# kubernetes-sigs/karpenter

Measured on NVIDIA H100. Metric: pods scheduled/sec, higher is better.
Workload: dtype int64

## Files before the change

### karpenter_b200/csrc/kp_api.cu

```cuda
#include <cuda_runtime.h>
#include <cub/cub.cuh>

#include <dlfcn.h>

#include <chrono>
#include <cstdio>
#include <cstdlib>
#include <memory>
#include <string>
#include <vector>

#include "kp_consolidate.cuh"
#include "kp_gosort_host.hpp"
#include "kp_prep.hpp"

#define CK(call)                                                                                     \
  do {                                                                                               \
    cudaError_t e_ = (call);                                                                         \
    if (e_ != cudaSuccess) {                                                                         \
      h->err = std::string(#call) + ": " + cudaGetErrorString(e_);                                   \
      return KP_ERR_CUDA;                                                                            \
    }                                                                                                \
  } while (0)

struct Arena {
  struct Chunk {
    char* base;
    size_t cap, used;
  };
  std::vector<Chunk> chunks;
  size_t bytes = 0;
  template <class T>
  cudaError_t alloc(T** out, size_t n) {
    size_t need = (std::max<size_t>(n, 1) * sizeof(T) + 255) & ~(size_t)255;
    bytes += need;
    for (auto& c : chunks)
      if (c.cap - c.used >= need) {
        *out = (T*)(c.base + c.used);
        c.used += need;
        return cudaSuccess;
      }
    size_t cap = std::max<size_t>(need, (size_t)32 << 20);
    void* p = nullptr;
    cudaError_t e = cudaMalloc(&p, cap);
    if (e != cudaSuccess) return e;
    chunks.push_back(Chunk{(char*)p, cap, need});
    *out = (T*)p;
    return cudaSuccess;
  }
  void reset() {
    if (chunks.size() > 1) {
      size_t total = bytes + bytes / 4;
      destroy();
      void* p = nullptr;
      if (cudaMalloc(&p, total) == cudaSuccess) chunks.push_back(Chunk{(char*)p, total, 0});
    }
    for (auto& c : chunks) c.used = 0;
    bytes = 0;
  }
  void destroy() {
    for (auto& c : chunks) cudaFree(c.base);
    chunks.clear();
  }
};

struct Instance {
  KpDev dev;
  HostTables host;
  bool resident = false;
  int64_t P = 0;
  int n_keys = 0, n_resources = 0, n_its = 0, hostname_key = -1, n_nodes = 0;
  std::vector<int> key_nvalues;
  std::vector<int64_t> tmpl_remaining0;
  int32_t* d_pod_class = nullptr;
  int64_t* d_pod_creation = nullptr;
  uint64_t *d_uid_hi = nullptr, *d_uid_lo = nullptr;
  int64_t* d_class_rank = nullptr;
  int32_t *d_nsig_rs = nullptr, *d_nsig_tolset = nullptr;
  int64_t* d_rv_req = nullptr;
  int strict_undefined = 0;
  struct Reset {
    void* dst;
    const void* src;
    size_t bytes;
  };
  std::vector<Reset> resets;
  const int32_t* d_host_cnt_nodes = nullptr;
  const uint32_t* d_host_pop_nodes = nullptr;
  void *sort_keys_a = nullptr, *sort_keys_b = nullptr, *sort_tmp = nullptr;
  int32_t* sort_perm_b = nullptr;
  size_t sort_tmp_bytes = 0;
  bool lean = false;
  bool cohort = false;
  int max_its = 0;
  PriceTabs price_tabs{};
  double* trunc_key = nullptr;
  int32_t* trunc_val = nullptr;
  unsigned long long* trunc_bits = nullptr;
  uint8_t* d_dropped = nullptr;
  int CS = 0, CR = 0;
  size_t smem = 0;
  int32_t* d_slot_src = nullptr;
  int64_t n_slots = 0, slot_off = 0;
};

struct NcclApi {
  void* lib = nullptr;
  int (*GetUniqueId)(void*) = nullptr;
  int (*CommInitRank)(void**, int,  struct KpNcclId, int) = nullptr;
  int (*AllReduce)(const void*, void*, size_t, int, int, void*, cudaStream_t) = nullptr;
  int (*CommDestroy)(void*) = nullptr;
  const char* (*GetErrorString)(int) = nullptr;
};
struct KpNcclId {
  char internal[128];
};
static NcclApi g_nccl;
static bool nccl_load(std::string& err) {
  if (g_nccl.lib) return true;
  void* lib = dlopen("libnccl.so.2", RTLD_NOW | RTLD_GLOBAL);
  if (!lib) lib = dlopen("libnccl.so", RTLD_NOW | RTLD_GLOBAL);
  if (!lib) {
    err = std::string("NCCL is not available: ") + dlerror();
    return false;
  }
  g_nccl.GetUniqueId = (int (*)(void*))dlsym(lib, "ncclGetUniqueId");
  g_nccl.CommInitRank = (int (*)(void**, int, KpNcclId, int))dlsym(lib, "ncclCommInitRank");
  g_nccl.AllReduce = (int (*)(const void*, void*, size_t, int, int, void*, cudaStream_t))dlsym(lib, "ncclAllReduce");
  g_nccl.CommDestroy = (int (*)(void*))dlsym(lib, "ncclCommDestroy");
  g_nccl.GetErrorString = (const char* (*)(int))dlsym(lib, "ncclGetErrorString");
  if (!g_nccl.GetUniqueId || !g_nccl.CommInitRank || !g_nccl.AllReduce || !g_nccl.CommDestroy) {
    err = "libnccl lacks an expected symbol";
    return false;
  }
  g_nccl.lib = lib;
  return true;
}

struct kp_handle {
  int device = 0;
  int n_sm = 132;
  cudaStream_t stream = nullptr;
  std::string err;
  Arena arena;
  enum Uploader { NONE, SINGLE, BATCH } uploaded = NONE;
  std::vector<std::unique_ptr<Instance>> insts;
  KpDev* d_devs = nullptr;
  int2* d_plan = nullptr;
  int devs_cap = 0;
  void* comm = nullptr;
  int comm_rank = 0, comm_world = 1;
  int32_t* d_gcnt = nullptr;
  int64_t gcnt_slots = 0;
  float allreduce_ms = 0;
  cudaEvent_t ev3 = nullptr;
  kp_stats stats{};
  cudaEvent_t ev0 = nullptr, ev1 = nullptr;
};

template <class T>
static cudaError_t up(kp_handle* h, const T** dst, const std::vector<T>& v) {
  T* p;
  cudaError_t e = h->arena.alloc(&p, v.size());
  if (e != cudaSuccess) return e;
  if (!v.empty()) e = cudaMemcpyAsync(p, v.data(), v.size() * sizeof(T), cudaMemcpyHostToDevice, h->stream);
  h->stats.bytes_h2d += v.size() * sizeof(T);
  *dst = p;
  return e;
}
template <class T>
static cudaError_t up_mut(kp_handle* h, Instance& in, T** dst, const std::vector<T>& v) {
  const T* init;
  cudaError_t e = up(h, &init, v);
  if (e != cudaSuccess) return e;
  T* work;
  e = h->arena.alloc(&work, v.size());
  if (e != cudaSuccess) return e;
  if (!v.empty()) in.resets.push_back(Instance::Reset{work, init, v.size() * sizeof(T)});
  *dst = work;
  return cudaSuccess;
}
template <class T>
static cudaError_t up_raw(kp_handle* h, T** dst, const T* src, size_t n) {
  T* p;
  cudaError_t e = h->arena.alloc(&p, n);
  if (e != cudaSuccess) return e;
  if (n) e = cudaMemcpyAsync(p, src, n * sizeof(T), cudaMemcpyHostToDevice, h->stream);
  h->stats.bytes_h2d += n * sizeof(T);
  *dst = p;
  return e;
}
template <class T>
static cudaError_t zeros(kp_handle* h, T** dst, size_t n) {
  T* p;
  cudaError_t e = h->arena.alloc(&p, n);
  if (e != cudaSuccess) return e;
  e = cudaMemsetAsync(p, 0, std::max<size_t>(n, 1) * sizeof(T), h->stream);
  *dst = p;
  return e;
}

__global__ void k_sort_keys(const int32_t* pod_class, const int64_t* class_rank, const int32_t* perm, int64_t n,
                            int64_t* out) {
  int64_t i = blockIdx.x * (int64_t)blockDim.x + threadIdx.x;
  if (i < n) out[i] = class_rank[pod_class[perm[i]]];
}
template <class T>
__global__ void k_gather(const T* src, const int32_t* perm, int64_t n, T* out) {
  int64_t i = blockIdx.x * (int64_t)blockDim.x + threadIdx.x;
  if (i < n) out[i] = src[perm[i]];
}
__global__ void k_fill_i32(int32_t* p, int64_t n, int32_t v) {
  int64_t i = blockIdx.x * (int64_t)blockDim.x + threadIdx.x;
  if (i < n) p[i] = v;
}

__global__ void k_scatter_counts(const int32_t* dom_cnt, const int32_t* slot_src, int64_t n, int32_t* out) {
  int64_t i = blockIdx.x * (int64_t)blockDim.x + threadIdx.x;
  if (i < n) out[i] = dom_cnt[slot_src[i]];
}

__global__ void k_slot_kats(const int64_t* val_int, uint64_t isint, uint64_t univ, const kp_slot_case* cs, int n, kp_slot_out* out) {
  const int i = blockIdx.x * blockDim.x + threadIdx.x;
  if (i >= n) return;
  const KeyInfo ki{val_int, isint, univ};
  const kp_slot_case c = cs[i];
  const Slot a{c.flags_a, c.mask_a, c.gte_a, c.lte_a}, b{c.flags_b, c.mask_b, c.gte_b, c.lte_b};
  kp_slot_out o;
  memset(&o, 0, sizeof(o));
  if (slot_present(a) && slot_present(b)) {
    const Slot r = slot_intersection(ki, a, b);
    o.mask = r.m;
    o.gte = r.gte;
    o.lte = r.lte;
    o.flags = r.f;
    o.op = slot_op(r);
    o.has_intersection = slot_has_intersection(ki, a, b);
  }
  o.has_value = c.value >= 0 ? slot_has(ki, a, c.value) : 0;
  o.compatible = slot_compatible(ki, a, b, c.well_known != 0, c.allow_undefined != 0);
  out[i] = o;
}

static int kp_consolidate_impl(kp_handle* h, const kp_problem* p, const kp_consol_input* in, int64_t deadline_ms,
                               kp_consol_result* out);
extern "C" {

int kp_debug_slot_algebra(kp_handle* h, const int64_t* value_int, uint64_t value_is_int, uint64_t universe,
                          const kp_slot_case* cases, int32_t n, kp_slot_out* out) {
  if (n < 0 || !value_int || (n > 0 && (!cases || !out))) return h->err = "kp_debug_slot_algebra: bad arguments", KP_ERR_INVALID;
  cudaSetDevice(h->device);
  int64_t* dv = nullptr;
  kp_slot_case* dc = nullptr;
  kp_slot_out* dout = nullptr;
  CK(cudaMalloc(&dv, 64 * 8));
  CK(cudaMalloc(&dc, sizeof(kp_slot_case) * std::max(n, 1)));
  CK(cudaMalloc(&dout, sizeof(kp_slot_out) * std::max(n, 1)));
  CK(cudaMemcpy(dv, value_int, 64 * 8, cudaMemcpyHostToDevice));
  CK(cudaMemcpy(dc, cases, sizeof(kp_slot_case) * n, cudaMemcpyHostToDevice));
  if (n > 0) k_slot_kats<<<(n + 127) / 128, 128, 0, h->stream>>>(dv, value_is_int, universe, dc, n, dout);
  CK(cudaStreamSynchronize(h->stream));
  CK(cudaGetLastError());
  CK(cudaMemcpy(out, dout, sizeof(kp_slot_out) * n, cudaMemcpyDeviceToHost));
  cudaFree(dv);
  cudaFree(dc);
  cudaFree(dout);
  return KP_OK;
}
}

extern "C" {

#define KP_TRUNC_BLOCKS 132
int kp_version(void) { return KP_ABI_VERSION; }

int kp_go_sort_f64(const double* keys, int32_t n, int32_t* perm_out) {
  if (n < 0 || (n > 0 && (!keys || !perm_out))) return KP_ERR_INVALID;
  host_go_sort(keys, n, perm_out);
  return KP_OK;
}
int kp_go_sort_i64(const int64_t* keys, int32_t n, int32_t* perm_out) {
  if (n < 0 || (n > 0 && (!keys || !perm_out))) return KP_ERR_INVALID;
  host_go_sort(keys, n, perm_out);
  return KP_OK;
}

int kp_create(int device, kp_handle** out) {
  *out = nullptr;
  int count = 0;
  if (cudaGetDeviceCount(&count) != cudaSuccess || count == 0) return KP_ERR_CUDA;
  kp_handle* h = new kp_handle();
  if (device < 0) cudaGetDevice(&device);
  h->device = device;
  if (cudaSetDevice(device) != cudaSuccess || cudaStreamCreate(&h->stream) != cudaSuccess) {
    delete h;
    return KP_ERR_CUDA;
  }
  cudaEventCreate(&h->ev0);
  cudaEventCreate(&h->ev1);
  cudaEventCreate(&h->ev3);
  cudaDeviceGetAttribute(&h->n_sm, cudaDevAttrMultiProcessorCount, device);
// ... 38 lines not shown
  d.E = t.E;
  d.D = t.D;
  d.n_reqsets = t.n_reqsets;
  d.n_taintsets = t.n_taintsets;
  d.n_tolsets = t.n_tolsets;
  d.has_bounds = t.has_bounds;
  d.hostname_key = t.hostname_key;
  d.nodes_res = t.nodes_res;
  d.n_rv = t.n_rv;
  d.stable_order = p->claim_order_mode == 1;
  CK(up(h, &d.key_wellknown, t.key_wellknown));
  CK(up(h, &d.key_univ, t.key_univ));
  CK(up(h, &d.val_int, t.val_int));
  CK(up(h, &d.val_isint, t.val_isint));
  CK(up(h, &d.rs_flags, t.rs_flags));
  CK(up(h, &d.rs_mask, t.rs_mask));
  CK(up(h, &d.rs_gte, t.rs_gte));
  CK(up(h, &d.rs_lte, t.rs_lte));
  CK(up(h, &d.tol_ok, t.tol_ok));
  CK(up(h, &d.itv_off, t.itv_off));
  CK(up(h, &d.itv, t.itv));
  CK(up(h, &d.it_nokey, t.it_nokey));
  CK(up(h, &d.it_dne, t.it_dne));
  CK(up(h, &d.it_nonempty, t.it_nonempty));
  CK(up(h, &d.it_valid, t.it_valid));
  CK(up(h, &d.ge_off, t.ge_off));
  CK(up(h, &d.ge_vals, t.ge_vals));
  CK(up(h, &d.ge_bits, t.ge_bits));
  d.n_ge = (int)t.ge_vals.size();
  d.n_itv = std::max(t.itv_off[d.K], 1);
  CK(up(h, &d.off_slots, t.off_slots));
  CK(up(h, &d.off_keys, t.off_keys));
  CK(up(h, &d.offset_bits, t.offset_bits));
  CK(up(h, &d.it_capacity, t.it_capacity));
  CK(up(h, &d.tmpl_rs, t.tmpl_rs));
  CK(up(h, &d.tmpl_taintset, t.tmpl_taintset));
  CK(up(h, &d.tmpl_its_raw, t.tmpl_its_raw));
  CK(zeros(h, &d.tmpl_its, t.tmpl_its_raw.size()));
  CK(up(h, &d.tmpl_daemon, t.tmpl_daemon));
  CK(up_mut(h, in, &d.tmpl_remaining, t.tmpl_remaining));
  CK(up(h, &d.tmpl_limit_present, t.tmpl_limit_present));
  CK(up(h, &d.cls_req, t.cls_req));
  CK(up(h, &d.cls_rs, t.cls_rs));
  CK(up(h, &d.cls_tolset, t.cls_tolset));
  CK(up(h, &d.cls_relax, t.cls_relax));
  d.mv_strict = t.min_values_strict ? 1 : 0;
  CK(up(h, &d.tmpl_mv_off, t.tmpl_mv_off));
  CK(up(h, &d.tmpl_mv_key, t.tmpl_mv_key));
  CK(up(h, &d.tmpl_mv_need, t.tmpl_mv_need));
  CK(up(h, &d.mv_val_off, t.mv_val_off));
  CK(up(h, &d.mv_masks, t.mv_masks));
  CK(up(h, &d.cls_match, t.cls_match));
  CK(up(h, &d.cls_rec, t.cls_rec));
  {
    if (t.N > 64) return h->err = "more than 64 NodePools", KP_ERR_CAPACITY;
    const ClassPlan& plan = t.plan;
    const bool domain_fp = !getenv("KP_NO_DOMAIN_FP");
    const size_t XK = (size_t)std::max(t.X, 1) * t.K;
    std::vector<int64_t> pg(XK, 0), pl(XK, 0), sg(XK, 0), sl(XK, 0);
    std::vector<ClsLane> rows((size_t)std::max(t.X, 1) * 32);
    memset(rows.data(), 0, rows.size() * sizeof(ClsLane));
    for (int x = 0; x < t.X; x++) {
      const int nm = t.cls_match_off[x + 1] - t.cls_match_off[x], nr = t.cls_rec_off[x + 1] - t.cls_rec_off[x];
      const int asig = plan.asig[x];
      int tki = 0xff;
      if (!plan.chain[x]) {
        tki = asig < 64 ? asig | TKI_ABIT : 0xff;
        if (plan.fast[x] && asig < 64) tki |= TKI_FAST;
        if (plan.fp[x] && nm <= KP_PG && nr <= KP_PG && domain_fp) tki |= TKI_FP | (plan.has_tk[x] ? TKI_TK : 0);
        if (nm + nr > 0) tki |= TKI_TOPO;
      }
      const int32_t hdr[KP_HDR] = {t.cls_tolset[x], t.cls_rv[x], t.cls_match_off[x], t.cls_match_off[x + 1], t.cls_rec_off[x],
                                   t.cls_rec_off[x + 1], plan.fsig[x], plan.nsig[x], plan.hchk_off[x], plan.hchk_off[x + 1]};
      const size_t a = (size_t)t.cls_rs[x] * t.K, b = (size_t)t.cls_strict_rs[x] * t.K;
      for (int l = 0; l < 32; l++) {
        ClsLane& c = rows[(size_t)x * 32 + l];
        if (l < t.K) {
          c.pod_m = t.rs_mask[a + l];
          c.strict_m = t.rs_mask[b + l];
          c.pod_f = t.rs_flags[a + l];
          c.strict_f = t.rs_flags[b + l];
          pg[(size_t)x * t.K + l] = t.rs_gte[a + l];
          pl[(size_t)x * t.K + l] = t.rs_lte[a + l];
          sg[(size_t)x * t.K + l] = t.rs_gte[b + l];
          sl[(size_t)x * t.K + l] = t.rs_lte[b + l];
        }
        if (l < t.R) c.req = t.cls_req[(size_t)x * t.R + l];
        if (l < KP_HDR) c.hdr = hdr[l];
        if (l == KP_HDR + 2) c.hdr = (int32_t)(plan.tok[x] & 0xffffffffull);
        if (l == KP_HDR + 3) c.hdr = (int32_t)(plan.tok[x] >> 32);
        if (l == KP_HDR + 4) c.hdr = t.cls_relax[x];
        if (l == KP_HDR + 5) c.hdr = tki;
        if (l == KP_HDR + 10) c.hdr = t.cls_vol_next[x];
        if (l >= KP_HDR + 6 && l <= KP_HDR + 9 && p->n_hostports > 0 && p->class_hostports) {
          const uint64_t ports = p->class_hostports[x];
          uint64_t conf = 0;
          for (uint64_t m = ports; m;) {
            const int i = __builtin_ctzll(m);
            m &= m - 1;
            conf |= p->hostport_conflicts[i];
          }
          const uint64_t v = l < KP_HDR + 8 ? ports : conf;
          c.hdr = (int32_t)(((l - KP_HDR) & 1) ? (v >> 32) : (v & 0xffffffffull));
        }
      }
    }
    std::vector<int4> hchk;
    for (const HostCheck& c : plan.hchk) hchk.push_back(int4{c.row, c.type | (c.self << 8), c.max_skew, c.g});
    if (hchk.empty()) hchk.push_back(int4{0, 0, 0, 0});
    std::vector<int32_t> nsig_rs = plan.nsig_rs, nsig_tolset = plan.nsig_tolset;
    if (nsig_rs.empty()) {
      nsig_rs.push_back(0);
      nsig_tolset.push_back(-1);
    }
    d.tk_key = plan.tk_key;
    d.n_fsig = plan.n_fsig;
    d.n_nsig = (int)plan.nsig_rs.size();
    d.EW = (t.E + 31) / 32;
    in.strict_undefined = plan.strict_undefined ? 1 : 0;
    std::vector<int64_t> rv_req((size_t)std::max(t.n_rv, 1) * t.R, 0);
    for (int x = 0; x < t.X; x++)
      for (int r = 0; r < t.R; r++) rv_req[(size_t)t.cls_rv[x] * t.R + r] = t.cls_req[(size_t)x * t.R + r];
    {
      const int32_t *a_, *b_;
      const int64_t* c_;
      CK(up(h, &a_, nsig_rs));
      CK(up(h, &b_, nsig_tolset));
      CK(up(h, &c_, rv_req));
      in.d_nsig_rs = const_cast<int32_t*>(a_);
      in.d_nsig_tolset = const_cast<int32_t*>(b_);
      in.d_rv_req = const_cast<int64_t*>(c_);
    }
    CK(up(h, &d.cls_hchk, hchk));
    std::vector<uint32_t> nact(std::max(d.EW, 1), 0);
    for (int n = 0; n < t.E; n++)
      if (t.node_flags[n] & KP_NODE_SCHEDULABLE) nact[n >> 5] |= 1u << (n & 31);
    CK(up_mut(h, in, &d.nactive, nact));
    d.ESW = (d.EW + 31) / 32;
    CK(zeros(h, &d.nfit_sum, (size_t)std::max(t.n_rv, 1) * std::max(d.ESW, 1)));
    CK(zeros(h, &d.nstat_sum, (size_t)std::max(d.n_nsig, 1) * std::max(d.ESW, 1)));
    CK(zeros(h, &d.nfit, (size_t)std::max(t.n_rv, 1) * std::max(d.EW, 1)));
    CK(zeros(h, &d.nstat, (size_t)std::max(d.n_nsig, 1) * std::max(d.EW, 1)));
    CK(up(h, &d.cls_lane, rows));
    CK(up(h, &d.cp_g, pg));
    CK(up(h, &d.cp_l, pl));
    CK(up(h, &d.cs_g, sg));
    CK(up(h, &d.cs_l, sl));
  }
  CK(up(h, &d.groups, t.groups));
  CK(up(h, &d.filter_rs, t.filter_rs));
  CK(up_mut(h, in, &d.dom_cnt, t.dom_cnt));
  CK(up_mut(h, in, &d.dom_reg, t.dom_reg));
  CK(up_mut(h, in, &d.dom_pop, t.dom_pop));
  d.n_lazy = 0;
  for (int32_t b : t.g_born) d.n_lazy += b == 0;
  CK(up_mut(h, in, &d.g_born, t.g_born));
  CK(up_mut(h, in, &d.g_birth, t.g_birth));
  CK(up(h, &d.cls_lazy_off, t.cls_lazy_off));
  CK(up(h, &d.cls_lazy, t.cls_lazy));
  CK(up_mut(h, in, &d.g_ndomains, t.g_ndomains));
  CK(up_mut(h, in, &d.g_nempty, t.g_nempty));
  CK(up(h, &d.node_taintset, t.node_taintset));
  CK(up(h, &d.node_flags, t.node_flags));
  CK(up_mut(h, in, &d.node_rem, t.node_rem));
  CK(up_mut(h, in, &d.node_rem_present, t.node_rem_present));
  CK(up_mut(h, in, &d.node_sflags, t.node_sflags));
  CK(up_mut(h, in, &d.node_smask, t.node_smask));
  CK(up_mut(h, in, &d.node_sgte, t.node_sgte));
  CK(up_mut(h, in, &d.node_slte, t.node_slte));
  CK(zeros(h, &d.node_npods, (size_t)std::max(t.E, 1)));
  d.Cmax = cmax_hint;
  size_t C = (size_t)d.Cmax;
  CK(zeros(h, &d.c_tmpl, C));
  CK(zeros(h, &d.c_npods, C));
  CK(zeros(h, &d.c_req, C * t.R));
  CK(zeros(h, &d.c_sflags, C * t.K));
  CK(zeros(h, &d.c_smask, C * t.K));
  CK(zeros(h, &d.c_sgte, C * t.K));
  CK(zeros(h, &d.c_slte, C * t.K));
  CK(zeros(h, &d.c_its, C * t.ITW));
  CK(zeros(h, &d.c_j, C * t.R));
  CK(zeros(h, &d.order, C));
  CK(zeros(h, &d.cnt_at, C));
  CK(zeros(h, &d.cmask, C));
  CK(zeros(h, &d.amask, C));
  CK(zeros(h, &d.c_dom, C));
  d.n_hostports = p->n_hostports > 0 ? p->n_hostports : 0;
  if (d.n_hostports > 64) return h->err = "more than 64 distinct host ports", KP_ERR_CAPACITY;
  if (d.n_hostports > 0 && !p->hostport_conflicts) return h->err = "hostport_conflicts is null", KP_ERR_INVALID;
  {
    std::vector<unsigned long long> np(std::max(t.E, 1), 0ull), tp(std::max(t.N, 1), 0ull);
    for (int n = 0; n < t.E; n++)
      if (d.n_hostports && p->node_hostports) np[n] = p->node_hostports[n];
    for (int n = 0; n < t.N; n++)
      if (d.n_hostports && p->tmpl_hostports) tp[n] = p->tmpl_hostports[n];
    CK(up_mut(h, in, &d.node_ports, np));
    CK(up(h, &d.tmpl_ports, tp));
    CK(zeros(h, &d.c_ports, C));
  }
  d.n_rsv = t.n_rsv;
  d.rsv_strict = t.rsv_strict ? 1 : 0;
  d.rsv_sets = 0;
  {
    std::vector<int32_t> sr(std::max(t.D, 1), -1);
    for (int dd = 0; dd < t.D && dd < (int)t.set_rsv.size(); dd++) {
      sr[dd] = t.set_rsv[dd];
      if (sr[dd] >= 0) d.rsv_sets |= 1u << dd;
    }
    CK(up(h, &d.set_rsv, sr));
    std::vector<int32_t> cap0 = t.rsv_cap0;
    if (cap0.empty()) cap0.push_back(0);
    CK(up_mut(h, in, &d.rsv_cap, cap0));
    CK(zeros(h, &d.c_rsv, C));
    d.rsv_ct_key = p->reservation_capacity_type_key;
    d.rsv_reserved_val = p->reservation_reserved_value;
    d.rsv_id_key = p->reservation_id_key;
    memset(d.rsv_val_of, 0, sizeof(d.rsv_val_of));
    if (t.n_rsv > 0) {
      if (d.rsv_ct_key < 0 || d.rsv_ct_key >= t.K || d.rsv_id_key < 0 || d.rsv_id_key >= t.K || !p->reservation_value ||
          d.rsv_reserved_val < 0 || d.rsv_reserved_val >= 64)
        return h->err = "reserved offerings need reservation_capacity_type_key / reservation_id_key / reservation_value", KP_ERR_INVALID;
      for (int i = 0; i < t.n_rsv; i++) {
        if (p->reservation_value[i] < 0 || p->reservation_value[i] >= 64) return h->err = "reservation_value out of range", KP_ERR_INVALID;
        d.rsv_val_of[i] = 1ull << p->reservation_value[i];
      }
    }
  }
  d.tmpl_all = t.N >= 64 ? ~0ull : ((1ull << t.N) - 1);
  d.H = t.E + d.Cmax;
  d.GHS = std::max(t.GH, 1);
  CK(zeros(h, &d.host_cnt, (size_t)d.GHS * d.H));
  {
    std::vector<int32_t> tr((size_t)std::max(t.E, 1) * d.GHS, 0);
    for (int r = 0; r < t.GH; r++)
      for (int n = 0; n < t.E; n++) tr[(size_t)n * d.GHS + r] = t.host_cnt_nodes[(size_t)r * t.E + n];
    CK(up(h, &in.d_host_cnt_nodes, tr));
  }
  d.HW = (d.H + 31) / 32;
  CK(zeros(h, &d.host_pop, (size_t)std::max(t.GH, 1) * d.HW));
  {
    const int ew = (t.E + 31) / 32;
    std::vector<uint32_t> bits((size_t)std::max(t.GH, 1) * std::max(ew, 1), 0);
    for (int r = 0; r < t.GH; r++)
      for (int n = 0; n < t.E; n++)
        if (t.host_cnt_nodes[(size_t)r * t.E + n] > 0) bits[(size_t)r * ew + (n >> 5)] |= 1u << (n & 31);
    CK(up(h, &in.d_host_pop_nodes, bits));
  }
  CK(zeros(h, &d.n_claims, 1));
  CK(zeros(h, &d.counters, 16));
  CK(zeros(h, &d.status, 1));
  return KP_OK;
}

static int reset_dynamic(kp_handle* h, Instance& in) {
  HostTables& t = in.host;
  KpDev& d = in.dev;
  for (auto& r : in.resets) CK(cudaMemcpyAsync(r.dst, r.src, r.bytes, cudaMemcpyDeviceToDevice, h->stream));
  CK(cudaMemsetAsync(d.node_npods, 0, (size_t)std::max(t.E, 1) * 4, h->stream));
  size_t C = (size_t)d.Cmax;
  CK(cudaMemsetAsync(d.c_npods, 0, C * 4, h->stream));
  CK(cudaMemsetAsync(d.cmask, 0, C * sizeof(ulonglong2), h->stream));
  CK(cudaMemsetAsync(d.amask, 0, C * 8, h->stream));
  CK(cudaMemsetAsync(d.c_rsv, 0, C * 8, h->stream));
  if (in.d_dropped) CK(cudaMemsetAsync(in.d_dropped, 0, C, h->stream));
  CK(cudaMemsetAsync(d.host_cnt, 0, (size_t)d.GHS * d.H * 4, h->stream));
  if (t.E && t.GH)
    CK(cudaMemcpyAsync(d.host_cnt, in.d_host_cnt_nodes, (size_t)t.E * d.GHS * 4, cudaMemcpyDeviceToDevice, h->stream));
  CK(cudaMemsetAsync(d.host_pop, 0, (size_t)std::max(t.GH, 1) * d.HW * 4, h->stream));
  if (t.E && t.GH) {
    const size_t ew = (size_t)(t.E + 31) / 32;
    CK(cudaMemcpy2DAsync(d.host_pop, (size_t)d.HW * 4, in.d_host_pop_nodes, ew * 4, ew * 4, t.GH,
                         cudaMemcpyDeviceToDevice, h->stream));
  }
  CK(cudaMemsetAsync(d.n_claims, 0, 4, h->stream));
  CK(cudaMemsetAsync(d.counters, 0, 128, h->stream));
  CK(cudaMemsetAsync(d.status, 0, 4, h->stream));
  CK(cudaMemsetAsync(d.last_len, 0, (size_t)std::max<int64_t>(in.P, 1) * 4, h->stream));
  return KP_OK;
}

static int plan_tables(const KpDev& d, size_t fixed, size_t budget) {
  const size_t tb = kp_tab_bytes(d);
  return (fixed + tb <= budget && tb <= 110 * 1024) ? (int)tb : 0;
}

static void plan_solve(Instance& in) {
  KpDev& d = in.dev;
  const size_t budget = 224 * 1024;
  const size_t fixed = KP_ALIGN16(sizeof(WSolveShared));
  d.tab_bytes = plan_tables(d, fixed, budget);
  size_t tb = d.tab_bytes;
  auto row_bytes = [&](int cr) {
    return KP_ALIGN16((size_t)cr * d.K * 8) + KP_ALIGN16((size_t)cr * d.R * 8) + KP_ALIGN16((size_t)cr * d.ITW * 8) +
           KP_ALIGN16((size_t)cr * d.R * 4) + KP_ALIGN16((size_t)cr * d.K);
  };
  int CR = std::min(d.Cmax, 512);
  while (CR > 0 && fixed + tb + row_bytes(CR) > budget / 2) CR -= 32;
  CR = std::max(CR, 0);
  if (getenv("KP_CS_LIMIT")) CR = std::min(CR, 32);
  if (const char* e = getenv("KP_CR")) CR = std::min(CR, std::max(0, atoi(e)) / 32 * 32);
  tb += CR ? row_bytes(CR) : 0;
  auto small_bytes = [&](int cs) { return (size_t)cs * 37; };
  int CS = 0;
  if (fixed + tb + small_bytes(64) + 64 <= budget) {
    int lo = 64, hi = ((d.Cmax + 31) / 32) * 32;
    if (const char* e = getenv("KP_CS_CAP")) hi = std::min(hi, std::max(64, atoi(e) / 32 * 32));
    while (lo < hi) {
      int mid = ((lo + hi + 32) / 64) * 32;
      if (mid <= lo) mid = lo + 32;
      if (fixed + tb + small_bytes(mid) + 64 <= budget)
        lo = mid;
      else
        hi = mid - 32;
    }
    CS = lo;
  }
  if (const char* lim = getenv("KP_CS_LIMIT")) CS = std::min(CS, std::max(0, atoi(lim)) / 32 * 32);
  in.lean = in.host.G == 0 && !in.host.has_bounds && !in.host.min_values_strict && in.host.n_rsv == 0 && d.n_hostports == 0 &&
            !in.host.has_vol_alts && !getenv("KP_NO_LEAN");
  if (in.host.has_vol_alts) in.cohort = false;
  in.CS = CS;
  in.CR = CR;
  in.smem = fixed + tb + (CS ? small_bytes(CS) : 0) + 64;
}

static void begin_upload(kp_handle* h, kp_handle::Uploader by) {
  cudaSetDevice(h->device);
  cudaStreamSynchronize(h->stream);
  h->insts.clear();
  h->uploaded = by;
  h->d_gcnt = nullptr;
  h->gcnt_slots = 0;
  h->arena.reset();
  h->stats = kp_stats{};
}

static int add_instance(kp_handle* h, const kp_problem* p, int64_t cmax) {
  h->insts.push_back(std::make_unique<Instance>());
  Instance& in = *h->insts.back();
  auto t0 = std::chrono::steady_clock::now();
  std::vector<uint8_t> active(p->n_nodes, 0);
  for (int i = 0; i < p->n_nodes; i++) active[i] = (p->node_flags[i] & KP_NODE_SCHEDULABLE) != 0;
  std::vector<int32_t> pending(p->pod_class, p->pod_class + p->n_pods);
  int rc = kp_prepare(p, active, {}, pending, in.host, h->err);
  if (rc != KP_OK) return rc;
  auto t1 = std::chrono::steady_clock::now();
  h->stats.prep_ms += std::chrono::duration<double, std::milli>(t1 - t0).count();
  in.P = p->n_pods;
  in.n_keys = p->n_keys;
  in.n_resources = p->n_resources;
  in.n_its = p->n_its;
  in.n_nodes = p->n_nodes;
  in.hostname_key = in.host.hostname_key;
  in.key_nvalues.resize(p->n_keys);
  for (int k = 0; k < p->n_keys; k++) in.key_nvalues[k] = p->key_value_off[k + 1] - p->key_value_off[k];
  if (p->n_pods >= (1ll << 31) - 2) return h->err = "more than 2^31 pods", KP_ERR_CAPACITY;
  rc = upload_tables(h, in, p, (int)cmax);
  if (rc != KP_OK) return rc;
  KpDev& d = in.dev;
  d.P = p->n_pods;
  size_t P = (size_t)p->n_pods;
  CK(up_raw(h, &in.d_pod_class, p->pod_class, P));
  d.pod_class = in.d_pod_class;
  if (p->pod_creation) {
    CK(up_raw(h, &in.d_pod_creation, p->pod_creation, P));
  } else {
    CK(zeros(h, &in.d_pod_creation, P));
  }
  CK(up_raw(h, &in.d_uid_hi, p->pod_uid_hi, P));
  CK(up_raw(h, &in.d_uid_lo, p->pod_uid_lo, P));
  const std::vector<int64_t>& rank = in.host.plan.rank;
  CK(up_raw(h, &in.d_class_rank, rank.data(), rank.size()));
  {
    const int X = in.host.X;
    std::vector<int64_t> pods_of(std::max(X, 1), 0), classes_at(std::max(X, 1), 0);
    for (size_t i = 0; i < P; i++) pods_of[p->pod_class[i]]++;
    for (int x = 0; x < X; x++)
      if (pods_of[x] > 0) classes_at[rank[x]]++;
    int64_t in_runs = 0;
    for (int x = 0; x < X; x++)
      if (pods_of[x] > 1 && classes_at[rank[x]] == 1) in_runs += pods_of[x];
    in.cohort = (in_runs * 4 >= (int64_t)P && P > 0 && !getenv("KP_NO_COHORT")) || getenv("KP_COHORT");
    d.cohort = in.cohort ? 1 : 0;
  }
  in.max_its = p->max_instance_types > 0 ? p->max_instance_types : 0;
  if (in.max_its > 0) {
    const int T = p->n_its;
    const PriceLists ml = order_by_price(p, in.host);
    CK(up(h, &in.price_tabs.ml_off, ml.off));
    CK(up(h, &in.price_tabs.ml_set, ml.set));
    CK(up(h, &in.price_tabs.ml_price, ml.price));
    const size_t NW = (size_t)KP_TRUNC_BLOCKS * 4;
    CK(h->arena.alloc(&in.trunc_key, NW * std::max(T, 1)));
    CK(h->arena.alloc(&in.trunc_val, NW * std::max(T, 1)));
    CK(h->arena.alloc(&in.trunc_bits, NW * std::max((T + 63) / 64, 1)));
    CK(zeros(h, &in.d_dropped, (size_t)std::max<int64_t>(d.Cmax, 1)));
  }
  {
    int64_t* ka;
    int64_t* kb;
    CK(h->arena.alloc(&ka, P));
    CK(h->arena.alloc(&kb, P));
    CK(h->arena.alloc(&in.sort_perm_b, P));
    in.sort_keys_a = ka;
    in.sort_keys_b = kb;
    size_t n1 = 0, n2 = 0;
    cub::DeviceRadixSort::SortPairs(nullptr, n1, (const uint64_t*)nullptr, (uint64_t*)nullptr, (const int32_t*)nullptr,
                                    (int32_t*)nullptr, (int)std::max<size_t>(P, 1));
    cub::DeviceRadixSort::SortPairs(nullptr, n2, (const int64_t*)nullptr, (int64_t*)nullptr, (const int32_t*)nullptr,
                                    (int32_t*)nullptr, (int)std::max<size_t>(P, 1));
    in.sort_tmp_bytes = std::max(n1, n2);
    char* tmp;
    CK(h->arena.alloc(&tmp, in.sort_tmp_bytes));
    in.sort_tmp = tmp;
  }
  CK(zeros(h, &d.queue, P + 1));
  CK(zeros(h, &d.qcls, P + 1));
  CK(zeros(h, &d.last_len, P));
  CK(zeros(h, &d.pod_target, P));
  CK(zeros(h, &d.pod_error, P));
  CK(cudaStreamSynchronize(h->stream));
  auto t2 = std::chrono::steady_clock::now();
  h->stats.upload_ms += std::chrono::duration<double, std::milli>(t2 - t1).count();
  plan_solve(in);
  in.resident = true;
  return KP_OK;
}

static int upload(kp_handle* h, const kp_problem* const* problems, int n, const int64_t* cmax, kp_handle::Uploader by) {
  begin_upload(h, by);
  for (int b = 0; b < n; b++) {
    int rc = add_instance(h, problems[b], cmax[b]);
    if (rc != KP_OK) return rc;
  }
  return KP_OK;
}

static int64_t cmax_guess(const kp_problem* p) {
  return std::max<int64_t>(1, std::min<int64_t>(p->n_pods, std::max<int64_t>(4096, p->n_pods / 8)));
}

int kp_upload(kp_handle* h, const kp_problem* p) {
  const int64_t cmax = cmax_guess(p);
  return upload(h, &p, 1, &cmax, kp_handle::SINGLE);
}

__global__ void k_iota(int32_t* p, int64_t n) {
  int64_t i = blockIdx.x * (int64_t)blockDim.x + threadIdx.x;
  if (i < n) p[i] = (int32_t)i;
}

static int sort_queue(kp_handle* h, Instance& in) {
  KpDev& d = in.dev;
  const int64_t P = in.P;
  if (P <= 0) return KP_OK;
  const int nb = (int)((P + 255) / 256), n = (int)P;
  int32_t* perm_a = d.queue;
  int32_t* perm_b = in.sort_perm_b;
  uint64_t *ua = (uint64_t*)in.sort_keys_a, *ub = (uint64_t*)in.sort_keys_b;
  int64_t *sa = (int64_t*)in.sort_keys_a, *sb = (int64_t*)in.sort_keys_b;
  size_t tb = in.sort_tmp_bytes;
  k_iota<<<nb, 256, 0, h->stream>>>(perm_a, P);
  k_gather<<<nb, 256, 0, h->stream>>>(in.d_uid_lo, perm_a, P, ua);
  CK(cub::DeviceRadixSort::SortPairs(in.sort_tmp, tb, ua, ub, perm_a, perm_b, n, 0, 64, h->stream));
  k_gather<<<nb, 256, 0, h->stream>>>(in.d_uid_hi, perm_b, P, ua);
  CK(cub::DeviceRadixSort::SortPairs(in.sort_tmp, tb, ua, ub, perm_b, perm_a, n, 0, 64, h->stream));
  k_gather<<<nb, 256, 0, h->stream>>>(in.d_pod_creation, perm_a, P, sa);
  CK(cub::DeviceRadixSort::SortPairs(in.sort_tmp, tb, sa, sb, perm_a, perm_b, n, 0, 64, h->stream));
  k_sort_keys<<<nb, 256, 0, h->stream>>>(d.pod_class, in.d_class_rank, perm_b, P, sa);
  CK(cub::DeviceRadixSort::SortPairs(in.sort_tmp, tb, sa, sb, perm_b, perm_a, n, 0, 64, h->stream));
  k_gather<<<nb, 256, 0, h->stream>>>(d.pod_class, d.queue, P, d.qcls);
  h->stats.kernel_launches += 6;
  return KP_OK;
}

static int launch_node_cand(kp_handle* h, Instance& in) {
  KpDev& d = in.dev;
  if (d.E <= 0) return KP_OK;
  dim3 grid((d.E + 255) / 256, d.n_nsig + d.n_rv);
  k_node_cand<<<grid, 256, 0, h->stream>>>(d, in.d_nsig_rs, in.d_nsig_tolset, in.d_rv_req, in.strict_undefined);
  const int nsum = (d.n_rv + d.n_nsig) * d.ESW;
  k_node_sum<<<(nsum + 255) / 256, 256, 0, h->stream>>>(d);
  h->stats.kernel_launches += 2;
  return KP_OK;
}

static int prep_solve(kp_handle* h, Instance& in) {
  KpDev& d = in.dev;
  if (d.N > 0) {
    k_feasibility<<<(d.N * 32 + 255) / 256, 256, 0, h->stream>>>(d, nullptr, 1);
    h->stats.kernel_launches++;
  }
  int rc = sort_queue(h, in);
  if (rc != KP_OK) return rc;
  if (in.P > 0) {
    k_fill_i32<<<(int)((in.P + 255) / 256), 256, 0, h->stream>>>(d.pod_target, in.P, KP_TARGET_UNSCHEDULED);
    h->stats.kernel_launches++;
  }
  return launch_node_cand(h, in);
}

static int reduce_counters(kp_handle* h) {
  if (!h->d_gcnt) return KP_OK;
  CK(cudaEventRecord(h->ev3, h->stream));
  CK(cudaMemsetAsync(h->d_gcnt, 0, (size_t)h->gcnt_slots * 4, h->stream));
  for (auto& in : h->insts)
    if (in->n_slots > 0) {
      k_scatter_counts<<<(int)((in->n_slots + 255) / 256), 256, 0, h->stream>>>(in->dev.dom_cnt, in->d_slot_src, in->n_slots,
                                                                                 h->d_gcnt + in->slot_off);
      h->stats.kernel_launches++;
    }
  if (h->comm) {
    int rc = g_nccl.AllReduce(h->d_gcnt, h->d_gcnt, (size_t)h->gcnt_slots,  2,  0, h->comm, h->stream);
    if (rc != 0) return h->err = std::string("ncclAllReduce: ") + (g_nccl.GetErrorString ? g_nccl.GetErrorString(rc) : "?"), KP_ERR_CUDA;
  }
  return KP_OK;
}

static const void* solver_kernel(const std::vector<std::unique_ptr<Instance>>& insts) {
  bool lean = true, cohort = false, vol = false;
  for (auto& in : insts) {
    lean = lean && in->lean;
    cohort = cohort || in->cohort;
    vol = vol || in->host.has_vol_alts;
  }
  if (vol) return (const void*)k_wsolve_batch<false, false, true>;
  return lean ? (cohort ? (const void*)k_wsolve_batch<true, true> : (const void*)k_wsolve_batch<true, false>)
              : (cohort ? (const void*)k_wsolve_batch<false, true> : (const void*)k_wsolve_batch<false, false>);
}

static int run_solve(kp_handle* h, int64_t deadline_ms, std::vector<int32_t>& statuses) {
  const int n = (int)h->insts.size();
  statuses.assign(n, KP_OK);
  if (n == 0) return KP_OK;
  cudaSetDevice(h->device);
  if (n > h->devs_cap) {
    cudaFree(h->d_devs);
    cudaFree(h->d_plan);
    h->d_devs = nullptr;
    h->d_plan = nullptr;
    h->devs_cap = 0;
    CK(cudaMalloc(&h->d_devs, sizeof(KpDev) * n));
    CK(cudaMalloc(&h->d_plan, sizeof(int2) * n));
    h->devs_cap = n;
  }
  std::vector<KpDev> devs(n);
  std::vector<int2> plan(n);
  size_t smem = 0;
  for (int b = 0; b < n; b++) {
    Instance& in = *h->insts[b];
    if (!in.resident) return h->err = "the last upload did not complete", KP_ERR_INVALID;
    in.dev.deadline_ns = deadline_ms > 0 ? deadline_ms * 1000000ll : 0;
    int rc = reset_dynamic(h, in);
    if (rc != KP_OK) return rc;
    devs[b] = in.dev;
    plan[b] = make_int2(in.CS, in.CR);
    smem = std::max(smem, in.smem);
  }
  CK(cudaMemcpyAsync(h->d_devs, devs.data(), sizeof(KpDev) * n, cudaMemcpyHostToDevice, h->stream));
  CK(cudaMemcpyAsync(h->d_plan, plan.data(), sizeof(int2) * n, cudaMemcpyHostToDevice, h->stream));
  CK(cudaEventRecord(h->ev0, h->stream));
  h->stats.kernel_launches = 0;
  h->stats.cohort_pods = 0;
  for (auto& in : h->insts) {
    int rc = prep_solve(h, *in);
    if (rc != KP_OK) return rc;
  }
  const void* fn = solver_kernel(h->insts);
  CK(cudaFuncSetAttribute(fn, cudaFuncAttributeMaxDynamicSharedMemorySize, (int)smem));
  {
    void* args[] = {(void*)&h->d_devs, (void*)&h->d_plan};
    CK(cudaLaunchKernel(fn, dim3(n), dim3(64), args, smem, h->stream));
  }
  h->stats.kernel_launches++;
  for (auto& in : h->insts)
    if (in->max_its > 0) {
      k_truncate_claims<<<KP_TRUNC_BLOCKS, 128, 0, h->stream>>>(in->dev, in->price_tabs, in->max_its, in->trunc_key, in->trunc_val,
                                                                 in->trunc_bits, in->d_dropped);
      if (in->P > 0)
        k_mark_dropped<<<(int)((in->P + 255) / 256), 256, 0, h->stream>>>(in->dev.pod_target, in->dev.pod_error, in->d_dropped, in->P);
      h->stats.kernel_launches += 2;
    }
  int rc = reduce_counters(h);
  if (rc != KP_OK) return rc;
  CK(cudaEventRecord(h->ev1, h->stream));
  CK(cudaStreamSynchronize(h->stream));
  CK(cudaGetLastError());
  float ms = 0;
  cudaEventElapsedTime(&ms, h->ev0, h->ev1);
  h->stats.solve_ms = ms;
  if (h->d_gcnt) cudaEventElapsedTime(&h->allreduce_ms, h->ev3, h->ev1);
  if (getenv("KP_DEBUG")) fprintf(stderr, "[kp] %d instance(s): step %.3f ms\n", n, ms);
  for (int b = 0; b < n; b++) CK(cudaMemcpy(&statuses[b], h->insts[b]->dev.status, 4, cudaMemcpyDeviceToHost));
  return KP_OK;
}

struct ReqLayout {
  int K, hostname_key;
  std::vector<int> woff;
  explicit ReqLayout(const Instance& in) : K(in.n_keys), hostname_key(in.hostname_key), woff(in.n_keys + 1, 0) {
    for (int k = 0; k < K; k++) woff[k + 1] = woff[k] + (k == hostname_key ? 0 : (in.key_nvalues[k] + 63) / 64);
  }
  int words() const { return woff[K]; }
  void store(size_t r, const uint8_t* sf, const uint64_t* sm, const int64_t* sg, const int64_t* sl, uint8_t* flags,
             int64_t* gte, int64_t* lte, uint64_t* mask) const {
    for (int k = 0; k < K; k++) {
      const uint8_t f = sf[k];
      if (!(f & SF_PRESENT) || k == hostname_key) continue;
      flags[r * K + k] = KP_SLOT_PRESENT | ((f & SF_COMPLEMENT) ? KP_REQ_COMPLEMENT : 0) | ((f & SF_HAS_GTE) ? KP_REQ_HAS_GTE : 0) |
                         ((f & SF_HAS_LTE) ? KP_REQ_HAS_LTE : 0);
      if ((f & SF_HAS_GTE) && sg) gte[r * K + k] = sg[k];
      if ((f & SF_HAS_LTE) && sl) lte[r * K + k] = sl[k];
      if (woff[k + 1] > woff[k]) mask[r * words() + woff[k]] = sm[k];
    }
  }
};

static int download(kp_handle* h, Instance& in, kp_result* out) {
  KpDev& d = in.dev;
  auto t0 = std::chrono::steady_clock::now();
  memset(out, 0, sizeof(*out));
  int32_t nclaims = 0;
  int64_t counters[16];
  CK(cudaMemcpy(&nclaims, d.n_claims, 4, cudaMemcpyDeviceToHost));
  CK(cudaMemcpy(counters, d.counters, 128, cudaMemcpyDeviceToHost));
  h->stats.cohort_pods += counters[5];
  if (getenv("KP_DEBUG"))
    fprintf(stderr, "[kp] slow_sorts=%lld evals=%lld commits=%lld fast_commits=%lld cohort_pods=%lld\n", (long long)counters[4],
            (long long)counters[6], (long long)counters[3], (long long)counters[9], (long long)counters[5]);
  int64_t P = in.P;
  int K = in.n_keys, R = in.n_resources, ITW = (in.n_its + 63) / 64;
  size_t C = (size_t)nclaims, c1 = C ? C : 1;
  out->n_pods = P;
  out->pod_target = (int32_t*)malloc(sizeof(int32_t) * (P ? P : 1));
  out->pod_error = (uint8_t*)malloc(P ? P : 1);
  CK(cudaMemcpy(out->pod_target, d.pod_target, P * 4, cudaMemcpyDeviceToHost));
  CK(cudaMemcpy(out->pod_error, d.pod_error, P, cudaMemcpyDeviceToHost));
  out->n_claims = nclaims;
  out->claim_template = (int32_t*)calloc(c1, 4);
  out->claim_npods = (int32_t*)calloc(c1, 4);
  out->claim_rank = (int32_t*)calloc(c1, 4);
  out->claim_reservations = (uint64_t*)calloc(c1, 8);
  CK(cudaMemcpy(out->claim_reservations, d.c_rsv, C * 8, cudaMemcpyDeviceToHost));
  out->claim_dropped = (uint8_t*)calloc(c1, 1);
  if (in.d_dropped) CK(cudaMemcpy(out->claim_dropped, in.d_dropped, C, cudaMemcpyDeviceToHost));
  out->claim_requests = (int64_t*)calloc(c1 * R, 8);
  out->it_words = ITW;
  out->claim_its = (uint64_t*)calloc(c1 * (ITW ? ITW : 1), 8);
  CK(cudaMemcpy(out->claim_template, d.c_tmpl, C * 4, cudaMemcpyDeviceToHost));
  CK(cudaMemcpy(out->claim_npods, d.c_npods, C * 4, cudaMemcpyDeviceToHost));
  CK(cudaMemcpy(out->claim_requests, d.c_req, C * R * 8, cudaMemcpyDeviceToHost));
  CK(cudaMemcpy(out->claim_its, d.c_its, C * ITW * 8, cudaMemcpyDeviceToHost));
  std::vector<int32_t> order(c1);
  CK(cudaMemcpy(order.data(), d.order, C * 4, cudaMemcpyDeviceToHost));
  for (size_t pos = 0; pos < C; pos++) out->claim_rank[order[pos]] = (int32_t)pos;
  std::vector<uint8_t> sf(c1 * K);
  std::vector<uint64_t> sm(c1 * K);
  std::vector<int64_t> sg(c1 * K), sl(c1 * K);
  CK(cudaMemcpy(sf.data(), d.c_sflags, C * K, cudaMemcpyDeviceToHost));
  CK(cudaMemcpy(sm.data(), d.c_smask, C * K * 8, cudaMemcpyDeviceToHost));
  CK(cudaMemcpy(sg.data(), d.c_sgte, C * K * 8, cudaMemcpyDeviceToHost));
  CK(cudaMemcpy(sl.data(), d.c_slte, C * K * 8, cudaMemcpyDeviceToHost));
  const ReqLayout L(in);
  const int MW = L.words();
  out->n_keys = K;
  out->mask_words = MW;
  out->claim_req_flags = (uint8_t*)calloc(c1 * (K ? K : 1), 1);
  out->claim_req_gte = (int64_t*)calloc(c1 * (K ? K : 1), 8);
  out->claim_req_lte = (int64_t*)calloc(c1 * (K ? K : 1), 8);
  out->claim_req_mask = (uint64_t*)calloc(c1 * (MW ? MW : 1), 8);
  for (size_t c = 0; c < C; c++)
    L.store(c, sf.data() + c * K, sm.data() + c * K, sg.data() + c * K, sl.data() + c * K, out->claim_req_flags,
            out->claim_req_gte, out->claim_req_lte, out->claim_req_mask);
  HostTables& t = in.host;
  std::vector<int32_t> cnt((size_t)std::max(t.G, 1) * 64);
  CK(cudaMemcpy(cnt.data(), d.dom_cnt, cnt.size() * 4, cudaMemcpyDeviceToHost));
  std::vector<int32_t> birth(std::max(t.G, 1));
  CK(cudaMemcpy(birth.data(), d.g_birth, birth.size() * 4, cudaMemcpyDeviceToHost));
  std::vector<int> gorder;
  for (int g = 0; g < t.n_regular; g++)
    if (t.g_born[g]) gorder.push_back(g);
  {
    std::vector<std::pair<int, int>> born;
    for (int g = 0; g < t.n_regular; g++)
      if (!t.g_born[g] && birth[g] >= 0) born.push_back({birth[g], g});
    std::sort(born.begin(), born.end());
    for (auto& b : born) gorder.push_back(b.second);
  }
  for (int g = t.n_regular; g < t.G; g++) gorder.push_back(g);
  std::vector<int32_t> off{0}, flat;
  for (int g : gorder) {
    int key = t.groups[g].key;
    if (key != t.hostname_key) {
      int nv = in.key_nvalues[key];
      for (int v = 0; v < nv; v++) flat.push_back(cnt[(size_t)g * 64 + v]);
    }
    off.push_back((int32_t)flat.size());
  }
  out->n_groups = (int32_t)gorder.size();
  out->n_domain_slots = (int32_t)flat.size();
  out->group_domain_off = (int32_t*)malloc(off.size() * 4);
  memcpy(out->group_domain_off, off.data(), off.size() * 4);
  out->domain_counts = (int32_t*)malloc((flat.size() ? flat.size() : 1) * 4);
  if (!flat.empty()) memcpy(out->domain_counts, flat.data(), flat.size() * 4);
  out->n_existing_evals = counters[0];
  out->n_inflight_evals = counters[1];
  out->n_template_evals = counters[2];
  out->n_commits = counters[3];
  out->solve_ms = h->stats.solve_ms;
  h->stats.bytes_d2h += P * 5 + C * (8 + (size_t)R * 8 + (size_t)ITW * 8 + (size_t)K * 25) + cnt.size() * 4;
  auto t1 = std::chrono::steady_clock::now();
  h->stats.download_ms += std::chrono::duration<double, std::milli>(t1 - t0).count();
  return KP_OK;
}

static int download_all(kp_handle* h, const std::vector<int32_t>& statuses, kp_result* outs) {
  h->stats.download_ms = 0;
  h->stats.bytes_d2h = 0;
  int worst = KP_OK;
  for (size_t b = 0; b < h->insts.size(); b++) {
    int rc = download(h, *h->insts[b], &outs[b]);
    if (rc != KP_OK) {
      for (size_t i = 0; i < b; i++) kp_result_free(&outs[i]);
      return rc;
    }
    if (statuses[b] == KP_DEADLINE) worst = KP_DEADLINE;
  }
  return worst;
}

static int solve_uploaded(kp_handle* h, int64_t deadline_ms, kp_result* outs) {
  std::vector<int32_t> st;
  int rc = run_solve(h, deadline_ms, st);
  if (rc != KP_OK) return rc;
  for (int32_t s : st)
    if (s != KP_OK && s != KP_DEADLINE) return h->err = "claim capacity exceeded", s;
  return download_all(h, st, outs);
}

static int solve_growing(kp_handle* h, const kp_problem* const* problems, int n, kp_handle::Uploader by, int64_t deadline_ms,
                         kp_result* outs) {
  std::vector<int64_t> cmax(n);
  for (int b = 0; b < n; b++) cmax[b] = cmax_guess(problems[b]);
  for (;;) {
    int rc = upload(h, problems, n, cmax.data(), by);
    if (rc != KP_OK) return rc;
    std::vector<int32_t> st;
    rc = run_solve(h, deadline_ms, st);
    if (rc != KP_OK) return rc;
    bool grow = false;
    for (int b = 0; b < n; b++) {
      if (st[b] == KP_ERR_CAPACITY && cmax[b] < problems[b]->n_pods) {
        cmax[b] = std::min<int64_t>(problems[b]->n_pods, cmax[b] * 4);
        grow = true;
      } else if (st[b] != KP_OK && st[b] != KP_DEADLINE) {
        return h->err = "claim capacity exceeded", st[b];
      }
    }
    if (!grow) return download_all(h, st, outs);
  }
}

int kp_solve_resident(kp_handle* h, int64_t deadline_ms, kp_result* out) {
  if (h->uploaded != kp_handle::SINGLE) return h->err = "kp_upload has not been called", KP_ERR_INVALID;
  return solve_uploaded(h, deadline_ms, out);
}

int kp_solve(kp_handle* h, const kp_problem* p, int64_t deadline_ms, kp_result* out) {
  return solve_growing(h, &p, 1, kp_handle::SINGLE, deadline_ms, out);
}

int kp_comm_unique_id(uint8_t* id128) {
  std::string err;
  if (!nccl_load(err)) return KP_ERR_CUDA;
  KpNcclId id;
  if (g_nccl.GetUniqueId(&id) != 0) return KP_ERR_CUDA;
  memcpy(id128, &id, sizeof(id));
  return KP_OK;
}

int kp_comm_init(kp_handle* h, const uint8_t* id128, int32_t rank, int32_t world) {
  if (!nccl_load(h->err)) return KP_ERR_CUDA;
  if (h->comm) {
    g_nccl.CommDestroy(h->comm);
    h->comm = nullptr;
  }
  cudaSetDevice(h->device);
  KpNcclId id;
  memcpy(&id, id128, sizeof(id));
  int rc = g_nccl.CommInitRank(&h->comm, world, id, rank);
  if (rc != 0) return h->err = std::string("ncclCommInitRank: ") + (g_nccl.GetErrorString ? g_nccl.GetErrorString(rc) : "?"), KP_ERR_CUDA;
  h->comm_rank = rank;
  h->comm_world = world;
  return KP_OK;
}

static Instance* pick_instance(kp_handle* h, int32_t instance) {
  const size_t i = instance < 0 ? 0 : (size_t)instance;
  if (h->uploaded != (instance < 0 ? kp_handle::SINGLE : kp_handle::BATCH) || i >= h->insts.size()) return nullptr;
  return h->insts[i]->resident ? h->insts[i].get() : nullptr;
}
int64_t kp_comm_counter_slots(kp_handle* h, int32_t instance) {
  Instance* in = pick_instance(h, instance);
  if (!in) return -1;
  int64_t n = 0;
  for (int g = 0; g < in->host.G; g++)
    if (in->host.groups[g].key != in->host.hostname_key) n += in->key_nvalues[in->host.groups[g].key];
  return n;
}

int kp_comm_set_counter_layout(kp_handle* h, int64_t total_slots, const int64_t* slot_offset, int32_t n_instances) {
  cudaSetDevice(h->device);
  if (n_instances <= 0 ? !pick_instance(h, -1) : h->uploaded != kp_handle::BATCH || n_instances != (int)h->insts.size())
    return h->err = "kp_comm_set_counter_layout: the instances do not match the upload", KP_ERR_INVALID;
  if (total_slots < 0) return h->err = "kp_comm_set_counter_layout: negative size", KP_ERR_INVALID;
  CK(h->arena.alloc(&h->d_gcnt, (size_t)std::max<int64_t>(total_slots, 1)));
  h->gcnt_slots = total_slots;
  for (size_t i = 0; i < h->insts.size(); i++) {
    Instance* in = h->insts[i].get();
    std::vector<int32_t> src;
    for (int g = 0; g < in->host.G; g++) {
      const int key = in->host.groups[g].key;
      if (key == in->host.hostname_key) continue;
      for (int v = 0; v < in->key_nvalues[key]; v++) src.push_back(g * 64 + v);
    }
    in->n_slots = (int64_t)src.size();
    in->slot_off = slot_offset[i];
    if (in->slot_off < 0 || in->slot_off + in->n_slots > total_slots)
      return h->err = "kp_comm_set_counter_layout: slice outside the table", KP_ERR_INVALID;
    CK(h->arena.alloc(&in->d_slot_src, std::max<size_t>(src.size(), 1)));
    if (!src.empty()) CK(cudaMemcpyAsync(in->d_slot_src, src.data(), src.size() * 4, cudaMemcpyHostToDevice, h->stream));
    CK(cudaStreamSynchronize(h->stream));
  }
  return KP_OK;
}

int kp_comm_global_counts(kp_handle* h, int32_t* out, int64_t n) {
  if (!h->d_gcnt || n != h->gcnt_slots) return h->err = "kp_comm_global_counts: no table of that size", KP_ERR_INVALID;
  cudaSetDevice(h->device);
  CK(cudaMemcpy(out, h->d_gcnt, (size_t)n * 4, cudaMemcpyDeviceToHost));
  return KP_OK;
}

double kp_comm_last_allreduce_ms(kp_handle* h) { return h->allreduce_ms; }

void kp_comm_destroy(kp_handle* h) {
  if (h->comm && g_nccl.CommDestroy) g_nccl.CommDestroy(h->comm);
  h->comm = nullptr;
}

int kp_upload_batch(kp_handle* h, const kp_problem* const* problems, int32_t n) {
  if (n < 0 || (n > 0 && !problems)) return h->err = "kp_upload_batch: bad arguments", KP_ERR_INVALID;
  std::vector<int64_t> cmax(n);
  for (int b = 0; b < n; b++) cmax[b] = cmax_guess(problems[b]);
  return upload(h, problems, n, cmax.data(), kp_handle::BATCH);
}

int kp_solve_batch_resident(kp_handle* h, int64_t deadline_ms, kp_result* outs) {
  if (h->uploaded != kp_handle::BATCH) return KP_OK;
  return solve_uploaded(h, deadline_ms, outs);
}

int kp_solve_batch(kp_handle* h, const kp_problem* const* problems, int32_t n, int64_t deadline_ms, kp_result* outs) {
  if (n < 0 || (n > 0 && (!problems || !outs))) return h->err = "kp_solve_batch: bad arguments", KP_ERR_INVALID;
  return solve_growing(h, problems, n, kp_handle::BATCH, deadline_ms, outs);
}

void kp_result_free(kp_result* r) {
  free(r->pod_target);
  free(r->pod_error);
  free(r->claim_template);
  free(r->claim_npods);
  free(r->claim_rank);
  free(r->claim_requests);
  free(r->claim_its);
  free(r->claim_req_flags);
  free(r->claim_req_gte);
  free(r->claim_req_lte);
  free(r->claim_req_mask);
  free(r->group_domain_off);
  free(r->domain_counts);
  free(r->claim_reservations);
  free(r->claim_dropped);
  memset(r, 0, sizeof(*r));
}

int kp_feasibility(kp_handle* h, const kp_problem* p, uint64_t* out_bits, int32_t* out_it_words) {
  const int64_t one = 1;
  int rc = upload(h, &p, 1, &one, kp_handle::SINGLE);
  if (rc != KP_OK) return rc;
  KpDev& d = h->insts[0]->dev;
  *out_it_words = d.ITW;
  size_t n = (size_t)d.X * d.N * d.ITW;
  uint64_t* dout;
  CK(cudaMalloc(&dout, std::max<size_t>(n, 1) * 8));
  if (d.N > 0) k_feasibility<<<(d.N * 32 + 255) / 256, 256, 0, h->stream>>>(d, nullptr, 1);
  CK(cudaEventRecord(h->ev0, h->stream));
  if (d.N > 0 && d.X > 0) {
    int blocks = h->n_sm * 8;
    k_feasibility<<<blocks, 256, 0, h->stream>>>(d, dout, 0);
  }
  CK(cudaEventRecord(h->ev1, h->stream));
  CK(cudaStreamSynchronize(h->stream));
  CK(cudaGetLastError());
  float ms = 0;
  cudaEventElapsedTime(&ms, h->ev0, h->ev1);
  h->stats.solve_ms = ms;
  CK(cudaMemcpy(out_bits, dout, n * 8, cudaMemcpyDeviceToHost));
  cudaFree(dout);
  return KP_OK;
}

int kp_consolidate(kp_handle* h, const kp_problem* cluster, const kp_consol_input* in, int64_t deadline_ms,
                   kp_consol_result* out) {
  memset(out, 0, sizeof(*out));
  int rc = kp_consolidate_impl(h, cluster, in, deadline_ms, out);
  if (rc != KP_OK && rc != KP_DEADLINE) kp_consol_result_free(out);
  return rc;
}

void kp_consol_result_free(kp_consol_result* r) {
  free(r->decision);
  free(r->replacement_its);
  free(r->n_new_claims);
  free(r->n_unscheduled);
  free(r->repl_template);
  free(r->repl_requests);
  free(r->repl_req_flags);
  free(r->repl_req_gte);
  free(r->repl_req_lte);
  free(r->repl_req_mask);
  free(r->repl_order_off);
  free(r->repl_order);
  memset(r, 0, sizeof(*r));
}
}

__global__ void k_scatter_rank(const int32_t* perm, int64_t n, int32_t* rank) {
  int64_t i = blockIdx.x * (int64_t)blockDim.x + threadIdx.x;
  if (i < n) rank[perm[i]] = (int32_t)i;
}

static int read_consol(kp_handle* h, const KpConsol& q, int n, const int32_t* at, const ReqLayout& L, int R, int ITW,
                       std::vector<std::vector<int32_t>>& order_rows, kp_consol_result* out) {
  const size_t K = (size_t)L.K, n1 = (size_t)std::max(n, 1), cap = (size_t)q.order_cap;
  auto sub = [&](size_t b) { return at ? (size_t)at[b] : b; };
  auto rows = [&](auto* dst, const auto* src, size_t width) {
    const size_t row = width * sizeof(*dst);
    if (!at) return cudaMemcpy(dst, src, n * row, cudaMemcpyDeviceToHost);
    std::vector<std::remove_pointer_t<decltype(dst)>> tmp(n1 * width);
    const cudaError_t e = cudaMemcpy(tmp.data(), src, n * row, cudaMemcpyDeviceToHost);
    for (size_t b = 0; b < (size_t)n; b++) memcpy(dst + sub(b) * width, tmp.data() + b * width, row);
    return e;
  };
  CK(rows(out->decision, q.decision, 1));
  CK(rows(out->replacement_its, q.replacement_its, ITW));
  CK(rows(out->n_new_claims, q.n_new_claims, 1));
  CK(rows(out->n_unscheduled, q.n_unscheduled, 1));
  CK(rows(out->repl_template, q.repl_tmpl, 1));
  CK(rows(out->repl_requests, q.repl_req, R));
  std::vector<uint8_t> sfl(n1 * K);
  std::vector<uint64_t> smk(n1 * K);
  std::vector<int32_t> on(n1), ord(q.repl_order ? n1 * cap : 0);
  std::vector<int64_t> sg(q.repl_sgte ? n1 * K : 0), sl(sg.size());
  CK(cudaMemcpy(sfl.data(), q.repl_sflags, (size_t)n * K, cudaMemcpyDeviceToHost));
  CK(cudaMemcpy(smk.data(), q.repl_smask, (size_t)n * K * 8, cudaMemcpyDeviceToHost));
  if (q.repl_sgte) {
    CK(cudaMemcpy(sg.data(), q.repl_sgte, (size_t)n * K * 8, cudaMemcpyDeviceToHost));
    CK(cudaMemcpy(sl.data(), q.repl_slte, (size_t)n * K * 8, cudaMemcpyDeviceToHost));
  }
  if (q.repl_order) {
    CK(cudaMemcpy(ord.data(), q.repl_order, (size_t)n * cap * 4, cudaMemcpyDeviceToHost));
    CK(cudaMemcpy(on.data(), q.repl_order_n, (size_t)n * 4, cudaMemcpyDeviceToHost));
  }
  for (size_t b = 0; b < (size_t)n; b++) {
    const size_t s = sub(b);
    if (out->decision[s] != KP_DECISION_REPLACE)
      out->repl_template[s] = -1;
    else
      L.store(s, sfl.data() + b * K, smk.data() + b * K, q.repl_sgte ? sg.data() + b * K : nullptr,
              q.repl_sgte ? sl.data() + b * K : nullptr, out->repl_req_flags, out->repl_req_gte, out->repl_req_lte,
              out->repl_req_mask);
    if (q.repl_order) order_rows[s].assign(ord.begin() + b * cap, ord.begin() + b * cap + on[b]);
  }
  return KP_OK;
}

static int kp_consolidate_impl(kp_handle* h, const kp_problem* p, const kp_consol_input* in, int64_t deadline_ms,
                               kp_consol_result* out) {
  const auto t_call = std::chrono::steady_clock::now();
  const int S = in->n_subsets;
  const int n_extra = in->n_extra_pods > 0 ? in->n_extra_pods : 0;
  if (p->n_nodes > 0 && !in->node_pod_off) return h->err = "kp_consolidate: node_pod_off is null", KP_ERR_INVALID;
  const int64_t extra_row0 = p->n_nodes > 0 ? in->node_pod_off[p->n_nodes] : 0;
  if (n_extra > 0 && (!in->extra_pod_kind || extra_row0 + n_extra != p->n_pods))
    return h->err = "kp_consolidate: the extra pods must be the last n_extra_pods rows of the pod table, with kinds", KP_ERR_INVALID;
  for (int i = 0; i < n_extra; i++)
// ... 396 lines not shown
```

### karpenter_b200/csrc/kp_consolidate.cuh

```cuda
#pragma once
#include "kp_wsolve.cuh"

#define KP_ALIGN16(x) (((x) + 15) & ~(size_t)15)

__host__ __device__ inline size_t kp_tab_bytes(const KpDev& d) {
  size_t K = d.K, R = d.R, ITW = d.ITW, D = d.D > 0 ? d.D : 1, N = d.N > 0 ? d.N : 1;
  size_t b = 0;
  b += KP_ALIGN16(K) + 2 * KP_ALIGN16(8 * K);
  b += KP_ALIGN16(4 * (R + 1)) + KP_ALIGN16(8 * (size_t)d.n_ge) + KP_ALIGN16(8 * (size_t)d.n_ge * ITW);
  b += KP_ALIGN16(4 * (K + 1)) + KP_ALIGN16(8 * (size_t)d.n_itv * ITW);
  b += 3 * KP_ALIGN16(8 * K * ITW) + KP_ALIGN16(8 * ITW);
  b += KP_ALIGN16(sizeof(Slot) * D * K) + KP_ALIGN16(4 * D) + KP_ALIGN16(8 * D * ITW);
  b += KP_ALIGN16(4 * N);
  b += KP_ALIGN16(4 * (size_t)d.n_rv * d.ESW) + KP_ALIGN16(4 * (size_t)d.n_nsig * d.ESW);
  return b;
}

__device__ __forceinline__ void stage_tables(const KpDev& d_in, KpDev* ds, unsigned char* tab) {
  const int tid = threadIdx.x, nt = blockDim.x;
  {
    const int* src = reinterpret_cast<const int*>(&d_in);
    int* dst = reinterpret_cast<int*>(ds);
    for (int i = tid; i < (int)(sizeof(KpDev) / 4); i += nt) dst[i] = src[i];
  }
  __syncthreads();
  if (d_in.tab_bytes > 0) {
    size_t off = 0;
#define KP_STAGE(field, type, count)                                     \
  {                                                                      \
    size_t n_ = (size_t)(count);                                         \
    type* dst_ = reinterpret_cast<type*>(tab + off);                     \
    const type* src_ = d_in.field;                                       \
    for (size_t i_ = tid; i_ < n_; i_ += nt) dst_[i_] = src_[i_];        \
    if (tid == 0) ds->field = dst_;                                      \
    off += KP_ALIGN16(sizeof(type) * n_);                                \
  }
    const size_t K_ = d_in.K, R_ = d_in.R, W_ = d_in.ITW, D_ = d_in.D > 0 ? d_in.D : 1, N_ = d_in.N > 0 ? d_in.N : 1;
    KP_STAGE(key_wellknown, uint8_t, K_)
    KP_STAGE(key_univ, uint64_t, K_)
    KP_STAGE(val_isint, uint64_t, K_)
    KP_STAGE(ge_off, int32_t, R_ + 1)
    KP_STAGE(ge_vals, int64_t, d_in.n_ge)
    KP_STAGE(ge_bits, uint64_t, (size_t)d_in.n_ge * W_)
    KP_STAGE(itv_off, int32_t, K_ + 1)
    KP_STAGE(itv, uint64_t, (size_t)d_in.n_itv * W_)
    KP_STAGE(it_nokey, uint64_t, K_ * W_)
    KP_STAGE(it_dne, uint64_t, K_ * W_)
    KP_STAGE(it_nonempty, uint64_t, K_ * W_)
    KP_STAGE(it_valid, uint64_t, W_)
    KP_STAGE(off_slots, Slot, D_ * K_)
    KP_STAGE(off_keys, uint32_t, D_)
    KP_STAGE(offset_bits, uint64_t, D_ * W_)
    KP_STAGE(tmpl_taintset, int32_t, N_)
    KP_STAGE(nfit_sum, uint32_t, (size_t)d_in.n_rv * d_in.ESW)
    KP_STAGE(nstat_sum, uint32_t, (size_t)d_in.n_nsig * d_in.ESW)
#undef KP_STAGE
  }
  __syncthreads();
}

__global__ void __launch_bounds__(256) k_node_cand(KpDev d, const int32_t* nsig_rs, const int32_t* nsig_tolset,
                                                    const int64_t* rv_req, int strict_undefined) {
  const int n = blockIdx.x * blockDim.x + threadIdx.x, row = blockIdx.y, lane = threadIdx.x & 31;
  bool bit = false;
  if (n < d.E) {
    if (row < d.n_nsig) {
      bit = tolerated(d, nsig_tolset[row], d.node_taintset[n]);
      const int rs = nsig_rs[row];
      for (int k = 0; rs >= 0 && k < d.K && bit; k++) {
        Slot pod = rs_slot(d, rs, k);
        if (!slot_present(pod)) continue;
        Slot nd = load_slot(d.node_sflags, d.node_smask, d.node_sgte, d.node_slte, (size_t)n * d.K + k, d.has_bounds);
        if (!slot_present(nd)) {
          if (strict_undefined && !op_is_negative(slot_op(pod))) bit = false;
        } else if (!slot_has_intersection(key_info(d, k), nd, pod) &&
                   !(op_is_negative(slot_op(pod)) && op_is_negative(slot_op(nd)))) {
          bit = false;
        }
      }
    } else {
      const int rv = row - d.n_nsig;
      const uint32_t pr = d.node_rem_present[n];
      bit = true;
      for (int r = 0; r < d.R; r++) {
        const int64_t rem = d.node_rem[(size_t)n * d.R + r];
        const bool present = (pr >> r) & 1;
        if (present && rem < 0) bit = false;
        if (rv_req[(size_t)rv * d.R + r] > (present ? rem : 0)) bit = false;
      }
    }
  }
  const unsigned m = __ballot_sync(FULL, bit);
  const int w = n >> 5;
  if (lane == 0 && w < d.EW) {
    if (row < d.n_nsig)
      d.nstat[(size_t)row * d.EW + w] = m;
    else
      d.nfit[(size_t)(row - d.n_nsig) * d.EW + w] = m;
  }
}

__global__ void __launch_bounds__(256) k_node_sum(KpDev d) {
  const int i = blockIdx.x * blockDim.x + threadIdx.x, rows = d.n_rv + d.n_nsig;
  if (i >= rows * d.ESW) return;
  const int row = i / d.ESW, s = i % d.ESW;
  const uint32_t* src = row < d.n_rv ? d.nfit + (size_t)row * d.EW : d.nstat + (size_t)(row - d.n_rv) * d.EW;
  uint32_t out = 0;
  for (int w = 0; w < 32; w++) {
    const int idx = s * 32 + w;
    if (idx < d.EW && (src[idx] & d.nactive[idx])) out |= 1u << w;
  }
  if (row < d.n_rv)
    d.nfit_sum[(size_t)row * d.ESW + s] = out;
  else
    d.nstat_sum[(size_t)(row - d.n_rv) * d.ESW + s] = out;
}

struct WSolveShared {
  KpDev ds;
  WInst inst;
  StageRing ring;
  Slot scratch[KP_MAXK];
};

template <bool LEAN, bool COHORT, bool VOL>
__device__ __forceinline__ void wsolve_cta(const KpDev& d_in, int CS, int CR) {
  extern __shared__ __align__(16) unsigned char smem_raw[];
  WSolveShared& sh = *reinterpret_cast<WSolveShared*>(smem_raw);
  const int lane = threadIdx.x & 31, warp = threadIdx.x >> 5;
  unsigned char* tab = smem_raw + KP_ALIGN16(sizeof(WSolveShared));
  stage_tables(d_in, &sh.ds, tab);
  const KpDev& d = sh.ds;
  WInst& I = sh.inst;
  const int Cmax = d.Cmax;
  if (threadIdx.x == 0) {
    sh.ring.produced = 0;
    sh.ring.consumed = 0;
    sh.ring.tail_pub = (int)d.P;
    sh.ring.done = 0;
    sh.ring.skip_to = 0;
    I.P = (int)d.P;
    I.queue = d.queue;
    I.qcls = d.qcls;
    I.last_len = d.last_len;
    I.pod_target = d.pod_target;
    I.pod_error = d.pod_error;
    I.pod_kind = d.pod_kind;
    I.Cmax = Cmax;
    I.c_tmpl = d.c_tmpl;
    I.c_npods = d.c_npods;
    I.c_req = d.c_req;
    I.c_sflags = d.c_sflags;
    I.c_smask = d.c_smask;
    I.c_sgte = d.c_sgte;
    I.c_slte = d.c_slte;
    I.c_its = d.c_its;
    I.c_j = d.c_j;
    I.order = d.order;
    I.cnt_at = d.cnt_at;
    I.cmask = d.cmask;
    I.amask = d.amask;
    I.tmpl_remaining = d.tmpl_remaining;
    I.node_rem = d.node_rem;
    I.node_rem_present = d.node_rem_present;
    I.node_sflags = d.node_sflags;
    I.node_smask = d.node_smask;
    I.node_sgte = d.node_sgte;
    I.node_slte = d.node_slte;
    I.node_npods = d.node_npods;
    I.nfit = d.nfit;
    I.nstat = d.nstat;
    I.nactive = d.nactive;
    I.nfit_sum = d.nfit_sum;
    I.nstat_sum = d.nstat_sum;
    I.n_removed = 0;
    I.removed = nullptr;
    I.ov_cap = 0;
    I.n_ov = 0;
    I.CS = 0;
    I.g_order = d.order;
    I.g_cnt_at = d.cnt_at;
    I.g_c_tmpl = d.c_tmpl;
    I.g_cmask = d.cmask;
    I.g_amask = d.amask;
    I.c_dom = d.c_dom;
    I.g_c_dom = d.c_dom;
    I.rsv_cap = d.rsv_cap;
    I.c_rsv = d.c_rsv;
    I.c_ports = d.c_ports;
    I.node_ports = d.node_ports;
    I.ov_ports = nullptr;
    I.CR = 0;
    unsigned char* p = tab + d_in.tab_bytes;
    if (CR > 0) {
      I.s_smask = reinterpret_cast<uint64_t*>(p);
      p += KP_ALIGN16((size_t)CR * d.K * 8);
      I.s_req = reinterpret_cast<int64_t*>(p);
      p += KP_ALIGN16((size_t)CR * d.R * 8);
      I.s_its = reinterpret_cast<uint64_t*>(p);
      p += KP_ALIGN16((size_t)CR * d.ITW * 8);
      I.s_j = reinterpret_cast<int32_t*>(p);
      p += KP_ALIGN16((size_t)CR * d.R * 4);
      I.s_sflags = reinterpret_cast<uint8_t*>(p);
      p += KP_ALIGN16((size_t)CR * d.K);
      I.CR = CR;
    }
    if (CS > 0) {
      I.cmask = reinterpret_cast<ulonglong2*>(p);
      p += (size_t)CS * 16;
      I.amask = reinterpret_cast<unsigned long long*>(p);
      p += (size_t)CS * 8;
      I.order = reinterpret_cast<int32_t*>(p);
      p += (size_t)CS * 4;
      I.cnt_at = reinterpret_cast<int32_t*>(p);
      p += (size_t)CS * 4;
      I.c_tmpl = reinterpret_cast<int32_t*>(p);
      p += (size_t)CS * 4;
      I.c_dom = reinterpret_cast<uint8_t*>(p);
      I.CS = CS;
    }
  }
  __syncthreads();
  if (warp == 1) {
    stager_run<COHORT>(d, I, &sh.ring, lane);
    return;
  }
  wsolve_run<false, true, LEAN, COHORT, VOL>(d, I, sh.ring.slot[0], sh.scratch, lane, &sh.ring);
  const int nC = I.n_claims;
  claim_rows_flush(d, I, nC, lane);
  if (!LEAN) claims_finalize(d, I.c_sflags, I.c_smask, I.c_rsv, nC, lane);
  if (I.CS > 0) {
    for (int i = lane; i < nC; i += 32) {
      d_in.order[i] = I.order[i];
      d_in.cnt_at[i] = I.cnt_at[i];
      d_in.c_tmpl[i] = I.c_tmpl[i];
    }
  }
  if (lane == 0) {
    *d.n_claims = nC;
    *d.status = I.status;
    d.counters[0] = I.ev_existing;
    d.counters[1] = I.ev_inflight;
    d.counters[2] = I.ev_tmpl;
    d.counters[3] = I.commits;
    d.counters[4] = I.slow_sorts;
    d.counters[5] = I.scan_chunks;
    d.counters[6] = I.evals;
    d.counters[7] = I.n_unsched;
    d.counters[8] = I.n_uninit;
    d.counters[9] = I.fast_commits;
  }
}
template <bool LEAN, bool COHORT, bool VOL = false>
__global__ void __launch_bounds__(64, 1) k_wsolve_batch(const KpDev* __restrict__ devs, const int2* __restrict__ plan) {
  wsolve_cta<LEAN, COHORT, VOL>(devs[blockIdx.x], plan[blockIdx.x].x, plan[blockIdx.x].y);
}

struct KpConsol {
  int n_subsets;
  const int32_t* subset_off;
  const int32_t* subset_nodes;
  const int32_t* node_pod_off;
  const int32_t* pod_class;
  const int32_t* pod_rank;
  const double* node_price;
  const uint8_t* node_is_spot;
  const int32_t* node_it;
  int filter_same_type;
  const int32_t* node_tmpl;
  const int64_t* node_capacity;
  const int64_t* tmpl_remaining0;
  const int32_t* wl_off;
  const int32_t* wl_set;
  const double* wl_price;
  const int32_t* ml_off;
  const int32_t* ml_set;
  const double* ml_price;
  int T;
  double* sort_key;
  int32_t* sort_val;
  unsigned long long* sort_bits;
  int ct_key, ct_spot, ct_od, ct_order_valid;
  int spot_to_spot_enabled;
  int n_extra, extra_row0;
  const uint8_t* extra_kind;
  uint8_t* kindl;
  int32_t* rsv_cap;
  unsigned long long* c_rsv;
  unsigned long long *c_ports, *ov_ports;
  long long deadline_ns;
  unsigned long long* t_start;
  int capq;
  int32_t *queue, *qcls, *last_len, *clsl, *rk;
  int32_t *c_tmpl, *c_npods, *order, *cnt_at;
  int64_t* c_req;
  uint8_t* c_sflags;
  uint64_t* c_smask;
  int64_t *c_sgte, *c_slte;
  uint64_t* c_its;
  int32_t* c_j;
  ulonglong2* cmask;
  unsigned long long* amask;
  int64_t* tmpl_remaining;
  int32_t* ov_node;
  int64_t* ov_rem;
  uint32_t* ov_present;
  uint8_t* ov_sflags;
  uint64_t* ov_smask;
  int64_t *ov_sgte, *ov_slte;
  uint8_t* decision;
  uint64_t* replacement_its;
  int32_t* n_new_claims;
  int32_t* n_unscheduled;
  int32_t* repl_tmpl;
  int64_t* repl_req;
  uint8_t* repl_sflags;
  uint64_t* repl_smask;
  int64_t *repl_sgte, *repl_slte;
  int export_order;
  int32_t* repl_order;
  int32_t* repl_order_n;
  int order_cap;
  int32_t* next;
  int32_t* status;
};

struct PriceTabs {
  const int32_t* ml_off;
  const int32_t* ml_set;
  const double* ml_price;
};
__device__ __forceinline__ void order_by_price(const PriceTabs& pt, uint64_t cur, int n_its, unsigned okmask, double* sk,
                                               int32_t* sv, int ITW, int lane) {
  const int cw = lane < ITW ? __popcll(cur) : 0;
  int pre = cw;
  for (int o = 1; o < 32; o <<= 1) {
    const int t = __shfl_up_sync(FULL, pre, o);
    if (lane >= o) pre += t;
  }
  int at = pre - cw;
  for (uint64_t bits = lane < ITW ? cur : 0ull; bits;) {
    const int b = __ffsll((long long)bits) - 1;
    bits &= bits - 1;
    const int t = lane * 64 + b;
    double mp = 1.7976931348623157e308;
    for (int e = pt.ml_off[t]; e < pt.ml_off[t + 1]; e++)
      if ((okmask >> pt.ml_set[e]) & 1u) {
        mp = pt.ml_price[e];
        break;
      }
    sk[at] = mp;
    sv[at] = t;
    at++;
  }
  __syncwarp();
  WarpSorterT<double> srt{sk, sv, lane};
  srt.pdqsort(0, n_its, WarpSorterT<double>::bits_len((unsigned long long)n_its));
}
__device__ __forceinline__ uint64_t first_types_bitmap(const int32_t* sv, int n, unsigned long long* sb, int ITW, int lane) {
  if (lane < ITW) sb[lane] = 0ull;
  __syncwarp();
  for (int i = lane; i < n; i += 32) atomicOr(&sb[sv[i] >> 6], 1ull << (sv[i] & 63));
  __syncwarp();
  return lane < ITW ? sb[lane] : 0ull;
}

__device__ __forceinline__ void consol_decide(const KpDev& d, const KpConsol& q, size_t slot, Slot* scratch,
                                              const uint8_t* c_sflags, const uint64_t* c_smask, const int64_t* c_sgte,
                                              const int64_t* c_slte, const uint64_t* c_its, int c_tmpl0, const int64_t* c_req0,
                                              int c_npods0, int sn, const int32_t* snodes, int unscheduled, int n_new, int s,
                                              int lane) {
  const int K = d.K, ITW = d.ITW;
  int decision = KP_DECISION_NOOP;
  uint64_t rep = 0;
  bool have_slots = false;
  bool spot_pinned = false, mv_dropped = false;
  int n_ord_out = 0;
  if (!unscheduled) {
    if (n_new == 0) {
      decision = KP_DECISION_DELETE;
    } else if (n_new == 1) {
      Slot S = lane < K ? load_slot(c_sflags, c_smask, c_sgte, c_slte, (size_t)lane, d.has_bounds) : slot_absent();
      const uint64_t its = lane < ITW ? c_its[lane] : 0ull;
      int n_its = lane < ITW ? __popcll(its) : 0;
      for (int o = 16; o; o >>= 1) n_its += __shfl_xor_sync(FULL, n_its, o);
      double price = 0;
      bool zero = false, all_spot = true;
      for (int i = 0; i < sn; i++) {
        const double np = q.node_price[snodes[i]];
        if (np < 0) zero = true;
        price += np;
        if (!q.node_is_spot[snodes[i]]) all_spot = false;
      }
      if (zero) price = 0.0;
      bool spot_ok = false;
      if (q.ct_key >= 0 && q.ct_spot >= 0) {
        const uint32_t f = __shfl_sync(FULL, S.f, q.ct_key);
        const uint64_t m = __shfl_sync(FULL, S.m, q.ct_key);
        const int64_t g = __shfl_sync(FULL, S.gte, q.ct_key), l = __shfl_sync(FULL, S.lte, q.ct_key);
        spot_ok = slot_has(key_info(d, q.ct_key), Slot{f, m, g, l}, q.ct_spot);
      }
      if (lane < K) scratch[lane] = S;
      __syncwarp();
      have_slots = true;
      unsigned okmask = offering_ok_mask(d, scratch, lane);
      const bool spot_path = all_spot && spot_ok;
      uint64_t cur = its;
      double* sk = q.sort_key + slot * (size_t)q.T;
// ... 99 lines not shown
        }
        if (any && q.filter_same_type && sn >= 2) {
          double max_price = 1.7976931348623157e308;
          for (int i = 0; i < sn; i++) {
            const int t = q.node_it[snodes[i]];
            if (t < 0) continue;
            const bool in_rep = (__shfl_sync(FULL, rep, t >> 6) >> (t & 63)) & 1ull;
            if (!in_rep) continue;
            double mine = 1.7976931348623157e308;
            for (int j = 0; j < sn; j++)
              if (q.node_it[snodes[j]] == t && q.node_price[snodes[j]] >= 0 && q.node_price[snodes[j]] < mine)
                mine = q.node_price[snodes[j]];
            if (mine > 1e308) mine = 0.0;
            if (mine < max_price) max_price = mine;
          }
          if (max_price < 1e308) {
            uint64_t keep = 0;
            if (lane < ITW)
              for (uint64_t bits = rep; bits;) {
                const int b = __ffsll((long long)bits) - 1;
                bits &= bits - 1;
                const int t = lane * 64 + b;
                double worst = 1.7976931348623157e308;
                for (int ci = 0; ci < 3 && worst > 1e308; ci++) {
                  if (q.ct_key < 0 || !((q.ct_order_valid >> ci) & 1)) continue;
                  for (int e = q.wl_off[t * 3 + ci]; e < q.wl_off[t * 3 + ci + 1]; e++)
                    if ((okmask >> q.wl_set[e]) & 1u) {
                      worst = q.wl_price[e];
                      break;
                    }
                }
                if (worst < max_price) keep |= 1ull << b;
              }
            rep = keep;
            any = __any_sync(FULL, rep != 0);
            if (any && d.mv_strict && !min_values_ok(d, c_tmpl0, rep, lane)) any = false;
          }
        }
        if (any) decision = KP_DECISION_REPLACE;
        if (any && q.export_order && q.repl_order) {
          if (lane < ITW) sb[lane] = rep;
          __syncwarp();
          int32_t* dst = q.repl_order + (size_t)s * q.order_cap;
          for (int b0 = 0; b0 < n_ord; b0 += 32) {
            const int i = b0 + lane;
            const int t = i < n_ord ? sv[i] : 0;
            const bool in = i < n_ord && ((sb[t >> 6] >> (t & 63)) & 1ull);
            const unsigned m = __ballot_sync(FULL, in);
            const int at = n_ord_out + __popc(m & ((1u << lane) - 1));
            if (in && at < q.order_cap) dst[at] = t;
            n_ord_out += __popc(m);
          }
          if (n_ord_out > q.order_cap) n_ord_out = q.order_cap;
        }
      }
    }
  }
  if (decision != KP_DECISION_REPLACE) rep = 0;
  if (lane < ITW) q.replacement_its[(size_t)s * ITW + lane] = rep;
  if (q.repl_tmpl) {
    const bool repl = decision == KP_DECISION_REPLACE && have_slots;
    Slot F = slot_absent();
    if (repl && lane < K) {
      F = scratch[lane];
      if (!spot_pinned && lane == q.ct_key && q.ct_spot >= 0 && q.ct_od >= 0) {
        const KeyInfo ki = key_info(d, lane);
        if (slot_has(ki, F, q.ct_spot) && slot_has(ki, F, q.ct_od)) F = slot_add(ki, F, Slot{SF_PRESENT, 1ull << q.ct_spot, 0, 0});
      }
    }
    if (lane < K) {
      const size_t i = (size_t)s * K + lane;
      q.repl_sflags[i] = (uint8_t)F.f;
      q.repl_smask[i] = F.m;
      if (q.repl_sgte) {
        q.repl_sgte[i] = F.gte;
        q.repl_slte[i] = F.lte;
      }
    }
    if (lane < d.R) q.repl_req[(size_t)s * d.R + lane] = repl ? c_req0[lane] : 0;
    if (lane == 0) {
      q.repl_tmpl[s] = repl ? c_tmpl0 : -1;
      if (q.repl_order_n) q.repl_order_n[s] = repl ? n_ord_out : 0;
    }
  }
  if (lane == 0) {
    q.decision[s] = (uint8_t)decision;
    q.n_new_claims[s] = n_new;
    q.n_unscheduled[s] = unscheduled;
  }
  __syncwarp();
}

#define CONSOL_WARPS 8
struct ConsolWarp {
  WInst inst;
  PodCtx ctx;
  Slot scratch[KP_MAXK];
};
struct ConsolShared {
  KpDev ds;
  ConsolWarp w[CONSOL_WARPS];
};

#ifndef CONSOL_MIN_CTAS
#define CONSOL_MIN_CTAS 2
#endif
template <bool LEAN>
__global__ void __launch_bounds__(CONSOL_WARPS * 32, CONSOL_MIN_CTAS) k_consolidate(const __grid_constant__ KpDev d_in,
                                                                    const __grid_constant__ KpConsol q) {
  extern __shared__ __align__(16) unsigned char smem_raw[];
  ConsolShared& sh = *reinterpret_cast<ConsolShared*>(smem_raw);
  const int lane = threadIdx.x & 31, warp = threadIdx.x >> 5;
  stage_tables(d_in, &sh.ds, smem_raw + KP_ALIGN16(sizeof(ConsolShared)));
  const KpDev& d = sh.ds;
  ConsolWarp& W = sh.w[warp];
  WInst& I = W.inst;
  const int K = d.K, R = d.R, ITW = d.ITW, N = d.N;
  const size_t slot = (size_t)blockIdx.x * CONSOL_WARPS + warp;
  const int capq = q.capq;
  if (lane == 0) {
    I.queue = q.queue + slot * (capq + 1);
    I.qcls = q.qcls + slot * (capq + 1);
    I.last_len = q.last_len + slot * capq;
    I.pod_target = nullptr;
    I.pod_error = nullptr;
    I.Cmax = capq;
    I.c_tmpl = q.c_tmpl + slot * capq;
    I.c_npods = q.c_npods + slot * capq;
    I.c_req = q.c_req + slot * capq * R;
    I.c_sflags = q.c_sflags + slot * capq * K;
    I.c_smask = q.c_smask + slot * capq * K;
    I.c_sgte = q.c_sgte ? q.c_sgte + slot * capq * K : nullptr;
    I.c_slte = q.c_slte ? q.c_slte + slot * capq * K : nullptr;
    I.c_its = q.c_its + slot * capq * ITW;
    I.c_j = q.c_j + slot * capq * R;
    I.order = q.order + slot * capq;
    I.cnt_at = q.cnt_at + slot * capq;
    I.cmask = q.cmask + slot * capq;
    I.amask = q.amask + slot * capq;
    I.tmpl_remaining = q.tmpl_remaining + slot * (size_t)(N > 0 ? N : 1) * R;
    I.node_rem = d.node_rem;
    I.node_rem_present = d.node_rem_present;
    I.node_sflags = d.node_sflags;
    I.node_smask = d.node_smask;
    I.node_sgte = d.node_sgte;
    I.node_slte = d.node_slte;
    I.node_npods = nullptr;
    I.nfit = d.nfit;
    I.nstat = d.nstat;
    I.nactive = d.nactive;
    I.nfit_sum = d.nfit_sum;
    I.nstat_sum = d.nstat_sum;
    I.CS = 0;
    I.CR = 0;
    I.c_dom = nullptr;
    I.g_c_dom = nullptr;
    I.rsv_cap = d.n_rsv ? q.rsv_cap + slot * d.n_rsv : nullptr;
    I.c_rsv = d.n_rsv ? q.c_rsv + slot * capq : nullptr;
    I.c_ports = d.n_hostports ? q.c_ports + slot * capq : nullptr;
    I.ov_ports = d.n_hostports ? q.ov_ports + slot * capq : nullptr;
    I.node_ports = d.node_ports;
    I.ov_cap = capq;
    I.ov_node = q.ov_node + slot * capq;
    I.ov_rem = q.ov_rem + slot * capq * R;
    I.ov_present = q.ov_present + slot * capq;
    I.ov_sflags = q.ov_sflags + slot * capq * K;
    I.ov_smask = q.ov_smask + slot * capq * K;
    I.ov_sgte = q.ov_sgte ? q.ov_sgte + slot * capq * K : nullptr;
    I.ov_slte = q.ov_slte ? q.ov_slte + slot * capq * K : nullptr;
  }
  __syncwarp();
  int32_t* clsl = q.clsl + slot * capq;
  int32_t* rk = q.rk + slot * capq;
  uint8_t* kindl = q.n_extra > 0 ? q.kindl + slot * capq : nullptr;
  if (lane == 0) I.pod_kind = kindl;
  unsigned long long t0 = 0;
  if (q.deadline_ns > 0) {
    if (lane == 0) {
      unsigned long long now;
      asm volatile("mov.u64 %0, %%globaltimer;" : "=l"(now));
      t0 = atomicCAS(q.t_start, 0ull, now);
      if (t0 == 0) t0 = now;
    }
    t0 = __shfl_sync(FULL, t0, 0);
  }

  for (;;) {
    if (q.deadline_ns > 0) {
      unsigned long long now;
      asm volatile("mov.u64 %0, %%globaltimer;" : "=l"(now));
      now = __shfl_sync(FULL, now, 0);
      if ((long long)(now - t0) > q.deadline_ns) break;
    }
    int s = 0;
    if (lane == 0) s = atomicAdd(q.next, 1);
    s = __shfl_sync(FULL, s, 0);
    if (s >= q.n_subsets) break;
    const int so = q.subset_off[s], sn = q.subset_off[s + 1] - so;
    const int32_t* snodes = q.subset_nodes + so;
    int n = 0;
    for (int i = 0; i < sn; i++) {
      const int node = snodes[i];
      const int a = q.node_pod_off[node], b = q.node_pod_off[node + 1];
      for (int j = a + lane; j < b; j += 32) {
        const int o = n + (j - a);
        if (o < capq) {
          clsl[o] = q.pod_class[j];
          rk[o] = q.pod_rank[j];
        }
      }
      n += b - a;
    }
    const int n_cand_pods = n;
    for (int j = lane; j < q.n_extra; j += 32) {
      const int o = n + j;
      if (o < capq) {
        clsl[o] = q.pod_class[q.extra_row0 + j];
        rk[o] = q.pod_rank[q.extra_row0 + j];
      }
    }
    n += q.n_extra;
    if (kindl)
      for (int i = lane; i < n && i < capq; i += 32) kindl[i] = i < n_cand_pods ? 0 : q.extra_kind[i - n_cand_pods];
    if (n > capq) {
      if (lane == 0) *q.status = KP_ERR_CAPACITY;
      break;
    }
    __syncwarp();
    for (int i = lane; i < n; i += 32) {
      const int my = rk[i];
      int pos = 0;
      for (int j = 0; j < n; j++) pos += rk[j] < my ? 1 : 0;
      I.queue[pos] = i;
      I.qcls[pos] = clsl[i];
    }
    if (lane == 0) {
      I.P = n;
      I.n_ov = 0;
      I.n_removed = sn;
      I.removed = snodes;
    }
    for (int i = lane; i < d.n_rsv; i += 32) I.rsv_cap[i] = d.rsv_cap[i];
    for (int i = lane; i < N * R; i += 32) {
      const int t = i / R, r = i % R;
      int64_t rem = q.tmpl_remaining0[i];
      if ((d.tmpl_limit_present[t] >> r) & 1)
        for (int c = 0; c < sn; c++)
          if (q.node_tmpl[snodes[c]] == t) rem += q.node_capacity[(size_t)snodes[c] * R + r];
      I.tmpl_remaining[i] = rem;
    }
    __syncwarp();
    wsolve_run<true, false, LEAN>(d, I, W.ctx, W.scratch, lane);
    if (I.status != KP_OK) {
      if (lane == 0) *q.status = I.status;
      break;
    }
    if (!LEAN) claims_finalize(d, I.c_sflags, I.c_smask, I.c_rsv, I.n_claims, lane);
    consol_decide(d, q, slot, W.scratch, I.c_sflags, I.c_smask, I.c_sgte, I.c_slte, I.c_its, I.n_claims > 0 ? I.c_tmpl[0] : -1,
                  I.c_req, I.n_claims > 0 ? I.c_npods[0] : 0, sn, snodes, I.n_unsched + I.n_uninit, I.n_claims, s, lane);
  }
}

__global__ void __launch_bounds__(32) k_decide_batch(const KpDev* __restrict__ devs, KpConsol q, const int32_t* __restrict__ soff,
                                                     const int32_t* __restrict__ snodes) {
  __shared__ Slot scratch[KP_MAXK];
  const int lane = threadIdx.x, b = blockIdx.x;
  const KpDev& d = devs[b];
  const int unscheduled = (int)(d.counters[7] + d.counters[8]);
  const int n_new = *d.n_claims;
  consol_decide(d, q, (size_t)b, scratch, d.c_sflags, d.c_smask, d.c_sgte, d.c_slte, d.c_its, n_new > 0 ? d.c_tmpl[0] : -1,
                d.c_req, n_new > 0 ? d.c_npods[0] : 0, soff[b + 1] - soff[b], snodes + soff[b], unscheduled, n_new, b, lane);
}

__global__ void __launch_bounds__(128) k_truncate_claims(KpDev d, PriceTabs pt, int max_n, double* sort_key, int32_t* sort_val,
                                                         unsigned long long* sort_bits, uint8_t* dropped) {
  __shared__ Slot scratch[4][KP_MAXK];
  const int lane = threadIdx.x & 31, wi = threadIdx.x >> 5, warp = blockIdx.x * 4 + wi, nw = gridDim.x * 4;
  const int K = d.K, ITW = d.ITW, nC = *d.n_claims;
  double* sk = sort_key + (size_t)warp * d.T;
  int32_t* sv = sort_val + (size_t)warp * d.T;
  unsigned long long* sb = sort_bits + (size_t)warp * ITW;
  for (int c = warp; c < nC; c += nw) {
    const uint64_t its = lane < ITW ? d.c_its[(size_t)c * ITW + lane] : 0ull;
    int n_its = lane < ITW ? __popcll(its) : 0;
    for (int o = 16; o; o >>= 1) n_its += __shfl_xor_sync(FULL, n_its, o);
    if (n_its <= max_n) continue;
    if (lane < K) scratch[wi][lane] = load_slot(d.c_sflags, d.c_smask, d.c_sgte, d.c_slte, (size_t)c * K + lane, d.has_bounds);
    __syncwarp();
    const unsigned okmask = offering_ok_mask(d, scratch[wi], lane);
    order_by_price(pt, its, n_its, okmask, sk, sv, ITW, lane);
    const uint64_t cur = first_types_bitmap(sv, max_n, sb, ITW, lane);
    if (lane < ITW) d.c_its[(size_t)c * ITW + lane] = cur;
    const bool ok = !d.mv_strict || min_values_ok(d, d.c_tmpl[c], cur, lane);
    if (lane == 0 && !ok) dropped[c] = 1;
    __syncwarp();
  }
}
__global__ void __launch_bounds__(256) k_mark_dropped(const int32_t* pod_target, uint8_t* pod_error, const uint8_t* dropped, int64_t P) {
  const int64_t i = blockIdx.x * (int64_t)blockDim.x + threadIdx.x;
  if (i >= P) return;
  const int t = pod_target[i];
  if (t <= -2 && dropped[-2 - t]) pod_error[i] = KP_PODERR_MINVALUES_TRUNCATED;
}
```

### karpenter_b200/csrc/kp_kernels.cuh

```cuda
#pragma once
#include <cuda_runtime.h>

#include "../../include/karpsolve.h"
#include "kp_slot.hpp"

#define FULL 0xffffffffu

__device__ __forceinline__ KeyInfo key_info(const KpDev& d, int k) {
  return KeyInfo{d.val_int + (size_t)k * 64, d.val_isint[k], d.key_univ[k]};
}
__device__ __forceinline__ Slot load_slot(const uint8_t* f, const uint64_t* m, const int64_t* g, const int64_t* l,
                                          size_t i, int has_bounds) {
  Slot s;
  s.f = f[i];
  s.m = m[i];
  s.gte = has_bounds ? g[i] : 0;
  s.lte = has_bounds ? l[i] : 0;
  return s;
}
__device__ __forceinline__ bool tolerated(const KpDev& d, int tolset, int taintset) {
  if (taintset < 0 || d.n_taintsets == 0) return true;
  return d.tol_ok[(size_t)(tolset + 1) * d.n_taintsets + taintset];
}
__device__ __forceinline__ Slot rs_slot(const KpDev& d, int rs, int k) {
  return load_slot(d.rs_flags, d.rs_mask, d.rs_gte, d.rs_lte, (size_t)rs * d.K + k, d.has_bounds);
}

__device__ __forceinline__ uint64_t fits_word(const KpDev& d, int64_t q_lane, int lane, int* j_lane, uint64_t its) {
  const int R = d.R, ITW = d.ITW;
  int j = 0;
  bool adv = false, fresh = false;
  if (lane < R) {
    const int end = d.ge_off[lane + 1];
    int lo = *j_lane;
    fresh = lo < d.ge_off[lane];
    if (fresh) lo = d.ge_off[lane];
    const int start = lo;
    while (lo < end && d.ge_vals[lo] < q_lane) lo++;
    adv = fresh || lo != start;
    j = lo == end ? -1 : lo;
    *j_lane = lo;
  }
  unsigned advm = __ballot_sync(FULL, adv);
  uint64_t fw = its;
  if (__any_sync(FULL, fresh)) fw &= (lane < ITW) ? d.it_valid[lane] : 0ull;
  while (advm) {
    const int r = __ffs(advm) - 1;
    advm &= advm - 1;
    const int jr = __shfl_sync(FULL, j, r);
    if (lane < ITW) fw &= jr >= 0 ? d.ge_bits[(size_t)jr * ITW + lane] : 0ull;
  }
  return fw;
}
__device__ __forceinline__ uint64_t compat_off_word(const KpDev& d, const Slot* S, int lane) {
  const int K = d.K, ITW = d.ITW;
  bool off_ok = false;
  if (lane < d.D) {
    uint32_t keys = d.off_keys[lane];
    off_ok = true;
    while (keys) {
      int k = __ffs(keys) - 1;
      keys &= keys - 1;
      if (!slot_compatible(key_info(d, k), S[k], d.off_slots[(size_t)lane * K + k], d.key_wellknown[k], true))
        off_ok = false;
    }
  }
  uint32_t off_mask = __ballot_sync(FULL, off_ok);
  uint64_t ow = 0, cw = ~0ull;
  if (lane < ITW) {
    while (off_mask) {
      int dd = __ffs(off_mask) - 1;
      off_mask &= off_mask - 1;
      ow |= d.offset_bits[(size_t)dd * ITW + lane];
    }
    for (int k = 0; k < K; k++) {
      Slot s = S[k];
      if (!slot_present(s)) continue;
      KeyInfo ki = key_info(d, k);
      uint64_t allowed = slot_allowed(ki, s);
      uint64_t bw = d.it_nokey[(size_t)k * ITW + lane];
      if (allowed == ki.univ) {
        bw |= d.it_nonempty[(size_t)k * ITW + lane];
      } else {
        while (allowed) {
          int v = __ffsll((long long)allowed) - 1;
          allowed &= allowed - 1;
          bw |= d.itv[((size_t)d.itv_off[k] + v) * ITW + lane];
        }
      }
      if (op_is_negative(slot_op(s))) bw |= d.it_dne[(size_t)k * ITW + lane];
      cw &= bw;
    }
  } else {
    cw = 0;
  }
  return cw & ow;
}
__device__ __forceinline__ uint64_t filter_its_word(const KpDev& d, const Slot* S, int64_t q_lane, int lane,
                                                    uint64_t* fits_out) {
  int j0 = -1;
  uint64_t fw = fits_word(d, q_lane, lane, &j0, ~0ull);
  *fits_out = fw;
  return compat_off_word(d, S, lane) & fw;
}

__device__ __forceinline__ Slot topo_domains(const KpDev& d, int g, const KpGroup& G, bool self, const Slot& pod_d,
                                             const Slot& node_d, uint64_t reg, uint64_t pop) {
  KeyInfo ki = key_info(d, G.key);
  const int32_t* cnt = d.dom_cnt + G.dom_off;
  uint64_t pod_allowed = slot_allowed(ki, pod_d);
  uint64_t node_allowed = slot_allowed(ki, node_d);
  bool node_in = slot_present(node_d) && slot_op(node_d) == OP_IN;
  Slot out;
  out.f = SF_PRESENT;
  out.m = 0;
  out.gte = 0;
  out.lte = 0;
  if (G.type == KP_TOPO_SPREAD) {
    uint64_t sup = reg & pod_allowed;
    long long mn = 2147483647LL;
    int nsup = __popcll(sup);
    for (uint64_t s = sup; s;) {
      int v = __ffsll((long long)s) - 1;
      s &= s - 1;
      if (cnt[v] < mn) mn = cnt[v];
    }
    if (G.min_domains >= 0 && nsup < G.min_domains) mn = 0;
    uint64_t cand = node_in ? (node_d.m & reg) : (reg & node_allowed);
    long long best_c = 2147483647LL;
    int best = -1;
    while (cand) {
      int v = __ffsll((long long)cand) - 1;
      cand &= cand - 1;
      long long c = (long long)cnt[v] + (self ? 1 : 0);
      if (c - mn <= (long long)G.max_skew && c < best_c) {
        best = v;
        best_c = c;
      }
    }
    if (best >= 0) out.m = 1ull << best;
    return out;
  }
  if (G.type == KP_TOPO_AFFINITY) {
    uint64_t opts = node_in ? (node_d.m & pod_allowed & reg & pop) : (reg & pod_allowed & pop & node_allowed);
    if (opts) {
      out.m = opts;
      return out;
    }
    bool none_populated = (reg & pop) == 0;
    bool any_compat = (reg & pop & pod_allowed) != 0;
    if (self && (none_populated || !any_compat)) {
      Slot pd = slot_present(pod_d) ? pod_d : slot_exists();
      Slot nd = slot_present(node_d) ? node_d : slot_exists();
      Slot inter = slot_intersection(ki, pd, nd);
      uint64_t a = reg & slot_allowed(ki, inter);
      if (a) out.m |= a & (~a + 1);
      uint64_t b = reg & pod_allowed;
      if (b) out.m |= b & (~b + 1);
    }
    return out;
  }
  out.m = reg & ~pop & node_allowed & pod_allowed;
  return out;
}

__device__ __forceinline__ void host_record(const KpDev& d, int row, int g, int host) {
  uint32_t* w = d.host_pop + (size_t)row * d.HW + (host >> 5);
  const uint32_t bit = 1u << (host & 31), cur = *w;
  if (!(cur & bit)) {
    *w = cur | bit;
    d.g_nempty[g]--;
  }
  atomicAdd(d.host_cnt + (size_t)host * d.GHS + row, 1);
}
__device__ __forceinline__ void prefetch_l1(const void* p) { asm volatile("prefetch.global.L1 [%0];" ::"l"(p)); }

struct Eval {
  bool ok;
  bool res_dead;
  bool changed;
  bool compat_fail;
  bool pod_noop;
  int j;
  Slot F;
  int64_t q;
  uint64_t its;
};

#define KP_PG 6
#define TKI_FP 0x100
#define TKI_TK 0x200
#define TKI_FAST 0x400
#define TKI_ABIT 0x800
#define TKI_TOPO 0x1000
#define TKI_ASIG(t) ((t) & 0xff)
struct PodCtx {
  union {
    struct {
      int tolset, rv, moff, mend, roff, rend, fsig, nsig, hoff, hend, cls, pod;
      unsigned long long tmpl_ok;
      int relax;
      int tkinfo;
      unsigned long long ports;
      unsigned long long port_conf;
      int vol_next;
    };
    int hdr[KP_HDR + 11];
  };
  int64_t req[KP_MAXR];
  Slot pod_slot[KP_MAXK];
  Slot strict_slot[KP_MAXK];
  int n_mg, n_rg;
  int m_e[KP_PG];
  int r_g[KP_PG];
  KpGroup mg[KP_PG];
  KpGroup rg[KP_PG];
  int n_hc;
  int4 hc[KP_PG];
  int run_n;
  int run_pod[32];
};
__device__ __forceinline__ void pod_match(const KpDev& d, const PodCtx& px, int i, int* e, KpGroup* G) {
  if (px.n_mg >= 0) {
    *e = px.m_e[i];
    *G = px.mg[i];
  } else {
    *e = d.cls_match[px.moff + i];
    *G = d.groups[*e & 0x3fffffff];
  }
}
__device__ __forceinline__ void pod_rec(const KpDev& d, const PodCtx& px, int i, int* g, KpGroup* G) {
  if (px.n_rg >= 0) {
    *g = px.r_g[i];
    *G = px.rg[i];
  } else {
    *g = d.cls_rec[px.roff + i];
    *G = d.groups[*g];
  }
}

template <bool LEAN = false>
__device__ __forceinline__ Eval eval_candidate(const KpDev& d, const PodCtx& px, bool is_claim, const Slot& base,
                                               int64_t base_q, uint64_t base_its, int base_j, int host, Slot* scratch,
                                               int lane) {
  Eval ev;
  ev.ok = false;
  ev.res_dead = false;
  ev.changed = false;
  ev.compat_fail = false;
  ev.pod_noop = false;
  ev.j = 0;
  const int K = d.K;
  const bool allow_undef = is_claim;
  const bool wk = lane < K ? d.key_wellknown[lane] : false;
  KeyInfo ki = lane < K ? key_info(d, lane) : KeyInfo{d.val_int, 0ull, 0ull};
  Slot pod = lane < K ? px.pod_slot[lane] : slot_absent();
  const bool nb = LEAN || !d.has_bounds;
  bool bad = lane < K && !(nb ? slot_compatible_nb(base, pod, wk, allow_undef) : slot_compatible(ki, base, pod, wk, allow_undef));
  if (__any_sync(FULL, bad)) {
    ev.compat_fail = true;
    return ev;
  }
  Slot M = lane < K ? (nb ? slot_add_nb(base, pod) : slot_add(ki, base, pod)) : slot_absent();
  const int nm = LEAN ? 0 : px.mend - px.moff;
  if (nm > 0) {
    ev.pod_noop = !__any_sync(FULL, lane < K && !slot_eq(M, base));
    Slot Tt = M;
    bool fail = false;
    Slot strict = lane < K ? px.strict_slot[lane] : slot_absent();
    for (int i = 0; i < nm; i++) {
      int e;
      KpGroup G;
      pod_match(d, px, i, &e, &G);
      int g = e & 0x3fffffff;
      bool self = (e >> 30) & 1;
      if (G.key == d.hostname_key) {
        if (lane == 0) {
          int cnt = __ldcg(d.host_cnt + (size_t)host * d.GHS + G.host_row);
          bool ok;
          if (G.type == KP_TOPO_SPREAD)
            ok = cnt + (self ? 1 : 0) <= G.max_skew;
          else if (G.type == KP_TOPO_AFFINITY)
            ok = cnt > 0 || (self && (d.g_ndomains[g] - d.g_nempty[g]) == 0);
          else
            ok = cnt == 0;
          if (!ok) fail = true;
        }
      } else if (lane == G.key) {
        Slot dm = topo_domains(d, g, G, self, strict, M, d.dom_reg[g], d.dom_pop[g]);
        if (dm.m == 0)
          fail = true;
        else
          Tt = slot_add(ki, Tt, dm);
      }
    }
    if (__any_sync(FULL, fail)) return ev;
    bad = lane < K && !slot_compatible(ki, M, Tt, wk, allow_undef);
    if (__any_sync(FULL, bad)) return ev;
    M = lane < K ? slot_add(ki, M, Tt) : slot_absent();
  }
  ev.F = M;
  if (!is_claim) {
    ev.changed = __any_sync(FULL, lane < K && !slot_eq(M, base));
    if (nm <= 0) ev.pod_noop = !ev.changed;
    ev.ok = true;
    return ev;
  }
  const bool changed = __any_sync(FULL, lane < K && !slot_eq(M, base));
  ev.changed = changed;
  if (nm <= 0) ev.pod_noop = !changed;
  int64_t q = base_q + (lane < d.R ? px.req[lane] : 0);
  ev.j = base_j;
  uint64_t fw = fits_word(d, q, lane, &ev.j, base_its);
  uint64_t w = fw;
  if (changed) {
    if (lane < K) scratch[lane] = M;
    __syncwarp();
    w &= compat_off_word(d, scratch, lane);
    __syncwarp();
  }
  ev.q = q;
  ev.its = w;
  ev.ok = __any_sync(FULL, w != 0);
  ev.res_dead = !__any_sync(FULL, fw != 0);
  return ev;
}

struct ClassRegs {
  int hdr;
  int64_t req;
  Slot pod, strict;
};
__device__ __forceinline__ ClassRegs load_class_regs(const KpDev& d, int X, int pod, int lane) {
  ClassRegs c;
  const uint4* p = reinterpret_cast<const uint4*>(d.cls_lane + ((size_t)X * 32 + lane));
  const uint4 a = p[0], b = p[1];
  c.pod.m = (uint64_t)a.x | ((uint64_t)a.y << 32);
  c.strict.m = (uint64_t)a.z | ((uint64_t)a.w << 32);
  c.req = (int64_t)((uint64_t)b.x | ((uint64_t)b.y << 32));
  c.hdr = lane == KP_HDR ? X : (lane == KP_HDR + 1 ? pod : (int)b.z);
  c.pod.f = b.w & 0xffu;
  c.strict.f = (b.w >> 8) & 0xffu;
  c.pod.gte = c.pod.lte = c.strict.gte = c.strict.lte = 0;
  if (d.has_bounds && lane < d.K) {
    const size_t i = (size_t)X * d.K + lane;
    c.pod.gte = d.cp_g[i];
    c.pod.lte = d.cp_l[i];
    c.strict.gte = d.cs_g[i];
    c.strict.lte = d.cs_l[i];
  }
  return c;
}
__device__ __forceinline__ void store_class_regs(const KpDev& d, PodCtx& px, const ClassRegs& c, int lane) {
  if (lane < KP_HDR + 11) px.hdr[lane] = c.hdr;
  if (lane < d.R) px.req[lane] = c.req;
  if (lane < d.K) {
    px.pod_slot[lane] = c.pod;
    px.strict_slot[lane] = c.strict;
  }
  const int moff = __shfl_sync(FULL, c.hdr, 2), mend = __shfl_sync(FULL, c.hdr, 3);
  const int roff = __shfl_sync(FULL, c.hdr, 4), rend = __shfl_sync(FULL, c.hdr, 5);
  const int nm = mend - moff, nr = rend - roff;
  if (nm == 0 && nr == 0) {
    if (lane == 0) {
      px.n_mg = 0;
      px.n_rg = 0;
      px.n_hc = 0;
    }
    return;
  }
  const bool sm = nm <= KP_PG, sr = nr <= KP_PG;
  int e = 0, g = 0;
  if (sm && lane < nm) e = d.cls_match[moff + lane];
  if (sr && lane < nr) g = d.cls_rec[roff + lane];
  if (lane == 0) {
    px.n_mg = sm ? nm : -1;
    px.n_rg = sr ? nr : -1;
  }
  if (sm && lane < nm) px.m_e[lane] = e;
  if (sr && lane < nr) px.r_g[lane] = g;
  if (sm)
    for (int i = 0; i < nm; i++) {
      const int gi = __shfl_sync(FULL, e, i) & 0x3fffffff;
      if (lane < (int)(sizeof(KpGroup) / 4)) reinterpret_cast<int*>(&px.mg[i])[lane] = reinterpret_cast<const int*>(&d.groups[gi])[lane];
    }
  if (sr)
    for (int i = 0; i < nr; i++) {
      const int gi = __shfl_sync(FULL, g, i);
      if (lane < (int)(sizeof(KpGroup) / 4)) reinterpret_cast<int*>(&px.rg[i])[lane] = reinterpret_cast<const int*>(&d.groups[gi])[lane];
    }
  __syncwarp();
  bool is_host = false;
  KpGroup G;
  if (sm && lane < nm) {
    G = px.mg[lane];
    is_host = G.key == d.hostname_key;
  }
  const unsigned hm = __ballot_sync(FULL, is_host);
  if (is_host) px.hc[__popc(hm & ((1u << lane) - 1))] = make_int4(G.host_row, G.type | (((e >> 30) & 1) << 8), G.max_skew, e & 0x3fffffff);
  if (lane == 0) px.n_hc = sm ? __popc(hm) : -1;
}

__device__ __forceinline__ void topo_record(const KpDev& d, const PodCtx& px, const Slot& F, int taintset, int host,
                                            bool allow_undef, int lane) {
  const int K = d.K;
  (void)allow_undef;
  const int nr = px.rend - px.roff;
  for (int i = 0; i < nr; i++) {
    int g;
    KpGroup G;
    pod_rec(d, px, i, &g, &G);
    if (d.n_lazy && !d.g_born[g]) continue;
    bool counts = true;
    if (!G.inverse) {
      if (G.affinity_policy == 1 && G.filter_n > 0) {
        bool any_alt = false;
        for (int a = 0; a < G.filter_n; a++) {
          int rs = d.filter_rs[G.filter_off + a];
          bool bad = lane < K &&
                     !slot_compatible(key_info(d, lane), F, rs_slot(d, rs, lane), d.key_wellknown[lane], false);
          if (!__any_sync(FULL, bad)) {
            any_alt = true;
            break;
          }
        }
        counts = any_alt;
      }
      if (counts && G.taint_policy == 1) {
        counts = tolerated(d, G.tolset, taintset);
      }
    }
    if (!counts) continue;
    if (G.key == d.hostname_key) {
      if (lane == 0) host_record(d, G.host_row, g, host);
    } else {
      uint32_t ff = __shfl_sync(FULL, F.f, G.key);
      uint64_t mm = __shfl_sync(FULL, F.m, G.key);
      if (lane == 0 && (ff & SF_PRESENT)) {
        uint64_t rec = 0;
        if (G.inverse || G.type == KP_TOPO_ANTI_AFFINITY)
          rec = mm;
        else if (!(ff & SF_COMPLEMENT) && __popcll(mm) == 1)
          rec = mm;
        uint64_t bits = rec;
        while (bits) {
          int v = __ffsll((long long)bits) - 1;
          bits &= bits - 1;
          d.dom_cnt[G.dom_off + v]++;
        }
        d.dom_reg[g] |= rec;
        d.dom_pop[g] |= rec;
      }
    }
  }
}

__device__ __forceinline__ unsigned offering_ok_mask(const KpDev& d, const Slot* S, int lane) {
  bool ok = false;
  if (lane < d.D) {
    uint32_t keys = d.off_keys[lane];
    ok = true;
    while (keys) {
      const int k = __ffs(keys) - 1;
      keys &= keys - 1;
      if (!slot_compatible(key_info(d, k), S[k], d.off_slots[(size_t)lane * d.K + k], d.key_wellknown[k], true)) ok = false;
    }
  }
  return __ballot_sync(FULL, ok);
}

__device__ __forceinline__ unsigned long long offerings_to_reserve(const KpDev& d, const int32_t* rsv_cap, const Slot* scratch,
                                                                    uint64_t its, unsigned long long held, int lane, bool* error) {
  *error = false;
  unsigned sets = offering_ok_mask(d, scratch, lane) & d.rsv_sets;
  unsigned long long compat = 0;
  while (sets) {
    const int dd = __ffs(sets) - 1;
    sets &= sets - 1;
    const bool hit = lane < d.ITW && (its & d.offset_bits[(size_t)dd * d.ITW + lane]) != 0;
    if (__any_sync(FULL, hit)) compat |= 1ull << d.set_rsv[dd];
  }
  const bool c0 = lane < d.n_rsv && rsv_cap[lane] > 0, c1 = lane + 32 < d.n_rsv && rsv_cap[lane + 32] > 0;
  const unsigned long long avail = (unsigned long long)__ballot_sync(FULL, c0) | ((unsigned long long)__ballot_sync(FULL, c1) << 32);
  const unsigned long long take = compat & (held | avail);
  if (d.rsv_strict && take == 0 && (compat != 0 || held != 0)) *error = true;
  return take;
}
__device__ __forceinline__ void reservations_commit(const KpDev& d, int32_t* rsv_cap, unsigned long long held,
                                                    unsigned long long take, int lane) {
  const unsigned long long inc = held & ~take, dec = take & ~held;
  if (lane < d.n_rsv) rsv_cap[lane] += (int)((inc >> lane) & 1ull) - (int)((dec >> lane) & 1ull);
  if (lane + 32 < d.n_rsv) rsv_cap[lane + 32] += (int)((inc >> (lane + 32)) & 1ull) - (int)((dec >> (lane + 32)) & 1ull);
  __syncwarp();
}

__device__ __forceinline__ void claims_finalize(const KpDev& d, uint8_t* sflags, uint64_t* smask, const unsigned long long* c_rsv,
                                                int nC, int lane) {
  if (!d.n_rsv || d.rsv_ct_key < 0 || d.rsv_id_key < 0) return;
  for (int c = lane; c < nC; c += 32) {
    const unsigned long long held = c_rsv[c];
    if (!held) continue;
    sflags[(size_t)c * d.K + d.rsv_ct_key] = SF_PRESENT;
    smask[(size_t)c * d.K + d.rsv_ct_key] = 1ull << d.rsv_reserved_val;
    uint64_t vals = 0;
    for (unsigned long long h = held; h;) {
      const int id = __ffsll((long long)h) - 1;
      h &= h - 1;
      vals |= d.rsv_val_of[id];
    }
    const size_t i = (size_t)c * d.K + d.rsv_id_key;
    const Slot cur{sflags[i], smask[i], 0, 0};
    const Slot out = slot_add_nb(cur, Slot{SF_PRESENT, vals, 0, 0});
    sflags[i] = (uint8_t)out.f;
    smask[i] = out.m;
  }
  __syncwarp();
}

__device__ __forceinline__ uint64_t domain_mask(const KpDev& d, const PodCtx& px, int lane, bool* exact) {
  uint64_t ez = ~0ull;
  *exact = true;
  const int nm = px.n_mg;
  const Slot strict = px.strict_slot[d.tk_key];
  const uint64_t univ = d.key_univ[d.tk_key];
  const uint64_t pod_allowed = (strict.f & SF_PRESENT) ? (((strict.f & SF_COMPLEMENT) ? ~strict.m : strict.m) & univ) : univ;
  for (int i = 0; i < nm; i++) {
    const KpGroup G = px.mg[i];
    if (G.key != d.tk_key) continue;
    const int e = px.m_e[i], g = e & 0x3fffffff;
    const bool self = (e >> 30) & 1;
    const uint64_t reg = d.dom_reg[g], pop = d.dom_pop[g];
    if (G.type == KP_TOPO_SPREAD) {
      const int32_t* cnt = d.dom_cnt + G.dom_off;
      const long long c0 = (reg >> lane) & 1ull ? (long long)cnt[lane] : 0, c1 = (reg >> (lane + 32)) & 1ull ? (long long)cnt[lane + 32] : 0;
      const uint64_t sup = reg & pod_allowed;
      long long mn = 2147483647LL;
      if ((sup >> lane) & 1ull) mn = c0;
      if (((sup >> (lane + 32)) & 1ull) && c1 < mn) mn = c1;
      mn = __reduce_min_sync(FULL, (int)mn);
      if (G.min_domains >= 0 && __popcll(sup) < G.min_domains) mn = 0;
      const long long add = self ? 1 : 0;
      const bool ok0 = ((reg >> lane) & 1ull) && c0 + add - mn <= (long long)G.max_skew;
      const bool ok1 = ((reg >> (lane + 32)) & 1ull) && c1 + add - mn <= (long long)G.max_skew;
      const uint64_t m = (uint64_t)__ballot_sync(FULL, ok0) | ((uint64_t)__ballot_sync(FULL, ok1) << 32);
      ez &= m;
    } else if (G.type == KP_TOPO_ANTI_AFFINITY) {
      ez &= reg & ~pop & pod_allowed;
    } else {
      const bool none_populated = (reg & pop) == 0, any_compat = (reg & pop & pod_allowed) != 0;
      if (self && (none_populated || !any_compat))
        *exact = false;
      else
        ez &= reg & pop & pod_allowed;
    }
  }
  return ez;
}

__device__ __forceinline__ void topo_record_fast(const KpDev& d, const PodCtx& px, int z, int taintset, int host, int lane) {
  if (lane < px.n_rg) {
    const KpGroup G = px.rg[lane];
    const int g = px.r_g[lane];
    bool counts = true;
    if (!G.inverse && G.taint_policy == 1) counts = tolerated(d, G.tolset, taintset);
    if (counts) {
      if (G.key == d.hostname_key) {
        host_record(d, G.host_row, g, host);
      } else if (z >= 0) {
        d.dom_cnt[G.dom_off + z]++;
        const uint64_t bit = 1ull << z;
        if (!(d.dom_reg[g] & bit)) d.dom_reg[g] |= bit;
        if (!(d.dom_pop[g] & bit)) d.dom_pop[g] |= bit;
      }
    }
  }
  __syncwarp();
}

__device__ __forceinline__ bool min_values_ok(const KpDev& d, int n, uint64_t its, int lane) {
  for (int e = d.tmpl_mv_off[n]; e < d.tmpl_mv_off[n + 1]; e++) {
    const int m = d.tmpl_mv_key[e], need = d.tmpl_mv_need[e];
    int seen = 0;
    for (int v = d.mv_val_off[m]; v < d.mv_val_off[m + 1] && seen < need; v++) {
      const bool hit = lane < d.ITW && (its & d.mv_masks[(size_t)v * d.ITW + lane]) != 0;
      seen += __any_sync(FULL, hit) ? 1 : 0;
    }
    if (seen < need) return false;
  }
  return true;
}

__global__ void __launch_bounds__(256) k_feasibility(KpDev d, uint64_t* out, int prefilter_only) {
  __shared__ Slot scratch_all[8][KP_MAXK];
  int lane = threadIdx.x & 31, wib = threadIdx.x >> 5;
  Slot* scratch = scratch_all[wib];
  int warps = (gridDim.x * blockDim.x) >> 5;
  int gw = (blockIdx.x * blockDim.x + threadIdx.x) >> 5;
  int npairs = prefilter_only ? d.N : d.X * d.N;
  for (int pair = gw; pair < npairs; pair += warps) {
    int X = prefilter_only ? -1 : pair / d.N, n = prefilter_only ? pair : pair % d.N;
    Slot base = lane < d.K ? rs_slot(d, d.tmpl_rs[n], lane) : slot_absent();
    uint64_t its = lane < d.ITW ? (prefilter_only ? d.tmpl_its_raw : d.tmpl_its)[(size_t)n * d.ITW + lane] : 0ull;
    uint64_t w = 0;
    if (prefilter_only) {
      if (lane < d.K) scratch[lane] = base;
      __syncwarp();
      uint64_t fw;
      w = filter_its_word(d, scratch, 0, lane, &fw) & its;
      __syncwarp();
      if (d.mv_strict && !min_values_ok(d, n, w, lane)) w = 0;
      if (lane < d.ITW) d.tmpl_its[(size_t)n * d.ITW + lane] = w;
    } else {
      bool tol_ok = tolerated(d, d.cls_tolset[X], d.tmpl_taintset[n]);
      KeyInfo ki = lane < d.K ? key_info(d, lane) : KeyInfo{d.val_int, 0ull, 0ull};
      Slot pod = lane < d.K ? rs_slot(d, d.cls_rs[X], lane) : slot_absent();
      bool bad = lane < d.K && !slot_compatible(ki, base, pod, d.key_wellknown[lane], true);
      bool any_bad = __any_sync(FULL, bad);
      Slot M = lane < d.K ? slot_add(ki, base, pod) : slot_absent();
      if (lane < d.K) scratch[lane] = M;
      __syncwarp();
      int64_t q = lane < d.R ? d.tmpl_daemon[(size_t)n * d.R + lane] + d.cls_req[(size_t)X * d.R + lane] : 0;
      uint64_t fw;
      w = filter_its_word(d, scratch, q, lane, &fw) & its;
      __syncwarp();
      if (any_bad || !tol_ok) w = 0;
      if (lane < d.ITW) out[((size_t)X * d.N + n) * d.ITW + lane] = w;
    }
  }
}
```

### karpenter_b200/csrc/kp_tables.hpp

```cpp
#pragma once
#include <cstdint>
#ifndef __CUDACC__
struct int4 { int x, y, z, w; };
struct ulonglong2 { unsigned long long x, y; };
#endif

#define KP_MAXK 32
#define KP_MAXR 8
#define KP_MAX_ITW 32
#define KP_MAX_OFFSETS 32
#define KP_HDR 10

#define SF_COMPLEMENT 0x01u
#define SF_HAS_GTE 0x02u
#define SF_HAS_LTE 0x04u
#define SF_PRESENT 0x10u

#define OP_IN 0
#define OP_NOT_IN 1
#define OP_EXISTS 2
#define OP_DNE 3

struct Slot {
  uint32_t f;
  uint64_t m;
  int64_t gte, lte;
};

struct ClsLane {
  uint64_t pod_m, strict_m;
  int64_t req;
  int32_t hdr;
  uint8_t pod_f, strict_f, pad[2];
};
static_assert(sizeof(ClsLane) == 32, "ClsLane is loaded as two 16-byte vectors");

struct KpGroup {
  int32_t key;
  int32_t type;
  int32_t max_skew;
  int32_t min_domains;
  int32_t inverse;
  int32_t dom_off;
  int32_t filter_off, filter_n;
  int32_t taint_policy, affinity_policy;
  int32_t tolset;
  int32_t host_row;
};
static_assert(sizeof(KpGroup) == 48, "KpGroup is read by value on the solver's critical path: three 16-byte loads");


struct KpDev {
  int K, R, T, ITW, N, X, G, GH, E, D;
  int n_reqsets, n_taintsets, n_tolsets;
  int has_bounds;
  int hostname_key;
  const uint8_t* key_wellknown;
  const uint64_t* key_univ;
  const int64_t* val_int;
  const uint64_t* val_isint;
  const uint8_t* rs_flags;
  const uint64_t* rs_mask;
  const int64_t* rs_gte;
  const int64_t* rs_lte;
  const uint8_t* tol_ok;
  const int32_t* itv_off;
  const uint64_t* itv;
  const uint64_t* it_nokey;
  const uint64_t* it_dne;
  const uint64_t* it_nonempty;
  const uint64_t* it_valid;
  const int32_t* ge_off;
  const int64_t* ge_vals;
  const uint64_t* ge_bits;
  const Slot* off_slots;
  const uint32_t* off_keys;
  const uint64_t* offset_bits;
  int tab_bytes;
  int n_ge, n_itv;
  const int64_t* it_capacity;
  const int32_t* tmpl_rs;
  const int32_t* tmpl_taintset;
  const uint64_t* tmpl_its_raw;
  uint64_t* tmpl_its;
  const int64_t* tmpl_daemon;
  int64_t* tmpl_remaining;
  const uint32_t* tmpl_limit_present;
  int nodes_res;
  const int64_t* cls_req;
  const int32_t* cls_rs;
  const int32_t* cls_tolset;
  const int32_t* cls_relax;
  int n_lazy;
  int32_t* g_born;
  int32_t* g_birth;
  const int32_t* cls_lazy_off;
  const int32_t* cls_lazy;
  int mv_strict;
  const int32_t* tmpl_mv_off;
  const int32_t* tmpl_mv_key;
  const int32_t* tmpl_mv_need;
  const int32_t* mv_val_off;
  const uint64_t* mv_masks;
  int n_rv;
  const int32_t* cls_match;
  const int32_t* cls_rec;
  const ClsLane* cls_lane;
  const int4* cls_hchk;
  const int64_t* cp_g;
  const int64_t* cp_l;
  const int64_t* cs_g;
  const int64_t* cs_l;
  const KpGroup* groups;
  const int32_t* filter_rs;
  int32_t* dom_cnt;
  uint64_t* dom_reg;
  uint64_t* dom_pop;
  int32_t* g_ndomains;
  int32_t* g_nempty;
  int32_t* host_cnt;
  int GHS;
  uint32_t* host_pop;
  int HW;
  int H;
  const int32_t* node_taintset;
  const uint8_t* node_flags;
  int64_t* node_rem;
  uint32_t* node_rem_present;
  uint8_t* node_sflags;
  uint64_t* node_smask;
  int64_t* node_sgte;
  int64_t* node_slte;
  int32_t* node_npods;
  int Cmax;
  int CS;
  int32_t* c_tmpl;
  int32_t* c_npods;
  int64_t* c_req;
  uint8_t* c_sflags;
  uint64_t* c_smask;
  int64_t* c_sgte;
  int64_t* c_slte;
  uint64_t* c_its;
  int32_t* c_j;
  int32_t* order;
  int32_t* cnt_at;
  int n_fsig;
  ulonglong2* cmask;
  unsigned long long* amask;
  unsigned long long tmpl_all;
  int n_nsig, EW;
  uint32_t* nfit;
  uint32_t* nstat;
  uint32_t* nactive;
  int ESW;
  uint32_t* nfit_sum;
  uint32_t* nstat_sum;
  int64_t P;
  const int32_t* pod_class;
  int32_t* queue;
  int32_t* qcls;
  int32_t* last_len;
  int32_t* pod_target;
  uint8_t* pod_error;
  const uint8_t* pod_kind;
  int32_t* n_claims;
  int64_t* counters;
  int32_t* status;
  int stable_order;
  int n_hostports;
  int cohort;
  unsigned long long* c_ports;
  unsigned long long* node_ports;
  const unsigned long long* tmpl_ports;
  int n_rsv, rsv_strict;
  unsigned rsv_sets;
  const int32_t* set_rsv;
  int32_t* rsv_cap;
  unsigned long long* c_rsv;
  int rsv_ct_key, rsv_reserved_val, rsv_id_key;
  unsigned long long rsv_val_of[64];
  int tk_key;
  uint8_t* c_dom;
  long long deadline_ns;
};
```

### karpenter_b200/csrc/kp_wsolve.cuh

```cuda
#pragma once
#include "kp_gosort.cuh"
#include "kp_kernels.cuh"

enum { PERT_NONE = 0, PERT_INC = 1, PERT_APPEND = 2 };

struct WInst {
  int P;
  int32_t* queue;
  int32_t* qcls;
  int32_t* last_len;
  int32_t* pod_target;
  uint8_t* pod_error;
  const uint8_t* pod_kind;
  int Cmax;
  int32_t *c_tmpl, *c_npods;
  int64_t* c_req;
  uint8_t* c_sflags;
  uint64_t* c_smask;
  int64_t *c_sgte, *c_slte;
  uint64_t* c_its;
  int32_t* c_j;
  int CR;
  uint8_t* s_sflags;
  uint64_t* s_smask;
  int64_t* s_req;
  int32_t* s_j;
  uint64_t* s_its;
  int32_t *order, *cnt_at;
  ulonglong2* cmask;
  unsigned long long* amask;
  unsigned long long* g_amask;
  uint8_t *c_dom, *g_c_dom;
  int32_t* rsv_cap;
  unsigned long long* c_rsv;
  unsigned long long *c_ports, *node_ports, *ov_ports;
  int CS;
  int32_t *g_order, *g_cnt_at, *g_c_tmpl;
  ulonglong2* g_cmask;
  int64_t* tmpl_remaining;
  int64_t* node_rem;
  uint32_t* node_rem_present;
  uint8_t* node_sflags;
  uint64_t* node_smask;
  int64_t *node_sgte, *node_slte;
  int32_t* node_npods;
  uint32_t *nfit, *nstat;
  const uint32_t* nactive;
  const uint32_t *nfit_sum, *nstat_sum;
  int n_removed;
  const int32_t* removed;
  int ov_cap, n_ov;
  int32_t* ov_node;
  int64_t* ov_rem;
  uint32_t* ov_present;
  uint8_t* ov_sflags;
  uint64_t* ov_smask;
  int64_t *ov_sgte, *ov_slte;
  int n_claims, n_unsched, n_uninit, status;
  long long ev_existing, ev_inflight, ev_tmpl, commits, slow_sorts, scan_chunks, evals, fast_commits;
};

__device__ __forceinline__ int ov_find(const WInst& I, int node, int lane) {
  for (int b = 0; b < I.n_ov; b += 32) {
    int i = b + lane;
    unsigned m = __ballot_sync(FULL, i < I.n_ov && I.ov_node[i] == node);
    if (m) return b + __ffs(m) - 1;
  }
  return -1;
}

template <bool LEAN = false>
__device__ __forceinline__ void claim_load(const KpDev& d, const WInst& I, int c, int lane, Slot* b, int64_t* q,
                                           uint64_t* its, int* j) {
  const int K = d.K, R = d.R, ITW = d.ITW;
  *b = slot_absent();
  *q = 0;
  *its = 0;
  *j = 0;
  if (c < I.CR) {
    if (lane < K) {
      b->f = I.s_sflags[c * K + lane];
      b->m = I.s_smask[c * K + lane];
    }
    if (lane < R) {
      *q = I.s_req[c * R + lane];
      *j = I.s_j[c * R + lane];
    }
    if (lane < ITW) *its = I.s_its[c * ITW + lane];
  } else {
    if (lane < K) {
      b->f = I.c_sflags[(size_t)c * K + lane];
      b->m = I.c_smask[(size_t)c * K + lane];
    }
    if (lane < R) {
      *q = I.c_req[(size_t)c * R + lane];
      *j = I.c_j[(size_t)c * R + lane];
    }
    if (lane < ITW) *its = I.c_its[(size_t)c * ITW + lane];
  }
  if (!LEAN && d.has_bounds && lane < K) {
    b->gte = I.c_sgte[(size_t)c * K + lane];
    b->lte = I.c_slte[(size_t)c * K + lane];
  }
}
template <bool LEAN = false>
__device__ __forceinline__ void claim_store(const KpDev& d, WInst& I, int c, int lane, const Eval& ev, bool slots) {
  const int K = d.K, R = d.R, ITW = d.ITW;
  if (!LEAN && slots && I.c_dom && lane == d.tk_key)
    I.c_dom[c] = (ev.F.f == SF_PRESENT && __popcll(ev.F.m) == 1) ? (uint8_t)(__ffsll((long long)ev.F.m) - 1) : (uint8_t)0xff;
  if (c < I.CR) {
    if (slots && lane < K) {
      I.s_sflags[c * K + lane] = (uint8_t)ev.F.f;
      I.s_smask[c * K + lane] = ev.F.m;
    }
    if (lane < R) {
      I.s_req[c * R + lane] = ev.q;
      I.s_j[c * R + lane] = ev.j;
    }
    if (lane < ITW) I.s_its[c * ITW + lane] = ev.its;
  } else {
    if (slots && lane < K) {
      I.c_sflags[(size_t)c * K + lane] = (uint8_t)ev.F.f;
      I.c_smask[(size_t)c * K + lane] = ev.F.m;
    }
    if (lane < R) {
      I.c_req[(size_t)c * R + lane] = ev.q;
      I.c_j[(size_t)c * R + lane] = ev.j;
    }
    if (lane < ITW) I.c_its[(size_t)c * ITW + lane] = ev.its;
  }
  if (!LEAN && slots && d.has_bounds && lane < K) {
    I.c_sgte[(size_t)c * K + lane] = ev.F.gte;
    I.c_slte[(size_t)c * K + lane] = ev.F.lte;
  }
}
__device__ __forceinline__ void claim_load_rq(const KpDev& d, const WInst& I, int c, int lane, int64_t* q, int* j) {
  *q = 0;
  *j = 0;
  if (lane < d.R) {
    if (c < I.CR) {
      *q = I.s_req[c * d.R + lane];
      *j = I.s_j[c * d.R + lane];
    } else {
      *q = I.c_req[(size_t)c * d.R + lane];
      *j = I.c_j[(size_t)c * d.R + lane];
    }
  }
}
__device__ __forceinline__ uint64_t claim_load_its(const KpDev& d, const WInst& I, int c, int lane) {
  if (lane >= d.ITW) return 0ull;
  return c < I.CR ? I.s_its[c * d.ITW + lane] : I.c_its[(size_t)c * d.ITW + lane];
}
__device__ __forceinline__ void claim_store_rq(const KpDev& d, WInst& I, int c, int lane, int64_t q, int j, bool with_its,
                                               uint64_t its) {
  if (c < I.CR) {
    if (lane < d.R) {
      I.s_req[c * d.R + lane] = q;
      I.s_j[c * d.R + lane] = j;
    }
    if (with_its && lane < d.ITW) I.s_its[c * d.ITW + lane] = its;
  } else {
    if (lane < d.R) {
      I.c_req[(size_t)c * d.R + lane] = q;
      I.c_j[(size_t)c * d.R + lane] = j;
    }
    if (with_its && lane < d.ITW) I.c_its[(size_t)c * d.ITW + lane] = its;
  }
}
__device__ __forceinline__ void claim_rows_flush(const KpDev& d, WInst& I, int nC, int lane) {
  const int n = nC < I.CR ? nC : I.CR;
  for (int i = lane; i < n * d.K; i += 32) {
    I.c_sflags[i] = I.s_sflags[i];
    I.c_smask[i] = I.s_smask[i];
  }
  for (int i = lane; i < n * d.R; i += 32) {
    I.c_req[i] = I.s_req[i];
    I.c_j[i] = I.s_j[i];
  }
  for (int i = lane; i < n * d.ITW; i += 32) I.c_its[i] = I.s_its[i];
  __syncwarp();
}

struct ScanCtx {
  unsigned long long fbit, rbit, tok;
  bool all_tmpl;
  int hoff, hend;
  int first_clear, first_rclear;
  bool use_ez;
  uint64_t ez;
  const int4* hc;
};
template <int U, bool LEAN = false>
__device__ __forceinline__ int next_candidate(const KpDev& d, const WInst& I, const int32_t* ord, int nC, int from,
                                              ScanCtx& sc, int lane, int E, int* cc_out, int limit = 0x7fffffff) {
  const ulonglong2* cm = I.cmask;
  if (limit > nC) limit = nC;
  for (int base = from; base < limit; base += 32 * U) {
    bool pass[U], fclear[U], rclear[U];
    int c[U];
#pragma unroll
    for (int u = 0; u < U; u++) {
      const int pos = base + u * 32 + lane;
      c[u] = -1;
      pass[u] = fclear[u] = rclear[u] = false;
      if (pos < limit && pos >= from) {
        c[u] = ord[pos];
        const ulonglong2 mk = cm[c[u]];
        fclear[u] = !(mk.x & sc.fbit);
        rclear[u] = !(mk.y & sc.rbit);
        pass[u] = fclear[u] && rclear[u];
        if (pass[u] && !sc.all_tmpl) pass[u] = (sc.tok >> I.c_tmpl[c[u]]) & 1ull;
      }
    }
    if (!LEAN && sc.use_ez) {
#pragma unroll
      for (int u = 0; u < U; u++)
        if (pass[u]) {
          const int z = I.c_dom[c[u]];
          if (z != 0xff) pass[u] = (sc.ez >> z) & 1ull;
        }
    }
    for (int i = sc.hoff; !LEAN && i < sc.hend; i += 2) {
      const bool two = i + 1 < sc.hend;
      const int4 ha = sc.hc[i], hb = two ? sc.hc[i + 1] : ha;
      const bool cnt_a = (ha.y & 0xff) == KP_TOPO_SPREAD, cnt_b = (hb.y & 0xff) == KP_TOPO_SPREAD;
      int ca[U], cb[U];
#pragma unroll
      for (int u = 0; u < U; u++) {
        const int hi = E + c[u];
        ca[u] = cb[u] = 0;
        if (pass[u]) {
          ca[u] = cnt_a ? __ldcg(d.host_cnt + (size_t)hi * d.GHS + ha.x)
                        : (int)((d.host_pop[(size_t)ha.x * d.HW + (hi >> 5)] >> (hi & 31)) & 1u);
          if (two)
            cb[u] = cnt_b ? __ldcg(d.host_cnt + (size_t)hi * d.GHS + hb.x)
                          : (int)((d.host_pop[(size_t)hb.x * d.HW + (hi >> 5)] >> (hi & 31)) & 1u);
        }
      }
#pragma unroll
      for (int r = 0; r < 2; r++) {
        if (r == 1 && !two) break;
        const int4 hc = r == 0 ? ha : hb;
        const int type = hc.y & 0xff, self = hc.y >> 8;
#pragma unroll
        for (int u = 0; u < U; u++) {
          if (!pass[u]) continue;
          const int hcnt = r == 0 ? ca[u] : cb[u];
          if (type == KP_TOPO_SPREAD)
            pass[u] = hcnt + self <= hc.z;
          else if (type == KP_TOPO_AFFINITY)
            pass[u] = hcnt > 0 || (self && (d.g_ndomains[hc.w] - d.g_nempty[hc.w]) == 0);
          else
            pass[u] = hcnt == 0;
        }
      }
    }
#pragma unroll
    for (int u = 0; u < U; u++) {
      if (sc.fbit && sc.first_clear < 0) {
        const unsigned fm = __ballot_sync(FULL, fclear[u]);
        if (fm) sc.first_clear = base + u * 32 + __ffs(fm) - 1;
      }
      if (sc.rbit && sc.first_rclear < 0) {
        const unsigned rm = __ballot_sync(FULL, rclear[u]);
        if (rm) sc.first_rclear = base + u * 32 + __ffs(rm) - 1;
      }
      const unsigned m = __ballot_sync(FULL, pass[u]);
      if (m) {
        const int l = __ffs(m) - 1;
        *cc_out = __shfl_sync(FULL, c[u], l);
        return base + u * 32 + l;
      }
    }
  }
  return -1;
}

template <bool LEAN>
__device__ __forceinline__ bool cheap_pass(const KpDev& d, const WInst& I, const ScanCtx& sc, int c, int E) {
  const ulonglong2 mk = I.cmask[c];
  bool pass = !(mk.x & sc.fbit) && !(mk.y & sc.rbit);
  if (pass && !sc.all_tmpl) pass = (sc.tok >> I.c_tmpl[c]) & 1ull;
  for (int i = sc.hoff; !LEAN && pass && i < sc.hend; i++) {
    const int4 hc = sc.hc[i];
    const int type = hc.y & 0xff, self = hc.y >> 8, hi = E + c;
    const int hcnt = type == KP_TOPO_SPREAD ? __ldcg(d.host_cnt + (size_t)hi * d.GHS + hc.x)
                                            : (int)((d.host_pop[(size_t)hc.x * d.HW + (hi >> 5)] >> (hi & 31)) & 1u);
    if (type == KP_TOPO_SPREAD)
      pass = hcnt + self <= hc.z;
    else if (type == KP_TOPO_AFFINITY)
      pass = hcnt > 0 || (self && (d.g_ndomains[hc.w] - d.g_nempty[hc.w]) == 0);
    else
      pass = hcnt == 0;
  }
  return pass;
}

__device__ __forceinline__ bool fp_fit(const KpDev& d, const WInst& I, const PodCtx& px, int cc, int k, int lane, int64_t* q_out,
                                       int* lo_out, bool* any_adv_out, uint64_t* its_out) {
  int64_t q;
  int j;
  claim_load_rq(d, I, cc, lane, &q, &j);
  int lo = j;
  bool adv = false;
  if (lane < d.R) {
    q += px.req[lane] * (int64_t)k;
    const int end = d.ge_off[lane + 1];
    while (lo < end && d.ge_vals[lo] < q) lo++;
    adv = lo != j;
  }
  unsigned advm = __ballot_sync(FULL, adv);
  const bool any_adv = advm != 0;
  uint64_t its = 0;
  bool ok = true;
  if (any_adv) {
    its = claim_load_its(d, I, cc, lane);
    const int jj = (lane < d.R && lo == d.ge_off[lane + 1]) ? -1 : lo;
    while (advm) {
      const int r = __ffs(advm) - 1;
      advm &= advm - 1;
      const int jr = __shfl_sync(FULL, jj, r);
      if (lane < d.ITW) its &= jr >= 0 ? d.ge_bits[(size_t)jr * d.ITW + lane] : 0ull;
    }
    ok = __any_sync(FULL, its != 0);
  }
  *q_out = q;
  *lo_out = lo;
  *any_adv_out = any_adv;
  *its_out = its;
  return ok;
}

__device__ __forceinline__ void migrate_small(const KpDev& d, WInst& I, int nC, int lane) {
  for (int i = lane; i < nC; i += 32) {
    I.g_order[i] = I.order[i];
    I.g_cnt_at[i] = I.cnt_at[i];
    I.g_c_tmpl[i] = I.c_tmpl[i];
    I.g_cmask[i] = I.cmask[i];
    I.g_amask[i] = I.amask[i];
    if (I.c_dom) I.g_c_dom[i] = I.c_dom[i];
  }
  __syncwarp();
  if (lane == 0) {
    I.order = I.g_order;
    I.cnt_at = I.g_cnt_at;
    I.c_tmpl = I.g_c_tmpl;
    I.cmask = I.g_cmask;
    I.amask = I.g_amask;
    if (I.c_dom) I.c_dom = I.g_c_dom;
    I.CS = 0;
  }
  __syncwarp();
}

#define KP_RING 8
struct StageRing {
  volatile int produced;
  volatile int consumed;
  volatile int tail_pub;
  volatile int done;
  volatile int skip_to;
  PodCtx slot[KP_RING];
};

template <bool COHORT>
__device__ void stager_run(const KpDev& d, const WInst& I, StageRing* ring, const int lane) {
  const int cap = I.P + 1;
  for (int base = 0;;) {
    int avail;
    for (;;) {
      if (ring->done) return;
      const int sk = __shfl_sync(FULL, (int)ring->skip_to, 0);
      if (sk > base) base = sk;
      avail = __shfl_sync(FULL, (int)ring->tail_pub, 0) - base;
      if (avail > 0) break;
      __nanosleep(64);
    }
    __threadfence_block();
    if (avail > 32) avail = 32;
    int li = 0, X = -1;
    if (lane < avail) {
      const int qi = (base + lane) % cap;
      li = __ldcg(I.queue + qi);
      X = __ldcg(I.qcls + qi);
    }
    ClassRegs nxt = load_class_regs(d, __shfl_sync(FULL, X, 0), __shfl_sync(FULL, li, 0), lane);
    bool rebased = false;
    for (int i = 0; i < avail; i++) {
      const int idx = base + i;
      const ClassRegs c = nxt;
      if (i + 1 < avail) nxt = load_class_regs(d, __shfl_sync(FULL, X, i + 1), __shfl_sync(FULL, li, i + 1), lane);
      int sk = 0;
      for (;;) {
        if (ring->done) return;
        sk = ring->skip_to;
        if (sk > idx || idx - ring->consumed < KP_RING) break;
        __nanosleep(32);
      }
      sk = __shfl_sync(FULL, sk, 0);
      if (sk > idx) {
        base = sk;
        rebased = true;
        break;
      }
      PodCtx& slot = ring->slot[idx & (KP_RING - 1)];
      store_class_regs(d, slot, c, lane);
      if (COHORT) {
        const int Xi = __shfl_sync(FULL, X, i);
        const unsigned same = __ballot_sync(FULL, lane >= i && lane < avail && X == Xi && base + lane < I.P);
        const unsigned tail_m = same >> i;
        const int run = tail_m == FULL ? 32 : __ffs(~tail_m) - 1;
        const int rp = __shfl_sync(FULL, li, (i + lane) & 31);
        slot.run_pod[lane] = rp;
        if (lane == 0) slot.run_n = run;
      }
      __syncwarp();
      if (slot.n_hc > 0) {
        const int g8 = lane >> 3, l8 = lane & 7;
        for (int k = g8; k < slot.n_hc; k += 4) {
          const int w = (d.E >> 5) + l8 * 32;
          if (w < d.HW) prefetch_l1(d.host_pop + (size_t)slot.hc[k].x * d.HW + w);
        }
      }
      if (slot.n_mg > 0 && lane < 2 * slot.n_mg) {
        const KpGroup& G = slot.mg[lane >> 1];
        if (G.key == d.tk_key) prefetch_l1(d.dom_cnt + G.dom_off + (lane & 1) * 32);
      }
      __threadfence_block();
      __syncwarp();
      if (lane == 0) ring->produced = idx + 1;
    }
    if (!rebased) base += avail;
  }
}

struct CohortOut {
  int state;
  int npods;
  int nevals;
  long long ev_sum;
  int pert, pert_pos;
  unsigned moved;
  int w0, gE;
};
template <bool LEAN>
__device__ __noinline__ CohortOut cohort_try(const KpDev& d, WInst& I, const PodCtx& px, const ScanCtx sc, int32_t* ord, int32_t* cnt,
                                             const int nC, const int lb, const int cpos, const int cc, const int E, const int lane,
                                             const unsigned long long abit, const unsigned long long rbit, const bool fast_ok,
                                             const bool has_tk) {
  CohortOut out;
  out.state = 0;
  out.npods = 0;
  out.nevals = 0;
  out.ev_sum = 0;
  out.pert = PERT_NONE;
  out.pert_pos = 0;
  out.moved = 0;
  out.w0 = 0;
  out.gE = 0;
  bool fp0 = (I.amask[cc] & abit) != 0;
  if (fp0 && !fast_ok && has_tk) fp0 = I.c_dom[cc] != 0xff;
  if (!fp0) return out;
  int w0 = cpos;
  if (!LEAN && sc.use_ez) {
    ScanCtx st = sc;
    st.use_ez = false;
    st.first_clear = 0;
    st.first_rclear = 0;
    int c2;
    w0 = st.hend > st.hoff ? next_candidate<4, LEAN>(d, I, ord, nC, lb, st, lane, E, &c2)
                           : next_candidate<1, LEAN>(d, I, ord, nC, lb, st, lane, E, &c2);
    if (w0 < 0 || w0 > cpos) w0 = cpos;
  }
  const int pw = w0 + lane;
  int wc = -1, wn = -1;
  if (pw < nC) {
    wc = ord[pw];
    wn = cnt[pw];
  }
  const int c0 = __shfl_sync(FULL, wn, 0);
  const unsigned gmask = __ballot_sync(FULL, pw < nC && wn == c0);
  const int gsz = gmask == FULL ? 32 : __ffs(~gmask) - 1;
  const int L = px.run_n;
  if (fast_ok && gsz == 1) {
    const int nxt = __shfl_sync(FULL, wn, 1);
    int kcap = L;
    if (w0 + 1 < nC && (long long)nxt - c0 + 1 < kcap) kcap = nxt - c0 + 1;
    int64_t q, qb;
    int lo, lob;
    bool adv, advb;
    uint64_t its, itsb;
    int k = kcap;
    out.nevals = 1;
    if (!fp_fit(d, I, px, cc, k, lane, &q, &lo, &adv, &its)) {
      int good = 0, bad = kcap;
      while (bad - good > 1) {
        const int mid = (good + bad) >> 1;
        if (fp_fit(d, I, px, cc, mid, lane, &qb, &lob, &advb, &itsb)) {
          good = mid;
          q = qb;
          lo = lob;
          adv = advb;
          its = itsb;
        } else {
          bad = mid;
        }
      }
      k = good;
    }
    if (k == 0) {
      if (lane == 0) I.cmask[cc].y |= rbit;
      __syncwarp();
      out.state = 1;
      return out;
    }
    claim_store_rq(d, I, cc, lane, q, lo, adv, its);
    if (lane == 0) cnt[cpos] += k;
    if (I.pod_target && lane < k) {
      I.pod_target[px.run_pod[lane]] = KP_TARGET_CLAIM(cc);
      I.pod_error[px.run_pod[lane]] = KP_PODERR_NONE;
    }
    __syncwarp();
    out.state = 2;
    out.npods = k;
    out.ev_sum = (long long)k * (cpos + 1);
    out.pert = PERT_INC;
    out.pert_pos = cpos;
    return out;
  }
  if (!(gsz >= 2 && cpos < w0 + gsz && (d.stable_order || nC <= 12 || nC >= 50))) return out;
  bool wpass = false, wfp = false;
  int wz = -1;
  if (lane < gsz) {
    wpass = cheap_pass<LEAN>(d, I, sc, wc, E);
    if (wpass) {
      wfp = (I.amask[wc] & abit) != 0;
      if (wfp && !fast_ok && has_tk) {
        wz = I.c_dom[wc];
        wfp = wz != 0xff;
      }
    }
  }
  unsigned avail = __ballot_sync(FULL, wpass && wfp);
  const unsigned bar = __ballot_sync(FULL, wpass && !wfp);
  if (bar) avail &= (1u << (__ffs(bar) - 1)) - 1;
  if (!((avail >> (cpos - w0)) & 1u)) return out;
  const bool gend_known = gsz < 32 || w0 + 32 >= nC;
  unsigned picked = 0;
  int npick = 0, nmoved = 0, my_t = -1, j = 0;
  int prev_l = -1, prev_pj = 0;
  bool prev_inv = false;
  while (j < L) {
    if (prev_l >= 0) {
      bool stable = true;
      if (prev_inv && !d.stable_order && nC > 12) {
        const int q4 = nC / 4, pj = prev_pj;
        stable = !(pj == q4 - 1 || pj == q4 || pj == 2 * q4 - 1 || pj == 2 * q4 || pj == 3 * q4 - 1 || pj == 3 * q4);
      }
      if (!stable) break;
      if (lane == prev_l) my_t = nmoved;
      nmoved++;
      picked |= 1u << prev_l;
      prev_l = -1;
    }
    unsigned allowed = avail;
    if (!LEAN && has_tk) {
      uint64_t ez = sc.ez;
      if (j > 0) {
        bool exact;
        ez = domain_mask(d, px, lane, &exact);
        if (!exact) break;
      }
      allowed &= __ballot_sync(FULL, wz >= 0 && ((ez >> wz) & 1ull));
    }
    if (!allowed) break;
    const int l = __ffs(allowed) - 1;
    const int cl = __shfl_sync(FULL, wc, l);
    int64_t q;
    int lo;
    bool adv;
    uint64_t its;
    out.nevals++;
    avail &= ~(1u << l);
    if (!fp_fit(d, I, px, cl, 1, lane, &q, &lo, &adv, &its)) {
      if (lane == 0) I.cmask[cl].y |= rbit;
      __syncwarp();
      continue;
    }
    claim_store_rq(d, I, cl, lane, q, lo, adv, its);
    const int pj = w0 + l - __popc(picked & ((1u << l) - 1));
    out.ev_sum += pj + 1;
    if (lane == 0 && I.pod_target) {
      I.pod_target[px.run_pod[j]] = KP_TARGET_CLAIM(cl);
      I.pod_error[px.run_pod[j]] = KP_PODERR_NONE;
    }
    if (!LEAN && !fast_ok) topo_record_fast(d, px, __shfl_sync(FULL, wz, l), d.tmpl_taintset[I.c_tmpl[cl]], E + cl, lane);
    __syncwarp();
    const unsigned rest = gmask & ~picked & ~(1u << l);
    prev_inv = !gend_known || (rest & ~((2u << l) - 1u)) != 0;
    prev_l = l;
    prev_pj = pj;
    j++;
    npick++;
  }
  if (npick == 0) {
    out.state = 1;
    return out;
  }
  const int m = nmoved;
  int gE = w0 + gsz - 1;
  if (gsz == 32 && m > 0) {
    for (int s0 = w0 + 32;; s0 += 32) {
      const int i = s0 + lane;
      const bool in = i < nC && cnt[i] == c0;
      const int vo = in ? ord[i] : 0;
      const unsigned gk = __ballot_sync(FULL, in);
      const int n = gk == FULL ? 32 : __ffs(~gk) - 1;
      __syncwarp();
      if (lane < n) {
        ord[i - m] = vo;
        cnt[i - m] = c0;
      }
      __syncwarp();
      gE = s0 + n - 1;
      if (n < 32) break;
    }
  }
  const bool mv = (picked >> lane) & 1u;
  const int rank = __popc(~picked & ((1u << lane) - 1));
  __syncwarp();
  if (lane < gsz) {
    if (mv) {
      ord[gE - my_t] = wc;
      cnt[gE - my_t] = c0 + 1;
    } else {
      ord[w0 + rank] = wc;
      cnt[w0 + rank] = lane == prev_l ? c0 + 1 : c0;
    }
  }
  __syncwarp();
  out.state = 2;
  out.npods = npick;
  out.moved = picked;
  out.w0 = w0;
  out.gE = gE;
  if (prev_l >= 0) {
    out.pert = PERT_INC;
    out.pert_pos = w0 + __popc(~picked & ((1u << prev_l) - 1));
  }
  return out;
}

__device__ __forceinline__ void load_alt_slots(const KpDev& d, PodCtx& px, int alt, int lane) {
  if (lane < d.K) {
    const ClsLane c = d.cls_lane[(size_t)alt * 32 + lane];
    Slot sl;
    sl.f = c.pod_f;
    sl.m = c.pod_m;
    sl.gte = 0;
    sl.lte = 0;
    if (d.has_bounds) {
      sl.gte = d.cp_g[(size_t)alt * d.K + lane];
      sl.lte = d.cp_l[(size_t)alt * d.K + lane];
    }
    px.pod_slot[lane] = sl;
  }
  __syncwarp();
}
__device__ __forceinline__ int next_alt(const KpDev& d, int alt) { return d.cls_lane[(size_t)alt * 32 + KP_HDR + 10].hdr; }

template <bool OVERLAY, bool STAGED, bool LEAN = false, bool COHORT = false, bool VOL = false>
__device__ void wsolve_run(const KpDev& d, WInst& I, PodCtx& ctx, Slot* scratch, const int lane, StageRing* ring = nullptr) {
  const int K = d.K, R = d.R, ITW = d.ITW, E = d.E, EW = d.EW;
  const int P = I.P;
  int head = 0, tail = P;
  const int cap = P + 1;
  int hq = 0, tq = P;
  const long long watchdog_limit = 4ll * P + 1024;
  int nC = 0;
  int pert = PERT_NONE, pert_pos = 0;
  long long ev_existing = 0, ev_inflight = 0, ev_tmpl = 0, commits = 0, slow_sorts = 0, scan_chunks = 0, evals = 0, fast_commits = 0;
  int n_unsched = 0, n_uninit = 0, status = KP_OK, n_born = 0;
  int32_t* ord = I.order;
  int32_t* cnt = I.cnt_at;
  int alive_tmpl = 0;
  for (int n = 0; n < d.N; n++) {
    uint64_t w = lane < ITW ? d.tmpl_its[(size_t)n * ITW + lane] : 0ull;
    alive_tmpl += __any_sync(FULL, w != 0) ? 1 : 0;
  }
  int n_active_nodes = 0;
  for (int w = lane; w < EW; w += 32) n_active_nodes += __popc(I.nactive[w]);
  for (int o = 16; o; o >>= 1) n_active_nodes += __shfl_xor_sync(FULL, n_active_nodes, o);
  if (OVERLAY) n_active_nodes -= I.n_removed;

  ClassRegs pf;
  int pf_idx = -1, ids_idx = -1, ids_cls = 0, ids_pod = 0;
  pf.hdr = 0;
  pf.req = 0;
  pf.pod = slot_absent();
  pf.strict = slot_absent();

  int lb0 = 0, lb1 = 0;
  int lr0 = 0, lr1 = 0;
  long long watchdog = 0;
  unsigned long long t_start = 0;
  if (d.deadline_ns > 0) asm volatile("mov.u64 %0, %%globaltimer;" : "=l"(t_start));
  for (;;) {
    const int len = tail - head;
    if (len == 0) break;
    if (d.deadline_ns > 0 && (watchdog & 63) == 0) {
      unsigned long long now;
      asm volatile("mov.u64 %0, %%globaltimer;" : "=l"(now));
      now = __shfl_sync(FULL, now, 0);
      if ((long long)(now - t_start) > d.deadline_ns) {
        status = KP_DEADLINE;
        break;
      }
    }
    if (++watchdog > watchdog_limit) {
      status = KP_ERR_INVALID;
      break;
    }
    const int h = head;
    const int hq1 = hq + 1 >= cap ? hq + 1 - cap : hq + 1, hq2 = hq1 + 1 >= cap ? hq1 + 1 - cap : hq1 + 1;
    int li, X;
    if (STAGED) {
      if (lane == 0) ring->consumed = h;
      while (ring->produced <= h) {
      }
      __threadfence_block();
      __syncwarp();
      const PodCtx& sx = ring->slot[h & (KP_RING - 1)];
      li = sx.pod;
      X = sx.cls;
    } else if (ids_idx == h) {
      li = ids_pod;
      X = ids_cls;
    } else {
      li = I.queue[hq];
      X = I.qcls[hq];
    }
    if (h >= P && I.last_len[li] == len) break;
    head = h + 1;
    hq = hq1;
    if (!STAGED) {
      {
        ClassRegs cur = pf_idx == h ? pf : load_class_regs(d, X, li, lane);
        __syncwarp();
        store_class_regs(d, ctx, cur, lane);
        __syncwarp();
      }
      pf_idx = -1;
      if (h + 1 < tail) {
        int nli, nX;
        if (ids_idx == h + 1) {
          nli = ids_pod;
          nX = ids_cls;
        } else {
          nli = I.queue[hq1];
          nX = I.qcls[hq1];
        }
        pf = load_class_regs(d, nX, nli, lane);
        pf_idx = h + 1;
      }
      ids_idx = -1;
      if (h + 2 < tail) {
        ids_pod = I.queue[hq2];
        ids_cls = I.qcls[hq2];
        ids_idx = h + 2;
      }
    }
    PodCtx& pxw = STAGED ? ring->slot[h & (KP_RING - 1)] : ctx;
    int Xc = X;
  try_pod:
    const PodCtx& px = pxw;
    const int rv = px.rv, fsig = px.fsig;
    const unsigned long long fbit = (fsig >= 0 && fsig < 64) ? 1ull << fsig : 0ull;
    const unsigned long long rbit = (rv < 64 && !(VOL && px.vol_next >= 0)) ? 1ull << rv : 0ull;
    bool found = false;

    if (E > 0 && px.nsig >= 0) {
      const uint32_t* fitrow = I.nfit + (size_t)rv * EW;
      const uint32_t* strow = I.nstat + (size_t)px.nsig * EW;
      int seen = 0;
      unsigned live = 0xffffffffu;
      if (d.ESW <= 32) {
        const uint32_t sw = lane < d.ESW ? (I.nfit_sum[(size_t)rv * d.ESW + lane] & I.nstat_sum[(size_t)px.nsig * d.ESW + lane]) : 0u;
        live = __ballot_sync(FULL, sw != 0);
      }
      for (int w0 = 0; w0 < EW && !found; w0 += 32) {
        if (d.ESW <= 32 && !((live >> (w0 >> 5)) & 1u)) continue;
        const int w = w0 + lane;
        uint32_t bits = w < EW ? (fitrow[w] & strow[w] & I.nactive[w]) : 0u;
        if (OVERLAY)
          for (int i = 0; i < I.n_removed; i++)
            if ((I.removed[i] >> 5) == w) bits &= ~(1u << (I.removed[i] & 31));
        unsigned has = __ballot_sync(FULL, bits != 0);
        while (has && !found) {
          const int src = __ffs(has) - 1;
          has &= has - 1;
          uint32_t bw = __shfl_sync(FULL, bits, src);
          while (bw && !found) {
            const int b = __ffs(bw) - 1;
            bw &= bw - 1;
            const int node = (w0 + src) * 32 + b;
            seen++;
            int oi = -1;
            if (OVERLAY) oi = ov_find(I, node, lane);
            Slot nb = slot_absent();
            int64_t rem = 0;
            uint32_t pr;
            if (OVERLAY && oi >= 0) {
              if (lane < K) nb = load_slot(I.ov_sflags, I.ov_smask, I.ov_sgte, I.ov_slte, (size_t)oi * K + lane, (!LEAN && d.has_bounds));
              if (lane < R) rem = I.ov_rem[(size_t)oi * R + lane];
              pr = I.ov_present[oi];
            } else {
              if (lane < K)
                nb = load_slot(I.node_sflags, I.node_smask, I.node_sgte, I.node_slte, (size_t)node * K + lane, (!LEAN && d.has_bounds));
              if (lane < R) rem = I.node_rem[(size_t)node * R + lane];
              pr = I.node_rem_present[node];
            }
            if (!LEAN && px.port_conf) {
              const unsigned long long used = (OVERLAY && oi >= 0) ? I.ov_ports[oi] : I.node_ports[node];
              if (used & px.port_conf) continue;
            }
            bool bad = false;
            if (lane < R) {
              const bool present = (pr >> lane) & 1;
              if (present && rem < 0) bad = true;
              if (px.req[lane] > (present ? rem : 0)) bad = true;
            }
            if (__any_sync(FULL, bad)) {
              if (!OVERLAY && lane == 0) I.nfit[(size_t)rv * EW + (node >> 5)] &= ~(1u << (node & 31));
              continue;
            }
            Eval ev = eval_candidate<LEAN>(d, px, false, nb, 0, 0, 0, node, scratch, lane);
            if (VOL && !ev.ok && px.vol_next >= 0) {
              for (int alt = px.vol_next; alt >= 0 && !ev.ok; alt = next_alt(d, alt)) {
                load_alt_slots(d, pxw, alt, lane);
                ev = eval_candidate<LEAN>(d, px, false, nb, 0, 0, 0, node, scratch, lane);
              }
              if (!ev.ok) load_alt_slots(d, pxw, Xc, lane);
            }
            if (!ev.ok) continue;
            if (OVERLAY) {
              const bool oi_new = oi < 0;
              if (oi < 0) {
                oi = I.n_ov;
                if (oi >= I.ov_cap) {
                  status = KP_ERR_CAPACITY;
                  break;
                }
                if (lane == 0) {
                  I.ov_node[oi] = node;
                  I.n_ov = oi + 1;
                }
              }
              if (lane < K) {
                const size_t i = (size_t)oi * K + lane;
                I.ov_sflags[i] = (uint8_t)ev.F.f;
                I.ov_smask[i] = ev.F.m;
                if ((!LEAN && d.has_bounds)) {
                  I.ov_sgte[i] = ev.F.gte;
                  I.ov_slte[i] = ev.F.lte;
                }
              }
              if (lane < R) I.ov_rem[(size_t)oi * R + lane] = rem - px.req[lane];
              if (lane == 0) I.ov_present[oi] = pr | ((1u << R) - 1);
              if (!LEAN && d.n_hostports && lane == 0) I.ov_ports[oi] = (oi_new ? I.node_ports[node] : I.ov_ports[oi]) | px.ports;
              __syncwarp();
            } else {
              if (ev.changed && lane < K) {
                const size_t i = (size_t)node * K + lane;
                I.node_sflags[i] = (uint8_t)ev.F.f;
                I.node_smask[i] = ev.F.m;
                if ((!LEAN && d.has_bounds)) {
                  I.node_sgte[i] = ev.F.gte;
                  I.node_slte[i] = ev.F.lte;
                }
              }
              if (lane < R) I.node_rem[(size_t)node * R + lane] = rem - px.req[lane];
              if (lane == 0) {
                I.node_rem_present[node] = pr | ((1u << R) - 1);
                I.node_npods[node]++;
                if (!LEAN && px.ports) I.node_ports[node] |= px.ports;
              }
            }
            if (lane == 0) {
              if (I.pod_target) {
                I.pod_target[li] = node;
                I.pod_error[li] = KP_PODERR_NONE;
              }
            }
            if (!(d.node_flags[node] & KP_NODE_INITIALIZED) && (!I.pod_kind || I.pod_kind[li] == 0)) n_uninit++;
            if (!LEAN) topo_record(d, px, ev.F, d.node_taintset[node], node, false, lane);
            ev_existing += node + 1;
            found = true;
          }
          if (status != KP_OK) break;
        }
        if (status != KP_OK) break;
      }
      if (status != KP_OK) break;
      if (found) {
        commits++;
        continue;
      }
      ev_existing += n_active_nodes;
    } else if (E > 0) {
      ev_existing += n_active_nodes;
    }

    if (pert != PERT_NONE) {
      const int p = pert_pos;
      const bool inversion = pert == PERT_INC ? (p + 1 < nC && cnt[p + 1] < cnt[p]) : (nC >= 2 && cnt[nC - 1] < cnt[nC - 2]);
      if (inversion) {
        bool stable = d.stable_order || nC <= 12;
        if (!stable && nC >= 50) {
          const int q4 = nC / 4;
          stable = pert == PERT_APPEND || !(p == q4 - 1 || p == q4 || p == 2 * q4 - 1 || p == 2 * q4 || p == 3 * q4 - 1 || p == 3 * q4);
        }
        if (stable) {
          if (pert == PERT_INC) {
            const int ec = cnt[p], eo = ord[p];
            int i0 = p;
            for (;;) {
              const int i = i0 + lane;
              const bool in = i + 1 < nC;
              const int vc = in ? cnt[i + 1] : 0x7fffffff, vo = in ? ord[i + 1] : 0;
              const unsigned stop = __ballot_sync(FULL, vc >= ec);
              const int nmove = stop ? __ffs(stop) - 1 : 32;
              __syncwarp();
              if (lane < nmove) {
                cnt[i] = vc;
                ord[i] = vo;
              }
              __syncwarp();
              i0 += nmove;
              if (nmove < 32) break;
            }
            if (lane == 0) {
              cnt[i0] = ec;
              ord[i0] = eo;
            }
            if (p < lb0 && lb0 <= i0) lb0--;
            if (p < lb1 && lb1 <= i0) lb1--;
            if (p < lr0 && lr0 <= i0) lr0--;
            if (p < lr1 && lr1 <= i0) lr1--;
          } else {
            const int ec = cnt[nC - 1], eo = ord[nC - 1];
            int i0 = nC - 1;
            for (;;) {
              const int i = i0 - lane;
              const bool in = i - 1 >= 0;
              const int vc = in ? cnt[i - 1] : -0x7fffffff, vo = in ? ord[i - 1] : 0;
              const unsigned stop = __ballot_sync(FULL, vc <= ec);
              const int nmove = stop ? __ffs(stop) - 1 : 32;
              __syncwarp();
              if (lane < nmove) {
                cnt[i] = vc;
                ord[i] = vo;
              }
              __syncwarp();
              i0 -= nmove;
              if (nmove < 32) break;
            }
            if (lane == 0) {
              cnt[i0] = ec;
              ord[i0] = eo;
            }
            if (lb0 > i0) lb0 = i0;
            if (lb1 > i0) lb1 = i0;
            if (lr0 > i0) lr0 = i0;
            if (lr1 > i0) lr1 = i0;
          }
        } else {
          WarpSorter s{cnt, ord, lane};
          s.pdqsort(0, nC, WarpSorter::bits_len((unsigned long long)nC));
          slow_sorts++;
          lb0 = 0;
          lb1 = 0;
          lr0 = 0;
          lr1 = 0;
        }
        __syncwarp();
      } else if (pert == PERT_APPEND) {
        if (lb0 > nC - 1) lb0 = nC - 1;
        if (lb1 > nC - 1) lb1 = nC - 1;
        if (lr0 > nC - 1) lr0 = nC - 1;
        if (lr1 > nC - 1) lr1 = nC - 1;
      }
      pert = PERT_NONE;
    }

    {
      ScanCtx sc;
      sc.fbit = fbit;
      sc.rbit = rbit;
      sc.tok = px.tmpl_ok;
      sc.all_tmpl = (sc.tok & d.tmpl_all) == d.tmpl_all;
      sc.first_clear = -1;
      sc.first_rclear = -1;
      sc.use_ez = false;
      sc.ez = ~0ull;
      const int tki = px.tkinfo;
      const unsigned long long abit = (tki & TKI_ABIT) ? 1ull << (tki & 63) : 0ull;
      const bool fast_ok = tki & TKI_FAST;
      bool dom_fp = false, has_tk = false;
      if (!LEAN && (tki & TKI_TOPO)) {
        if (px.n_hc >= 0) {
          sc.hc = px.hc;
          sc.hoff = 0;
          sc.hend = px.n_hc;
        } else {
          sc.hc = d.cls_hchk;
          sc.hoff = px.hoff;
          sc.hend = px.hend;
        }
        dom_fp = (tki & TKI_FP) && I.c_dom != nullptr;
        has_tk = tki & TKI_TK;
        if (dom_fp && has_tk) {
          bool exact;
          sc.ez = domain_mask(d, px, lane, &exact);
          sc.use_ez = exact;
          dom_fp = exact;
        }
        dom_fp = dom_fp && abit != 0;
      } else {
        sc.hc = nullptr;
        sc.hoff = 0;
        sc.hend = 0;
      }
      int lbf = 0, lbr = 0;
      if (fbit) lbf = __shfl_sync(FULL, fsig < 32 ? lb0 : lb1, fsig & 31);
      if (rbit) lbr = __shfl_sync(FULL, rv < 32 ? lr0 : lr1, rv & 31);
      const int lb = lbf > lbr ? lbf : lbr;
      const bool scanned = (sc.tok & d.tmpl_all) != 0;
      int from = lb;
      unsigned coh_moved = 0;
      int coh_w0 = 0, coh_gE = 0, coh_extra = 0;
      bool coh_ok = COHORT && STAGED && !OVERLAY && d.cohort && Xc == X && px.run_n >= 2 && abit != 0 && (fast_ok || dom_fp) &&
                    (LEAN || (px.ports == 0 && px.port_conf == 0)) && (fast_ok || !has_tk || n_active_nodes == 0);
      for (int i = sc.hoff; !LEAN && coh_ok && i < sc.hend; i++)
        if ((sc.hc[i].y & 0xff) == KP_TOPO_AFFINITY) coh_ok = false;
      while (scanned && !found) {
        int cc;
        int cpos;
        if (sc.hend > sc.hoff) {
          const int lim = from + 32;
          cpos = next_candidate<1, LEAN>(d, I, ord, nC, from, sc, lane, E, &cc, lim);
          if (cpos < 0 && lim < nC) cpos = next_candidate<4, LEAN>(d, I, ord, nC, lim, sc, lane, E, &cc);
        } else {
          cpos = next_candidate<1, LEAN>(d, I, ord, nC, from, sc, lane, E, &cc);
        }
        if (cpos < 0) break;
        from = cpos + 1;
        {
          if (!LEAN && px.port_conf && (I.c_ports[cc] & px.port_conf)) continue;
          if (COHORT && coh_ok) {
            const CohortOut co = cohort_try<LEAN>(d, I, px, sc, ord, cnt, nC, lb, cpos, cc, E, lane, abit, rbit, fast_ok, has_tk);
            evals += co.nevals;
            if (co.state == 2) {
              fast_commits += co.npods;
              ev_inflight += co.ev_sum;
              coh_extra = co.npods - 1;
              coh_moved = co.moved;
              coh_w0 = co.w0;
              coh_gE = co.gE;
              pert = co.pert;
              pert_pos = co.pert_pos;
              found = true;
              continue;
            }
            if (co.state == 1) continue;
          }
          int zdom = -1;
          bool fp = false;
          if ((fast_ok || dom_fp) && (I.amask[cc] & abit)) {
            fp = true;
            if (!fast_ok && has_tk) {
              zdom = I.c_dom[cc];
              fp = zdom != 0xff;
            }
          }
          if (fp) {
            int64_t q;
            int lo;
            bool any_adv;
            uint64_t its;
            const bool ok = fp_fit(d, I, px, cc, 1, lane, &q, &lo, &any_adv, &its);
            evals++;
            if (!ok) {
              if (lane == 0) I.cmask[cc].y |= rbit;
              __syncwarp();
              continue;
            }
            claim_store_rq(d, I, cc, lane, q, lo, any_adv, its);
            if (lane == 0) {
              if (!LEAN && px.ports) I.c_ports[cc] |= px.ports;
              cnt[cpos]++;
              if (I.pod_target) {
                I.pod_target[li] = KP_TARGET_CLAIM(cc);
                I.pod_error[li] = KP_PODERR_NONE;
              }
            }
            if (!LEAN && !fast_ok) topo_record_fast(d, px, zdom, d.tmpl_taintset[I.c_tmpl[cc]], E + cc, lane);
            fast_commits++;
            __syncwarp();
            pert = PERT_INC;
            pert_pos = cpos;
            ev_inflight += cpos + 1;
            found = true;
            continue;
          }
          Slot b;
          int64_t bq;
          uint64_t bi;
          int bj;
          claim_load<LEAN>(d, I, cc, lane, &b, &bq, &bi, &bj);
          evals++;
          Eval ev;
          unsigned long long held = 0, take = 0;
          bool alt_loaded = false;
          for (int alt = -1;;) {
            ev = eval_candidate<LEAN>(d, px, true, b, bq, bi, bj, E + cc, scratch, lane);
            if (!LEAN && d.mv_strict && ev.ok && !min_values_ok(d, I.c_tmpl[cc], ev.its, lane)) ev.ok = false;
            if (abit && ev.pod_noop && lane == 0) I.amask[cc] |= abit;
            held = 0;
            take = 0;
            if (!LEAN && d.n_rsv && ev.ok) {
              if (lane < K) scratch[lane] = ev.F;
              __syncwarp();
              held = I.c_rsv[cc];
              bool rerr;
              take = offerings_to_reserve(d, I.rsv_cap, scratch, ev.its, held, lane, &rerr);
              __syncwarp();
              if (rerr) ev.ok = false;
            }
            if (!VOL || ev.ok) break;
            alt = alt < 0 ? px.vol_next : next_alt(d, alt);
            if (alt < 0) break;
            load_alt_slots(d, pxw, alt, lane);
            alt_loaded = true;
          }
          if (VOL && alt_loaded && !ev.ok) load_alt_slots(d, pxw, Xc, lane);
          if (!ev.ok) {
            if (lane == 0) {
              ulonglong2 mk = I.cmask[cc];
              if (ev.res_dead) mk.y |= rbit;
              if (ev.compat_fail) mk.x |= fbit;
              I.cmask[cc] = mk;
            }
            __syncwarp();
            continue;
          }
          claim_store<LEAN>(d, I, cc, lane, ev, ev.changed);
          if (!LEAN && d.n_rsv) {
            reservations_commit(d, I.rsv_cap, held, take, lane);
            if (lane == 0) I.c_rsv[cc] = take;
          }
          if (lane == 0) {
            if (!LEAN && px.ports) I.c_ports[cc] |= px.ports;
            cnt[cpos]++;
            if (I.pod_target) {
              I.pod_target[li] = KP_TARGET_CLAIM(cc);
              I.pod_error[li] = KP_PODERR_NONE;
            }
          }
          if (!LEAN) topo_record(d, px, ev.F, d.tmpl_taintset[I.c_tmpl[cc]], E + cc, true, lane);
          __syncwarp();
          pert = PERT_INC;
          pert_pos = cpos;
          ev_inflight += cpos + 1;
          found = true;
        }
      }
      if (fbit && scanned && lbf == lb) {
        const int nb = sc.first_clear >= 0 ? sc.first_clear : nC;
        if (lane == (fsig & 31)) {
          if (fsig < 32)
            lb0 = nb;
          else
            lb1 = nb;
        }
      }
      if (rbit && scanned && lbr == lb) {
        const int nb = sc.first_rclear >= 0 ? sc.first_rclear : nC;
        if (lane == (rv & 31)) {
          if (rv < 32)
            lr0 = nb;
          else
            lr1 = nb;
        }
      }
      if (found && coh_moved) {
        const int w0 = coh_w0, gE = coh_gE;
#define KP_COH_ADJ(b)                                                          \
  if ((b) > w0 && (b) <= gE) {                                                 \
    const int nb_ = (b) - w0;                                                  \
    (b) -= __popc(coh_moved & (nb_ >= 32 ? FULL : (1u << nb_) - 1u));          \
  }
        KP_COH_ADJ(lb0)
        KP_COH_ADJ(lb1)
        KP_COH_ADJ(lr0)
        KP_COH_ADJ(lr1)
#undef KP_COH_ADJ
      }
      if (found && coh_extra > 0) {
        commits += coh_extra;
        watchdog += coh_extra;
        scan_chunks += coh_extra + 1;
        if (E > 0) ev_existing += (long long)coh_extra * n_active_nodes;
        head += coh_extra;
        hq += coh_extra;
        if (hq >= cap) hq -= cap;
        if (STAGED) {
          if (lane == 0) ring->skip_to = head;
        }
      }
      if (found) {
        commits++;
        continue;
      }
      ev_inflight += nC;
    }

    int err = alive_tmpl ? KP_PODERR_INCOMPATIBLE : KP_PODERR_NO_TEMPLATES;
    for (int n = 0; n < d.N && !found; n++) {
      uint64_t tw = lane < ITW ? d.tmpl_its[(size_t)n * ITW + lane] : 0ull;
      const bool alive = __any_sync(FULL, tw != 0);
      if (!alive) continue;
      ev_tmpl++;
      const uint32_t lp = d.tmpl_limit_present[n];
      if (lp) {
        if (d.nodes_res >= 0 && (lp >> d.nodes_res & 1) && I.tmpl_remaining[(size_t)n * R + d.nodes_res] == 0) continue;
        if (lane < ITW) {
          uint64_t keep = 0;
          for (uint64_t bits = tw; bits;) {
            const int b = __ffsll((long long)bits) - 1;
            bits &= bits - 1;
            const int t = lane * 64 + b;
            bool viable = true;
            for (int r = 0; r < R; r++)
              if ((lp >> r & 1) && d.it_capacity[(size_t)t * R + r] > I.tmpl_remaining[(size_t)n * R + r]) viable = false;
            if (viable) keep |= 1ull << b;
          }
          tw = keep;
        }
        if (!__any_sync(FULL, tw != 0)) continue;
      }
      const int cnew = nC;
      if (cnew >= I.Cmax) {
        status = KP_ERR_CAPACITY;
        break;
      }
      if (!((px.tmpl_ok >> n) & 1ull)) continue;
      if (!LEAN && px.port_conf && (d.tmpl_ports[n] & px.port_conf)) continue;
      if (I.CS && cnew >= I.CS) {
        migrate_small(d, I, nC, lane);
        ord = I.order;
        cnt = I.cnt_at;
      }
      Slot b = lane < K ? rs_slot(d, d.tmpl_rs[n], lane) : slot_absent();
      const int64_t bq = lane < R ? d.tmpl_daemon[(size_t)n * R + lane] : 0;
      Eval ev;
      unsigned long long take = 0;
      bool rerr = false, alt_loaded = false;
      for (int alt = -1;;) {
        ev = eval_candidate<LEAN>(d, px, true, b, bq, tw, -1, E + cnew, scratch, lane);
        if (!LEAN && d.mv_strict && ev.ok && !min_values_ok(d, n, ev.its, lane)) ev.ok = false;
        take = 0;
        rerr = false;
        if (!LEAN && d.n_rsv && ev.ok) {
          if (lane < K) scratch[lane] = ev.F;
          __syncwarp();
          take = offerings_to_reserve(d, I.rsv_cap, scratch, ev.its, 0ull, lane, &rerr);
          __syncwarp();
          if (rerr) ev.ok = false;
        }
        if (!VOL || ev.ok) break;
        alt = alt < 0 ? px.vol_next : next_alt(d, alt);
        if (alt < 0) break;
        load_alt_slots(d, pxw, alt, lane);
        alt_loaded = true;
      }
      if (VOL && alt_loaded && !ev.ok) load_alt_slots(d, pxw, Xc, lane);
      if (rerr) {
        err = KP_PODERR_RESERVED;
        break;
      }
      if (!ev.ok) continue;
      claim_store<LEAN>(d, I, cnew, lane, ev, true);
      if (lane == 0) {
        I.c_tmpl[cnew] = n;
        ord[cnew] = cnew;
        cnt[cnew] = 1;
        if (I.pod_target) {
          I.pod_target[li] = KP_TARGET_CLAIM(cnew);
          I.pod_error[li] = KP_PODERR_NONE;
        }
      }
      if (lane == 0) {
        I.cmask[cnew] = make_ulonglong2(0ull, 0ull);
        I.amask[cnew] = ((px.tkinfo & TKI_ABIT) && ev.pod_noop) ? 1ull << (px.tkinfo & 63) : 0ull;
        if (!LEAN && d.n_rsv) I.c_rsv[cnew] = take;
        if (!LEAN && d.n_hostports) I.c_ports[cnew] = d.tmpl_ports[n] | px.ports;
      }
      if (!LEAN && d.n_rsv) reservations_commit(d, I.rsv_cap, 0ull, take, lane);
      if (lp) {
        for (int r = 0; r < R; r++) {
          if (!(lp >> r & 1)) continue;
          long long mx = 0;
          if (lane < ITW)
            for (uint64_t bits = ev.its; bits;) {
              const int bb = __ffsll((long long)bits) - 1;
              bits &= bits - 1;
              const long long capv = d.it_capacity[(size_t)(lane * 64 + bb) * R + r];
              if (capv > mx) mx = capv;
            }
          for (int o = 16; o; o >>= 1) {
            const long long other = __shfl_xor_sync(FULL, mx, o);
            if (other > mx) mx = other;
          }
          if (lane == 0) I.tmpl_remaining[(size_t)n * R + r] -= mx;
        }
      }
      if (!LEAN && d.GH > 0) {
        for (int g = lane; g < d.G; g += 32)
          if (d.groups[g].key == d.hostname_key) {
            d.g_ndomains[g]++;
            d.g_nempty[g]++;
          }
        __syncwarp();
      }
      if (!LEAN) topo_record(d, px, ev.F, d.tmpl_taintset[n], E + cnew, true, lane);
      __syncwarp();
      nC = cnew + 1;
      pert = PERT_APPEND;
      pert_pos = cnew;
      found = true;
      commits++;
    }
    if (status != KP_OK) break;
    if (!found) {
      const int nx = err == KP_PODERR_RESERVED ? -1 : px.relax;
      if (nx >= 0) {
        Xc = nx;
        for (int i = d.cls_lazy_off[nx]; !LEAN && i < d.cls_lazy_off[nx + 1]; i++) {
          const int g = d.cls_lazy[i];
          if (d.g_born[g]) continue;
          if (lane == 0) {
            d.g_born[g] = 1;
            d.g_birth[g] = n_born;
          }
          n_born++;
          __syncwarp();
        }
        ClassRegs cur = load_class_regs(d, Xc, li, lane);
        __syncwarp();
        store_class_regs(d, pxw, cur, lane);
        __syncwarp();
        goto try_pod;
      }
      if (lane == 0) {
        if (I.pod_target) {
          I.pod_error[li] = (uint8_t)err;
          I.pod_target[li] = KP_TARGET_UNSCHEDULED;
        }
        I.queue[tq] = li;
        I.qcls[tq] = X;
        I.last_len[li] = tail + 1 - head;
      }
      tail++;
      tq = tq + 1 >= cap ? tq + 1 - cap : tq + 1;
      if (STAGED) {
        __threadfence_block();
        if (lane == 0) ring->tail_pub = tail;
      }
      __syncwarp();
    }
  }
  if (STAGED) {
    __syncwarp();
    if (lane == 0) ring->done = 1;
  }
  for (int i = lane; i < nC; i += 32) I.c_npods[ord[i]] = cnt[i];
  n_unsched = tail - head;
  if (I.pod_kind && n_unsched > 0) {
    int keep = 0;
    for (int i = head + lane; i < tail; i += 32) keep += I.pod_kind[I.queue[i % cap]] != KP_EXTRA_PENDING;
    for (int o = 16; o; o >>= 1) keep += __shfl_xor_sync(FULL, keep, o);
    n_unsched = keep;
  }
  if (lane == 0) {
    I.n_claims = nC;
    I.n_unsched = n_unsched;
    I.n_uninit = n_uninit;
    I.status = status;
    I.ev_existing = ev_existing;
    I.ev_inflight = ev_inflight;
    I.ev_tmpl = ev_tmpl;
    I.commits = commits;
    I.slow_sorts = slow_sorts;
    I.scan_chunks = scan_chunks;
    I.evals = evals;
    I.fast_commits = fast_commits;
  }
  __syncwarp();
}
```

Before: 207,100.

## Stage topology-key domain state in shared memory and split claim rows hot/cold

```diff
diff --git a/karpenter_b200/csrc/kp_api.cu b/karpenter_b200/csrc/kp_api.cu
--- a/karpenter_b200/csrc/kp_api.cu
+++ b/karpenter_b200/csrc/kp_api.cu
@@ -98,7 +98,7 @@
   int32_t* trunc_val = nullptr;
   unsigned long long* trunc_bits = nullptr;
   uint8_t* d_dropped = nullptr;
-  int CS = 0, CR = 0;
+  int CS = 0, CQ = 0, CR = 0, tk_groups = 0;
   size_t smem = 0;
   int32_t* d_slot_src = nullptr;
   int64_t n_slots = 0, slot_off = 0;
@@ -146,7 +146,7 @@
   enum Uploader { NONE, SINGLE, BATCH } uploaded = NONE;
   std::vector<std::unique_ptr<Instance>> insts;
   KpDev* d_devs = nullptr;
-  int2* d_plan = nullptr;
+  int4* d_plan = nullptr;
   int devs_cap = 0;
   void* comm = nullptr;
   int comm_rank = 0, comm_world = 1;
@@ -491,6 +491,10 @@
   CK(up_mut(h, in, &d.dom_cnt, t.dom_cnt));
   CK(up_mut(h, in, &d.dom_reg, t.dom_reg));
   CK(up_mut(h, in, &d.dom_pop, t.dom_pop));
+  d.tk_slot = nullptr;
+  d.tk_reg = d.tk_pop = nullptr;
+  d.tk_cnt = nullptr;
+  d.tk_nv = t.plan.tk_key >= 0 ? 64 - __builtin_clzll(t.key_univ[t.plan.tk_key] | 1ull) : 0;
   d.n_lazy = 0;
   for (int32_t b : t.g_born) d.n_lazy += b == 0;
   CK(up_mut(h, in, &d.g_born, t.g_born));
@@ -586,7 +590,7 @@
     CK(up(h, &in.d_host_pop_nodes, bits));
   }
   CK(zeros(h, &d.n_claims, 1));
-  CK(zeros(h, &d.counters, 16));
+  CK(zeros(h, &d.counters, KP_NCOUNTERS));
   CK(zeros(h, &d.status, 1));
   return KP_OK;
 }
@@ -629,16 +633,35 @@
   const size_t fixed = KP_ALIGN16(sizeof(WSolveShared));
   d.tab_bytes = plan_tables(d, fixed, budget);
   size_t tb = d.tab_bytes;
-  auto row_bytes = [&](int cr) {
-    return KP_ALIGN16((size_t)cr * d.K * 8) + KP_ALIGN16((size_t)cr * d.R * 8) + KP_ALIGN16((size_t)cr * d.ITW * 8) +
-           KP_ALIGN16((size_t)cr * d.R * 4) + KP_ALIGN16((size_t)cr * d.K);
+  const bool dom_fp = std::any_of(in.host.plan.fp.begin(), in.host.plan.fp.end(), [](uint8_t f) { return f != 0; });
+  in.tk_groups = 0;
+  if (dom_fp && !in.cohort && d.tk_key >= 0 && d.tk_nv > 0 && d.tk_nv <= 64) {
+    int ntk = 0;
+    for (const KpGroup& G : in.host.groups) ntk += G.key == d.tk_key;
+    if (ntk > 0 && kp_tk_bytes(d, ntk) <= 64 * 1024) {
+      in.tk_groups = ntk;
+      tb += kp_tk_bytes(d, ntk);
+    }
+  }
+  auto hot_bytes = [&](int n) { return KP_ALIGN16((size_t)n * d.R * 8) + KP_ALIGN16((size_t)n * d.R * 4); };
+  auto cold_bytes = [&](int n) {
+    return KP_ALIGN16((size_t)n * d.K * 8) + KP_ALIGN16((size_t)n * d.ITW * 8) + KP_ALIGN16((size_t)n * d.K);
   };
   int CR = std::min(d.Cmax, 512);
-  while (CR > 0 && fixed + tb + row_bytes(CR) > budget / 2) CR -= 32;
+  while (CR > 0 && fixed + tb + hot_bytes(CR) + cold_bytes(CR) > budget / 2) CR -= 32;
   CR = std::max(CR, 0);
-  if (getenv("KP_CS_LIMIT")) CR = std::min(CR, 32);
-  if (const char* e = getenv("KP_CR")) CR = std::min(CR, std::max(0, atoi(e)) / 32 * 32);
-  tb += CR ? row_bytes(CR) : 0;
+  const size_t rows = CR ? hot_bytes(CR) + cold_bytes(CR) : 0;
+  int CQ = CR;
+  if (dom_fp) {
+    CQ = std::min((d.Cmax + 31) / 32 * 32, (int)(rows / ((size_t)d.R * 12 + 1)) / 32 * 32);
+    while (CQ > 0 && hot_bytes(CQ) > rows) CQ -= 32;
+    CR = 0;
+    while (CR + 32 <= CQ && hot_bytes(CQ) + cold_bytes(CR + 32) <= rows) CR += 32;
+  }
+  if (getenv("KP_CS_LIMIT")) CQ = std::min(CQ, 32);
+  if (const char* e = getenv("KP_CR")) CQ = std::min(CQ, std::max(0, atoi(e)) / 32 * 32);
+  CR = std::min(CR, CQ);
+  tb += (CQ ? hot_bytes(CQ) : 0) + (CR ? cold_bytes(CR) : 0);
   auto small_bytes = [&](int cs) { return (size_t)cs * 37; };
   int CS = 0;
   if (fixed + tb + small_bytes(64) + 64 <= budget) {
@@ -659,8 +682,12 @@
             !in.host.has_vol_alts && !getenv("KP_NO_LEAN");
   if (in.host.has_vol_alts) in.cohort = false;
   in.CS = CS;
+  in.CQ = CQ;
   in.CR = CR;
   in.smem = fixed + tb + (CS ? small_bytes(CS) : 0) + 64;
+  if (getenv("KP_DEBUG"))
+    fprintf(stderr, "[kp] solver plan: tables %zu B, topology-key groups on chip %d, hot rows %d, cold rows %d, small arrays %d, %zu B shared\n",
+            (size_t)d.tab_bytes, in.tk_groups, CQ, CR, CS, in.smem);
 }
 
 static void begin_upload(kp_handle* h, kp_handle::Uploader by) {
@@ -880,11 +907,11 @@
     h->d_plan = nullptr;
     h->devs_cap = 0;
     CK(cudaMalloc(&h->d_devs, sizeof(KpDev) * n));
-    CK(cudaMalloc(&h->d_plan, sizeof(int2) * n));
+    CK(cudaMalloc(&h->d_plan, sizeof(int4) * n));
     h->devs_cap = n;
   }
   std::vector<KpDev> devs(n);
-  std::vector<int2> plan(n);
+  std::vector<int4> plan(n);
   size_t smem = 0;
   for (int b = 0; b < n; b++) {
     Instance& in = *h->insts[b];
@@ -893,11 +920,11 @@
     int rc = reset_dynamic(h, in);
     if (rc != KP_OK) return rc;
     devs[b] = in.dev;
-    plan[b] = make_int2(in.CS, in.CR);
+    plan[b] = make_int4(in.CS, in.CQ, in.CR, in.tk_groups);
     smem = std::max(smem, in.smem);
   }
   CK(cudaMemcpyAsync(h->d_devs, devs.data(), sizeof(KpDev) * n, cudaMemcpyHostToDevice, h->stream));
-  CK(cudaMemcpyAsync(h->d_plan, plan.data(), sizeof(int2) * n, cudaMemcpyHostToDevice, h->stream));
+  CK(cudaMemcpyAsync(h->d_plan, plan.data(), sizeof(int4) * n, cudaMemcpyHostToDevice, h->stream));
   CK(cudaEventRecord(h->ev0, h->stream));
   h->stats.kernel_launches = 0;
   h->stats.cohort_pods = 0;
@@ -1182,6 +1209,16 @@
 }
 
 double kp_comm_last_allreduce_ms(kp_handle* h) { return h->allreduce_ms; }
+
+#ifdef KP_PHASE_PROF
+int kp_phase_profile(kp_handle* h, int32_t instance, int64_t* out, int32_t n) {
+  Instance* in = pick_instance(h, instance);
+  if (!in || n < KP_NPHASE + 1) return h->err = "kp_phase_profile: no such instance or buffer too small", -1;
+  cudaSetDevice(h->device);
+  CK(cudaMemcpy(out, in->dev.counters + KP_PROF_AT, (KP_NPHASE + 1) * 8, cudaMemcpyDeviceToHost));
+  return KP_NPHASE + 1;
+}
+#endif
 
 void kp_comm_destroy(kp_handle* h) {
   if (h->comm && g_nccl.CommDestroy) g_nccl.CommDestroy(h->comm);
diff --git a/karpenter_b200/csrc/kp_consolidate.cuh b/karpenter_b200/csrc/kp_consolidate.cuh
--- a/karpenter_b200/csrc/kp_consolidate.cuh
+++ b/karpenter_b200/csrc/kp_consolidate.cuh
@@ -2,6 +2,10 @@
 #include "kp_wsolve.cuh"
 
 #define KP_ALIGN16(x) (((x) + 15) & ~(size_t)15)
+
+__host__ __device__ inline size_t kp_tk_bytes(const KpDev& d, int ntk) {
+  return KP_ALIGN16((size_t)d.G * 4) + 2 * KP_ALIGN16((size_t)ntk * 8) + KP_ALIGN16((size_t)ntk * d.tk_nv * 4);
+}
 
 __host__ __device__ inline size_t kp_tab_bytes(const KpDev& d) {
   size_t K = d.K, R = d.R, ITW = d.ITW, D = d.D > 0 ? d.D : 1, N = d.N > 0 ? d.N : 1;
@@ -124,7 +128,7 @@
 };
 
 template <bool LEAN, bool COHORT, bool VOL>
-__device__ __forceinline__ void wsolve_cta(const KpDev& d_in, int CS, int CR) {
+__device__ __forceinline__ void wsolve_cta(const KpDev& d_in, int CS, int CQ, int CR, int ntk) {
   extern __shared__ __align__(16) unsigned char smem_raw[];
   WSolveShared& sh = *reinterpret_cast<WSolveShared*>(smem_raw);
   const int lane = threadIdx.x & 31, warp = threadIdx.x >> 5;
@@ -132,6 +136,34 @@
   stage_tables(d_in, &sh.ds, tab);
   const KpDev& d = sh.ds;
   WInst& I = sh.inst;
+  unsigned char* p = tab + d_in.tab_bytes;
+  int32_t* s_slot = nullptr;
+  uint64_t *s_reg = nullptr, *s_pop = nullptr;
+  int32_t* s_cnt = nullptr;
+  if (ntk > 0) {
+    const int nv = d_in.tk_nv;
+    s_slot = reinterpret_cast<int32_t*>(p);
+    s_reg = reinterpret_cast<uint64_t*>(p + KP_ALIGN16((size_t)d_in.G * 4));
+    s_pop = s_reg + KP_ALIGN16((size_t)ntk * 8) / 8;
+    s_cnt = reinterpret_cast<int32_t*>(s_pop + KP_ALIGN16((size_t)ntk * 8) / 8);
+    if (warp == 0) {
+      for (int base = 0, n = 0; base < d_in.G; base += 32) {
+        const int g = base + lane;
+        const KpGroup* G_ = g < d_in.G ? d_in.groups + g : nullptr;
+        const bool on = G_ && G_->key == d_in.tk_key;
+        const unsigned m = __ballot_sync(FULL, on);
+        const int s = n + __popc(m & ((1u << lane) - 1));
+        if (g < d_in.G) s_slot[g] = on ? s : -1;
+        if (on) {
+          s_reg[s] = d_in.dom_reg[g];
+          s_pop[s] = d_in.dom_pop[g];
+          for (int v = 0; v < nv; v++) s_cnt[s * nv + v] = d_in.dom_cnt[G_->dom_off + v];
+        }
+        n += __popc(m);
+      }
+    }
+    p += kp_tk_bytes(d_in, ntk);
+  }
   const int Cmax = d.Cmax;
   if (threadIdx.x == 0) {
     sh.ring.produced = 0;
@@ -190,17 +222,26 @@
     I.c_ports = d.c_ports;
     I.node_ports = d.node_ports;
     I.ov_ports = nullptr;
+    I.CQ = 0;
     I.CR = 0;
-    unsigned char* p = tab + d_in.tab_bytes;
+    if (ntk > 0) {
+      sh.ds.tk_slot = s_slot;
+      sh.ds.tk_reg = s_reg;
+      sh.ds.tk_pop = s_pop;
+      sh.ds.tk_cnt = s_cnt;
+    }
+    if (CQ > 0) {
+      I.s_req = reinterpret_cast<int64_t*>(p);
+      p += KP_ALIGN16((size_t)CQ * d.R * 8);
+      I.s_j = reinterpret_cast<int32_t*>(p);
+      p += KP_ALIGN16((size_t)CQ * d.R * 4);
+      I.CQ = CQ;
+    }
     if (CR > 0) {
       I.s_smask = reinterpret_cast<uint64_t*>(p);
       p += KP_ALIGN16((size_t)CR * d.K * 8);
-      I.s_req = reinterpret_cast<int64_t*>(p);
-      p += KP_ALIGN16((size_t)CR * d.R * 8);
       I.s_its = reinterpret_cast<uint64_t*>(p);
       p += KP_ALIGN16((size_t)CR * d.ITW * 8);
-      I.s_j = reinterpret_cast<int32_t*>(p);
-      p += KP_ALIGN16((size_t)CR * d.R * 4);
       I.s_sflags = reinterpret_cast<uint8_t*>(p);
       p += KP_ALIGN16((size_t)CR * d.K);
       I.CR = CR;
@@ -228,6 +269,16 @@
   wsolve_run<false, true, LEAN, COHORT, VOL>(d, I, sh.ring.slot[0], sh.scratch, lane, &sh.ring);
   const int nC = I.n_claims;
   claim_rows_flush(d, I, nC, lane);
+  if (ntk > 0) {
+    for (int g = lane; g < d.G; g += 32) {
+      const int s = s_slot[g];
+      if (s < 0) continue;
+      d_in.dom_reg[g] = s_reg[s];
+      d_in.dom_pop[g] = s_pop[s];
+      for (int v = 0; v < d.tk_nv; v++) d_in.dom_cnt[d_in.groups[g].dom_off + v] = s_cnt[s * d.tk_nv + v];
+    }
+    __syncwarp();
+  }
   if (!LEAN) claims_finalize(d, I.c_sflags, I.c_smask, I.c_rsv, nC, lane);
   if (I.CS > 0) {
     for (int i = lane; i < nC; i += 32) {
@@ -249,11 +300,16 @@
     d.counters[7] = I.n_unsched;
     d.counters[8] = I.n_uninit;
     d.counters[9] = I.fast_commits;
+#ifdef KP_PHASE_PROF
+    for (int p = 0; p < KP_NPHASE; p++) d.counters[KP_PROF_AT + p] = I.prof[p];
+    d.counters[KP_PROF_AT + KP_NPHASE] = I.prof_total;
+#endif
   }
 }
 template <bool LEAN, bool COHORT, bool VOL = false>
-__global__ void __launch_bounds__(64, 1) k_wsolve_batch(const KpDev* __restrict__ devs, const int2* __restrict__ plan) {
-  wsolve_cta<LEAN, COHORT, VOL>(devs[blockIdx.x], plan[blockIdx.x].x, plan[blockIdx.x].y);
+__global__ void __launch_bounds__(64, 1) k_wsolve_batch(const KpDev* __restrict__ devs, const int4* __restrict__ plan) {
+  const int4 pl = plan[blockIdx.x];
+  wsolve_cta<LEAN, COHORT, VOL>(devs[blockIdx.x], pl.x, pl.y, pl.z, LEAN || COHORT ? 0 : pl.w);
 }
 
 struct KpConsol {
@@ -659,6 +715,7 @@
     I.nfit_sum = d.nfit_sum;
     I.nstat_sum = d.nstat_sum;
     I.CS = 0;
+    I.CQ = 0;
     I.CR = 0;
     I.c_dom = nullptr;
     I.g_c_dom = nullptr;
diff --git a/karpenter_b200/csrc/kp_kernels.cuh b/karpenter_b200/csrc/kp_kernels.cuh
--- a/karpenter_b200/csrc/kp_kernels.cuh
+++ b/karpenter_b200/csrc/kp_kernels.cuh
@@ -104,10 +104,20 @@
   return compat_off_word(d, S, lane) & fw;
 }
 
+struct GroupState {
+  uint64_t *reg, *pop;
+  int32_t* cnt;
+};
+__device__ __forceinline__ GroupState tk_state(const KpDev& d, int g, const KpGroup& G) {
+  const int s = (d.tk_slot && G.key == d.tk_key) ? d.tk_slot[g] : -1;
+  if (s >= 0) return GroupState{d.tk_reg + s, d.tk_pop + s, d.tk_cnt + s * d.tk_nv};
+  return GroupState{d.dom_reg + g, d.dom_pop + g, d.dom_cnt + G.dom_off};
+}
+
 __device__ __forceinline__ Slot topo_domains(const KpDev& d, int g, const KpGroup& G, bool self, const Slot& pod_d,
                                              const Slot& node_d, uint64_t reg, uint64_t pop) {
   KeyInfo ki = key_info(d, G.key);
-  const int32_t* cnt = d.dom_cnt + G.dom_off;
+  const int32_t* cnt = tk_state(d, g, G).cnt;
   uint64_t pod_allowed = slot_allowed(ki, pod_d);
   uint64_t node_allowed = slot_allowed(ki, node_d);
   bool node_in = slot_present(node_d) && slot_op(node_d) == OP_IN;
@@ -287,7 +297,8 @@
           if (!ok) fail = true;
         }
       } else if (lane == G.key) {
-        Slot dm = topo_domains(d, g, G, self, strict, M, d.dom_reg[g], d.dom_pop[g]);
+        const GroupState st = tk_state(d, g, G);
+        Slot dm = topo_domains(d, g, G, self, strict, M, *st.reg, *st.pop);
         if (dm.m == 0)
           fail = true;
         else
@@ -443,13 +454,14 @@
         else if (!(ff & SF_COMPLEMENT) && __popcll(mm) == 1)
           rec = mm;
         uint64_t bits = rec;
+        const GroupState st = tk_state(d, g, G);
         while (bits) {
           int v = __ffsll((long long)bits) - 1;
           bits &= bits - 1;
-          d.dom_cnt[G.dom_off + v]++;
+          st.cnt[v]++;
         }
-        d.dom_reg[g] |= rec;
-        d.dom_pop[g] |= rec;
+        *st.reg |= rec;
+        *st.pop |= rec;
       }
     }
   }
@@ -529,9 +541,10 @@
     if (G.key != d.tk_key) continue;
     const int e = px.m_e[i], g = e & 0x3fffffff;
     const bool self = (e >> 30) & 1;
-    const uint64_t reg = d.dom_reg[g], pop = d.dom_pop[g];
+    const GroupState st = tk_state(d, g, G);
+    const uint64_t reg = *st.reg, pop = *st.pop;
     if (G.type == KP_TOPO_SPREAD) {
-      const int32_t* cnt = d.dom_cnt + G.dom_off;
+      const int32_t* cnt = st.cnt;
       const long long c0 = (reg >> lane) & 1ull ? (long long)cnt[lane] : 0, c1 = (reg >> (lane + 32)) & 1ull ? (long long)cnt[lane + 32] : 0;
       const uint64_t sup = reg & pod_allowed;
       long long mn = 2147483647LL;
@@ -567,10 +580,11 @@
       if (G.key == d.hostname_key) {
         host_record(d, G.host_row, g, host);
       } else if (z >= 0) {
-        d.dom_cnt[G.dom_off + z]++;
+        const GroupState st = tk_state(d, g, G);
+        st.cnt[z]++;
         const uint64_t bit = 1ull << z;
-        if (!(d.dom_reg[g] & bit)) d.dom_reg[g] |= bit;
-        if (!(d.dom_pop[g] & bit)) d.dom_pop[g] |= bit;
+        if (!(*st.reg & bit)) *st.reg |= bit;
+        if (!(*st.pop & bit)) *st.pop |= bit;
       }
     }
   }
diff --git a/karpenter_b200/csrc/kp_tables.hpp b/karpenter_b200/csrc/kp_tables.hpp
--- a/karpenter_b200/csrc/kp_tables.hpp
+++ b/karpenter_b200/csrc/kp_tables.hpp
@@ -116,6 +116,10 @@
   int32_t* dom_cnt;
   uint64_t* dom_reg;
   uint64_t* dom_pop;
+  int32_t* tk_slot;
+  uint64_t *tk_reg, *tk_pop;
+  int32_t* tk_cnt;
+  int tk_nv;
   int32_t* g_ndomains;
   int32_t* g_nempty;
   int32_t* host_cnt;
diff --git a/karpenter_b200/csrc/kp_wsolve.cuh b/karpenter_b200/csrc/kp_wsolve.cuh
--- a/karpenter_b200/csrc/kp_wsolve.cuh
+++ b/karpenter_b200/csrc/kp_wsolve.cuh
@@ -3,6 +3,23 @@
 #include "kp_kernels.cuh"
 
 enum { PERT_NONE = 0, PERT_INC = 1, PERT_APPEND = 2 };
+
+enum { PH_POP = 0, PH_SORT, PH_DMASK, PH_SCAN, PH_FAST, PH_RECORD, PH_EVAL, PH_NEW, PH_OTHER, KP_NPHASE };
+#ifdef KP_PHASE_PROF
+#define KP_PROF_LAP(p)                        \
+  do {                                        \
+    const long long t_ = clock64();           \
+    if (lane == 0) I.prof[p] += t_ - prof_t;  \
+    prof_t = t_;                              \
+  } while (0)
+#define KP_PROF_AT 16
+#define KP_NCOUNTERS (KP_PROF_AT + KP_NPHASE + 1)
+#else
+#define KP_PROF_LAP(p) \
+  do {                 \
+  } while (0)
+#define KP_NCOUNTERS 16
+#endif
 
 struct WInst {
   int P;
@@ -20,7 +37,7 @@
   int64_t *c_sgte, *c_slte;
   uint64_t* c_its;
   int32_t* c_j;
-  int CR;
+  int CQ, CR;
   uint8_t* s_sflags;
   uint64_t* s_smask;
   int64_t* s_req;
@@ -58,6 +75,9 @@
   int64_t *ov_sgte, *ov_slte;
   int n_claims, n_unsched, n_uninit, status;
   long long ev_existing, ev_inflight, ev_tmpl, commits, slow_sorts, scan_chunks, evals, fast_commits;
+#ifdef KP_PHASE_PROF
+  long long prof[KP_NPHASE], prof_total;
+#endif
 };
 
 __device__ __forceinline__ int ov_find(const WInst& I, int node, int lane) {
@@ -82,21 +102,22 @@
       b->f = I.s_sflags[c * K + lane];
       b->m = I.s_smask[c * K + lane];
     }
-    if (lane < R) {
-      *q = I.s_req[c * R + lane];
-      *j = I.s_j[c * R + lane];
-    }
     if (lane < ITW) *its = I.s_its[c * ITW + lane];
   } else {
     if (lane < K) {
       b->f = I.c_sflags[(size_t)c * K + lane];
       b->m = I.c_smask[(size_t)c * K + lane];
     }
-    if (lane < R) {
+    if (lane < ITW) *its = I.c_its[(size_t)c * ITW + lane];
+  }
+  if (lane < R) {
+    if (c < I.CQ) {
+      *q = I.s_req[c * R + lane];
+      *j = I.s_j[c * R + lane];
+    } else {
       *q = I.c_req[(size_t)c * R + lane];
       *j = I.c_j[(size_t)c * R + lane];
     }
-    if (lane < ITW) *its = I.c_its[(size_t)c * ITW + lane];
   }
   if (!LEAN && d.has_bounds && lane < K) {
     b->gte = I.c_sgte[(size_t)c * K + lane];
@@ -113,21 +134,22 @@
       I.s_sflags[c * K + lane] = (uint8_t)ev.F.f;
       I.s_smask[c * K + lane] = ev.F.m;
     }
-    if (lane < R) {
-      I.s_req[c * R + lane] = ev.q;
-      I.s_j[c * R + lane] = ev.j;
-    }
     if (lane < ITW) I.s_its[c * ITW + lane] = ev.its;
   } else {
     if (slots && lane < K) {
       I.c_sflags[(size_t)c * K + lane] = (uint8_t)ev.F.f;
       I.c_smask[(size_t)c * K + lane] = ev.F.m;
     }
-    if (lane < R) {
+    if (lane < ITW) I.c_its[(size_t)c * ITW + lane] = ev.its;
+  }
+  if (lane < R) {
+    if (c < I.CQ) {
+      I.s_req[c * R + lane] = ev.q;
+      I.s_j[c * R + lane] = ev.j;
+    } else {
       I.c_req[(size_t)c * R + lane] = ev.q;
       I.c_j[(size_t)c * R + lane] = ev.j;
     }
-    if (lane < ITW) I.c_its[(size_t)c * ITW + lane] = ev.its;
   }
   if (!LEAN && slots && d.has_bounds && lane < K) {
     I.c_sgte[(size_t)c * K + lane] = ev.F.gte;
@@ -138,7 +160,7 @@
   *q = 0;
   *j = 0;
   if (lane < d.R) {
-    if (c < I.CR) {
+    if (c < I.CQ) {
       *q = I.s_req[c * d.R + lane];
       *j = I.s_j[c * d.R + lane];
     } else {
@@ -153,27 +175,29 @@
 }
 __device__ __forceinline__ void claim_store_rq(const KpDev& d, WInst& I, int c, int lane, int64_t q, int j, bool with_its,
                                                uint64_t its) {
-  if (c < I.CR) {
-    if (lane < d.R) {
+  if (lane < d.R) {
+    if (c < I.CQ) {
       I.s_req[c * d.R + lane] = q;
       I.s_j[c * d.R + lane] = j;
-    }
-    if (with_its && lane < d.ITW) I.s_its[c * d.ITW + lane] = its;
-  } else {
-    if (lane < d.R) {
+    } else {
       I.c_req[(size_t)c * d.R + lane] = q;
       I.c_j[(size_t)c * d.R + lane] = j;
     }
-    if (with_its && lane < d.ITW) I.c_its[(size_t)c * d.ITW + lane] = its;
+  }
+  if (with_its && lane < d.ITW) {
+    if (c < I.CR)
+      I.s_its[c * d.ITW + lane] = its;
+    else
+      I.c_its[(size_t)c * d.ITW + lane] = its;
   }
 }
 __device__ __forceinline__ void claim_rows_flush(const KpDev& d, WInst& I, int nC, int lane) {
-  const int n = nC < I.CR ? nC : I.CR;
+  const int n = nC < I.CR ? nC : I.CR, nq = nC < I.CQ ? nC : I.CQ;
   for (int i = lane; i < n * d.K; i += 32) {
     I.c_sflags[i] = I.s_sflags[i];
     I.c_smask[i] = I.s_smask[i];
   }
-  for (int i = lane; i < n * d.R; i += 32) {
+  for (int i = lane; i < nq * d.R; i += 32) {
     I.c_req[i] = I.s_req[i];
     I.c_j[i] = I.s_j[i];
   }
@@ -422,7 +446,7 @@
           if (w < d.HW) prefetch_l1(d.host_pop + (size_t)slot.hc[k].x * d.HW + w);
         }
       }
-      if (slot.n_mg > 0 && lane < 2 * slot.n_mg) {
+      if (!d.tk_slot && slot.n_mg > 0 && lane < 2 * slot.n_mg) {
         const KpGroup& G = slot.mg[lane >> 1];
         if (G.key == d.tk_key) prefetch_l1(d.dom_cnt + G.dom_off + (lane & 1) * 32);
       }
@@ -705,7 +729,14 @@
   long long watchdog = 0;
   unsigned long long t_start = 0;
   if (d.deadline_ns > 0) asm volatile("mov.u64 %0, %%globaltimer;" : "=l"(t_start));
+#ifdef KP_PHASE_PROF
+  long long prof_t = clock64();
+  const long long prof_t0 = prof_t;
+  if (lane == 0)
+    for (int p = 0; p < KP_NPHASE; p++) I.prof[p] = 0;
+#endif
   for (;;) {
+    KP_PROF_LAP(PH_OTHER);
     const int len = tail - head;
     if (len == 0) break;
     if (d.deadline_ns > 0 && (watchdog & 63) == 0) {
@@ -778,6 +809,7 @@
     const unsigned long long fbit = (fsig >= 0 && fsig < 64) ? 1ull << fsig : 0ull;
     const unsigned long long rbit = (rv < 64 && !(VOL && px.vol_next >= 0)) ? 1ull << rv : 0ull;
     bool found = false;
+    KP_PROF_LAP(PH_POP);
 
     if (E > 0 && px.nsig >= 0) {
       const uint32_t* fitrow = I.nfit + (size_t)rv * EW;
@@ -911,6 +943,7 @@
       ev_existing += n_active_nodes;
     }
 
+    KP_PROF_LAP(PH_OTHER);
     if (pert != PERT_NONE) {
       const int p = pert_pos;
       const bool inversion = pert == PERT_INC ? (p + 1 < nC && cnt[p + 1] < cnt[p]) : (nC >= 2 && cnt[nC - 1] < cnt[nC - 2]);
@@ -992,6 +1025,7 @@
       }
       pert = PERT_NONE;
     }
+    KP_PROF_LAP(PH_SORT);
 
     {
       ScanCtx sc;
@@ -1031,6 +1065,7 @@
         sc.hoff = 0;
         sc.hend = 0;
       }
+      KP_PROF_LAP(PH_DMASK);
       int lbf = 0, lbr = 0;
       if (fbit) lbf = __shfl_sync(FULL, fsig < 32 ? lb0 : lb1, fsig & 31);
       if (rbit) lbr = __shfl_sync(FULL, rv < 32 ? lr0 : lr1, rv & 31);
@@ -1053,12 +1088,14 @@
         } else {
           cpos = next_candidate<1, LEAN>(d, I, ord, nC, from, sc, lane, E, &cc);
         }
+        KP_PROF_LAP(PH_SCAN);
         if (cpos < 0) break;
         from = cpos + 1;
         {
           if (!LEAN && px.port_conf && (I.c_ports[cc] & px.port_conf)) continue;
           if (COHORT && coh_ok) {
             const CohortOut co = cohort_try<LEAN>(d, I, px, sc, ord, cnt, nC, lb, cpos, cc, E, lane, abit, rbit, fast_ok, has_tk);
+            KP_PROF_LAP(PH_FAST);
             evals += co.nevals;
             if (co.state == 2) {
               fast_commits += co.npods;
@@ -1093,6 +1130,7 @@
             if (!ok) {
               if (lane == 0) I.cmask[cc].y |= rbit;
               __syncwarp();
+              KP_PROF_LAP(PH_FAST);
               continue;
             }
             claim_store_rq(d, I, cc, lane, q, lo, any_adv, its);
@@ -1104,9 +1142,11 @@
                 I.pod_error[li] = KP_PODERR_NONE;
               }
             }
+            KP_PROF_LAP(PH_FAST);
             if (!LEAN && !fast_ok) topo_record_fast(d, px, zdom, d.tmpl_taintset[I.c_tmpl[cc]], E + cc, lane);
             fast_commits++;
             __syncwarp();
+            KP_PROF_LAP(PH_RECORD);
             pert = PERT_INC;
             pert_pos = cpos;
             ev_inflight += cpos + 1;
@@ -1152,6 +1192,7 @@
               I.cmask[cc] = mk;
             }
             __syncwarp();
+            KP_PROF_LAP(PH_EVAL);
             continue;
           }
           claim_store<LEAN>(d, I, cc, lane, ev, ev.changed);
@@ -1167,8 +1208,10 @@
               I.pod_error[li] = KP_PODERR_NONE;
             }
           }
+          KP_PROF_LAP(PH_EVAL);
           if (!LEAN) topo_record(d, px, ev.F, d.tmpl_taintset[I.c_tmpl[cc]], E + cc, true, lane);
           __syncwarp();
+          KP_PROF_LAP(PH_RECORD);
           pert = PERT_INC;
           pert_pos = cpos;
           ev_inflight += cpos + 1;
@@ -1341,6 +1384,7 @@
       found = true;
       commits++;
     }
+    KP_PROF_LAP(PH_NEW);
     if (status != KP_OK) break;
     if (!found) {
       const int nx = err == KP_PODERR_RESERVED ? -1 : px.relax;
@@ -1380,6 +1424,10 @@
       __syncwarp();
     }
   }
+#ifdef KP_PHASE_PROF
+  KP_PROF_LAP(PH_OTHER);
+  if (lane == 0) I.prof_total = prof_t - prof_t0;
+#endif
   if (STAGED) {
     __syncwarp();
     if (lane == 0) ring->done = 1;
```

New measurement: 218,500, median of 6. +5.5%, better.
